# chenruduan/OAReactDiff

Hardware: AMD Instinct MI355X
Metric: denoising_steps_per_sec (higher is better)
Workload: dtype f32; 1 GPU; EGNNDynamics.forward (LEFTNet H=196 R=96 L=6), B=64 reactions/GPU x 3 objects x 23 atoms, complete graph per reaction (N=4416, E=300288), T=1000 sampler step shape; batch_per_gpu=64, atoms_per_object=23, parallelism=replica x1 (no collective), launch=eager

## Files before the change

oareactdiff_amd/_capi.py:

```python
from __future__ import annotations

import ctypes as C
import os

from .build import LIB

OARD_MAX_OBJECTS = 8
ABI_VERSION = 2048
OARD_OK, OARD_EINVAL, OARD_ENOTCOMPLETE, OARD_EHIP, OARD_ENOMEM = 0, -1, -2, -3, -4
ERRORS = {OARD_EINVAL: "invalid argument / unsupported configuration", OARD_ENOTCOMPLETE: "topology is not complete-per-sample",
          OARD_EHIP: "HIP runtime error", OARD_ENOMEM: "workspace too small"}

PREC_GCL_BF16X3, PREC_EQUI_BF16X3, PREC_TRAIN_BF16X3 = 1, 2, 4
TAP_S, TAP_VEC, TAP_EDGE, TAP_POS_FRAME, TAP_DPOS, TAP_HOUT, TAP_LABELS, TAP_NE1 = 1, 2, 3, 4, 5, 6, 7, 8

EXPORTS = ["oard_version", "oard_supported", "oard_param_count", "oard_packed_bytes", "oard_pack_weights",
           "oard_topology_create", "oard_topology_destroy", "oard_topology_num_nodes", "oard_topology_num_edges",
           "oard_topology_num_inner_edges", "oard_topology_num_samples", "oard_topology_check_edge_index",
           "oard_workspace_bytes", "oard_forward", "oard_active_inner_edges", "oard_debug_lin3u_table", "oard_sampler_step", "oard_sampler_step_dev", "oard_inpaint_step", "oard_inpaint_step_dev", "oard_tap", "oard_debug_stop_after", "oard_debug_option", "oard_timing_enable", "oard_timing_reset",
           "oard_timing_get",
           "oard_topology_create_parts", "oard_topology_export", "oard_tape_bytes", "oard_tape_entry", "oard_forward_train",
           "oard_packed_bwd_bytes", "oard_pack_weights_bwd", "oard_gcl_backward_dx", "oard_edge_node_sums",
           "oard_equi_backward_dx", "oard_scalarize_backward", "oard_equi_msg_backward", "oard_lin3u_forward", "oard_lin3u_backward", "oard_wgrad_scratch_bytes", "oard_wgrad",
           "oard_train_scratch_bytes", "oard_train_scratch_poison", "oard_train_scratch_entry", "oard_train_tail_backward",
           "oard_train_layer_backward", "oard_train_init_backward", "oard_train_stage_backward",
           "oard_loss_prepare", "oard_loss_terms", "oard_loss_eval_prepare", "oard_loss_eval_terms", "oard_adamw_step", "oard_adamw_step_dev", "oard_nan_replace",
           "oard_adamw_step_ema", "oard_adamw_step_dev_ema", "oard_ema_update", "oard_kabsch_rmsd", "oard_matched_rmsd", "oard_rank_metrics",
           "oard_graph_create", "oard_graph_destroy", "oard_graph_num_nodes", "oard_graph_num_edges", "oard_graph_object_rows",
           "oard_graph_is_complete", "oard_graph_workspace_bytes", "oard_graph_forward", "oard_library_stream",
           "oard_confidence_forward", "oard_confidence_forward_train", "oard_confidence_tail_backward", "oard_dataset_gather"]
STAGE_RECOMPUTE, STAGE_UPDATE, STAGE_MESSAGE, STAGE_GCL_NODE, STAGE_NODE_PRE, STAGE_GCL_EDGE, STAGE_EQUI_EDGE = range(7)
SCRATCH_XH, SCRATCH_XQ, SCRATCH_CR, SCRATCH_DCD, SCRATCH_DCR = range(1, 6)

TOPO_NODE_REF, TOPO_NODE_OBJ, TOPO_NODE_ROW, TOPO_NODE_SAMPLE, TOPO_NODE_TIDX, TOPO_SAMPLE_PTR, TOPO_GROUP_PTR, \
    TOPO_INNER_SRC, TOPO_INNER_TGT, TOPO_ROW_SRC, TOPO_ROW_TGT = range(1, 12)
TAPE_HIN, TAPE_GEO, TAPE_RBF, TAPE_PP0, TAPE_X1 = 1, 2, 3, 4, 5
TAPE_S_IN, TAPE_VEC_IN, TAPE_EW, TAPE_AGG, TAPE_S_MID, TAPE_Z1, TAPE_Z2, TAPE_ATT, TAPE_Z3, TAPE_ZD1, TAPE_CD, TAPE_S_A, TAPE_VEC_A = range(16, 29)


class OardConfig(C.Structure):
    _fields_ = [
        ("hidden", C.c_int32), ("num_radial", C.c_int32), ("num_layers", C.c_int32), ("in_hidden", C.c_int32),
        ("n_obj", C.c_int32), ("node_nf", C.c_int32 * OARD_MAX_OBJECTS), ("enc_alias", C.c_int32 * OARD_MAX_OBJECTS),
        ("condition_nf", C.c_int32), ("condition_time", C.c_int32), ("pos_dim", C.c_int32), ("cutoff", C.c_float),
        ("reflect_equiv", C.c_int32), ("precision", C.c_int32),
    ]


OARD_STORE_OBJECTS = 3


class OardReactionStore(C.Structure):
    _fields_ = [
        ("offsets", C.c_void_p * OARD_STORE_OBJECTS), ("pos", C.c_void_p * OARD_STORE_OBJECTS), ("z", C.c_void_p * OARD_STORE_OBJECTS),
        ("sel", C.c_void_p), ("target", C.c_void_p), ("rmsd", C.c_void_p), ("ediff", C.c_void_p * 2),
        ("n_raw", C.c_int64), ("n_sel", C.c_int64), ("n_obj", C.c_int32),
        ("src_obj", C.c_int32 * OARD_STORE_OBJECTS), ("reflect_obj", C.c_int32 * OARD_STORE_OBJECTS),
        ("append_charge", C.c_int32 * OARD_STORE_OBJECTS),
        ("swap", C.c_int32), ("reflect", C.c_int32), ("center", C.c_int32), ("zero_charge", C.c_int32), ("append_frag", C.c_int32),
    ]


class OardError(RuntimeError):
    pass


def check(rc: int, what: str) -> None:
    if rc != OARD_OK:
        raise OardError(f"{what} failed: {ERRORS.get(rc, rc)}")


def ptr_array(tensors, n=None):
    if tensors is None:
        return None
    ptrs = [None if t is None else t.data_ptr() for t in tensors]
    return (C.c_void_p * (len(ptrs) if n is None else n))(*ptrs)


_lib = None


def lib() -> C.CDLL:
    global _lib
    if _lib is not None:
        return _lib
    if not os.path.exists(LIB):
        raise OardError(f"{LIB} not found: build it with `python -m oareactdiff_amd.build` "
                        "(there is no CPU fallback for the HIP backend)")
    L = C.CDLL(LIB)
    vp, i32, i64, sz = C.c_void_p, C.c_int32, C.c_int64, C.c_size_t
    cfgp = C.POINTER(OardConfig)
    L.oard_version.restype = C.c_int
    got = L.oard_version()
    if got != ABI_VERSION:
        raise OardError(f"{LIB} has ABI version {got}, this package expects {ABI_VERSION}: rebuild it "
                        "(`python -m oareactdiff_amd.build --force`, or the script that made the OARD_LIB build)")
    L.oard_supported.argtypes = [cfgp]; L.oard_supported.restype = C.c_int
    L.oard_param_count.argtypes = [cfgp]; L.oard_param_count.restype = sz
    L.oard_packed_bytes.argtypes = [cfgp]; L.oard_packed_bytes.restype = sz
    L.oard_pack_weights.argtypes = [cfgp, C.POINTER(vp), sz, vp, sz, vp]; L.oard_pack_weights.restype = C.c_int
    L.oard_topology_create.argtypes = [cfgp, C.POINTER(i64), C.POINTER(i64), i64, C.POINTER(vp)]
    L.oard_topology_create.restype = C.c_int
    L.oard_topology_destroy.argtypes = [vp]; L.oard_topology_destroy.restype = None
    for f in ("oard_topology_num_nodes", "oard_topology_num_edges", "oard_topology_num_inner_edges",
              "oard_topology_num_samples"):
        getattr(L, f).argtypes = [vp]; getattr(L, f).restype = i64
    L.oard_topology_check_edge_index.argtypes = [vp, vp, i64, vp, vp]; L.oard_topology_check_edge_index.restype = C.c_int
    L.oard_workspace_bytes.argtypes = [cfgp, vp]; L.oard_workspace_bytes.restype = sz
    L.oard_forward.argtypes = [cfgp, vp, vp, C.POINTER(vp), vp, C.c_int, vp, C.POINTER(vp), vp, sz, vp, vp]
    L.oard_forward.restype = C.c_int
    L.oard_confidence_forward.argtypes = [cfgp, vp, vp, C.POINTER(vp), C.POINTER(vp), vp, C.c_int, vp, vp, vp, sz, vp, vp]
    L.oard_confidence_forward.restype = C.c_int
    L.oard_confidence_forward_train.argtypes = [cfgp, vp, vp, C.POINTER(vp), C.POINTER(vp), vp, C.c_int, vp, vp, vp, sz, vp, sz, vp, vp]
    L.oard_confidence_forward_train.restype = C.c_int
    L.oard_confidence_tail_backward.argtypes = [cfgp, vp, vp, C.POINTER(vp), vp, vp, vp, C.POINTER(vp), vp, sz, vp]
    L.oard_confidence_tail_backward.restype = C.c_int
    L.oard_debug_lin3u_table.argtypes = [cfgp, vp, C.c_int, vp, vp]; L.oard_debug_lin3u_table.restype = C.c_int
    L.oard_active_inner_edges.argtypes = [cfgp, vp, vp, sz, C.POINTER(i64), vp]; L.oard_active_inner_edges.restype = C.c_int
    L.oard_sampler_step.argtypes = [cfgp, vp, C.c_int, C.POINTER(vp), C.POINTER(vp), C.POINTER(vp), C.POINTER(vp),
                                    C.c_float, C.c_float, C.c_float, C.c_int, C.POINTER(vp), vp]
    L.oard_sampler_step.restype = C.c_int
    L.oard_sampler_step_dev.argtypes = [cfgp, vp, C.c_int, C.POINTER(vp), C.POINTER(vp), C.POINTER(vp), C.POINTER(vp), vp, C.c_int,
                                        C.POINTER(vp), vp]
    L.oard_sampler_step_dev.restype = C.c_int
    pv = C.POINTER(vp)
    L.oard_inpaint_step.argtypes = [cfgp, vp, C.c_uint, pv, pv, pv, pv, pv, pv, pv, C.POINTER(C.c_float), C.c_int, pv, vp]
    L.oard_inpaint_step.restype = C.c_int
    L.oard_inpaint_step_dev.argtypes = [cfgp, vp, C.c_uint, pv, pv, pv, pv, pv, pv, pv, vp, C.c_int, pv, vp]
    L.oard_inpaint_step_dev.restype = C.c_int
    L.oard_tap.argtypes = [cfgp, vp, vp, C.c_int, C.c_int, vp, vp]; L.oard_tap.restype = C.c_int
    ci = C.c_int
    L.oard_topology_create_parts.argtypes = [cfgp, C.POINTER(i64), C.POINTER(i64), i64, ci, C.POINTER(vp)]
    L.oard_topology_create_parts.restype = ci
    L.oard_topology_export.argtypes = [vp, ci, vp, i64, vp]; L.oard_topology_export.restype = ci
    L.oard_tape_bytes.argtypes = [cfgp, vp]; L.oard_tape_bytes.restype = sz
    L.oard_tape_entry.argtypes = [cfgp, vp, ci, ci, C.POINTER(sz), C.POINTER(i64), C.POINTER(i64)]; L.oard_tape_entry.restype = ci
    L.oard_forward_train.argtypes = [cfgp, vp, vp, C.POINTER(vp), vp, ci, vp, C.POINTER(vp), vp, sz, vp, sz, vp, vp]
    L.oard_forward_train.restype = ci
    L.oard_packed_bwd_bytes.argtypes = [cfgp]; L.oard_packed_bwd_bytes.restype = sz
    L.oard_pack_weights_bwd.argtypes = [cfgp, C.POINTER(vp), sz, vp, sz, vp]; L.oard_pack_weights_bwd.restype = ci
    L.oard_gcl_backward_dx.argtypes = [cfgp, vp, vp, ci, vp, vp, vp, vp, vp, vp, vp, vp, vp]; L.oard_gcl_backward_dx.restype = ci
    L.oard_edge_node_sums.argtypes = [cfgp, vp, vp, vp, vp, vp]; L.oard_edge_node_sums.restype = ci
    L.oard_equi_backward_dx.argtypes = [cfgp, vp, vp, ci, vp, vp, vp, vp, vp]; L.oard_equi_backward_dx.restype = ci
    L.oard_scalarize_backward.argtypes = [cfgp, vp, vp, vp, vp, ci, vp, vp, vp, vp]; L.oard_scalarize_backward.restype = ci
    L.oard_equi_msg_backward.argtypes = [cfgp, vp, vp, ci, vp, vp, vp, vp, vp, vp, vp, vp, vp]; L.oard_equi_msg_backward.restype = ci
    L.oard_lin3u_forward.argtypes = [cfgp, vp, ci, vp, i64, vp, vp]; L.oard_lin3u_forward.restype = ci
    L.oard_lin3u_backward.argtypes = [cfgp, vp, ci, vp, vp, i64, vp, vp, vp, vp, vp, vp, vp]; L.oard_lin3u_backward.restype = ci
    L.oard_wgrad_scratch_bytes.argtypes = [ci, ci, i64]; L.oard_wgrad_scratch_bytes.restype = sz
    L.oard_wgrad.argtypes = [vp, ci, ci, ci, ci, ci, vp, ci, ci, ci, ci, ci, ci, i64, vp, vp, vp, sz, vp]; L.oard_wgrad.restype = ci
    pvp = C.POINTER(vp)
    L.oard_train_scratch_bytes.argtypes = [cfgp, vp]; L.oard_train_scratch_bytes.restype = sz
    L.oard_train_scratch_poison.argtypes = [cfgp, vp, vp, sz, vp]; L.oard_train_scratch_poison.restype = ci
    L.oard_train_scratch_entry.argtypes = [cfgp, vp, ci, C.POINTER(sz), C.POINTER(i64), C.POINTER(i64)]; L.oard_train_scratch_entry.restype = ci
    L.oard_train_tail_backward.argtypes = [cfgp, vp, vp, vp, vp, pvp, vp, vp, pvp, pvp, vp, sz, vp]; L.oard_train_tail_backward.restype = ci
    L.oard_train_layer_backward.argtypes = [cfgp, vp, vp, vp, vp, ci, vp, vp, vp, pvp, pvp, vp, sz, vp]; L.oard_train_layer_backward.restype = ci
    L.oard_train_init_backward.argtypes = [cfgp, vp, vp, vp, vp, pvp, vp, vp, pvp, pvp, vp, sz, vp]; L.oard_train_init_backward.restype = ci
    L.oard_train_stage_backward.argtypes = [cfgp, vp, vp, vp, vp, ci, ci, vp, vp, vp, vp, vp, vp, pvp, pvp, vp, sz, vp]
    L.oard_train_stage_backward.restype = ci
    L.oard_nan_replace.argtypes = [cfgp, vp, vp, pvp, pvp, vp]; L.oard_nan_replace.restype = ci
    pf, cf = C.POINTER(C.c_float), C.c_float
    L.oard_loss_prepare.argtypes = [cfgp, vp, pvp, pvp, pvp, pvp, vp, vp, ci, pf, pf, ci, ci, pvp, pvp, vp]; L.oard_loss_prepare.restype = ci
    L.oard_loss_terms.argtypes = [cfgp, vp, pvp, pvp, pvp, pvp, pvp, vp, vp, ci, pf, pf, pf, ci, ci, vp, vp, pvp, vp]; L.oard_loss_terms.restype = ci
    cd = C.c_double
    L.oard_loss_eval_prepare.argtypes = [cfgp, vp, pvp, pvp, pvp, pvp, pvp, vp, vp, ci, pf, pf, ci, ci, pvp, pvp, pvp, pvp, vp]
    L.oard_loss_eval_prepare.restype = ci
    L.oard_loss_eval_terms.argtypes = [cfgp, vp, pvp, pvp, pvp, pvp, pvp, pvp, pvp, vp, vp, vp, ci, pf, pf, pf, ci, cd, ci, vp, vp, vp]
    L.oard_loss_eval_terms.restype = ci
    L.oard_adamw_step.argtypes = [vp, vp, vp, vp, vp, i64, cd, cd, cd, cd, cd, i64, ci, cd, vp]; L.oard_adamw_step.restype = ci
    L.oard_adamw_step_dev.argtypes = [vp, vp, vp, vp, vp, i64, cd, cd, cd, cd, cd, ci, ci, vp, ci, vp, vp, vp, vp]; L.oard_adamw_step_dev.restype = ci
    L.oard_adamw_step_ema.argtypes = [vp, vp, vp, vp, vp, i64, cd, cd, cd, cd, cd, i64, ci, cd, vp, cd, vp]; L.oard_adamw_step_ema.restype = ci
    L.oard_adamw_step_dev_ema.argtypes = [vp, vp, vp, vp, vp, i64, cd, cd, cd, cd, cd, ci, ci, vp, ci, vp, vp, vp, vp, cd, vp]
    L.oard_adamw_step_dev_ema.restype = ci
    L.oard_ema_update.argtypes = [vp, vp, i64, cd, vp]; L.oard_ema_update.restype = ci
    L.oard_kabsch_rmsd.argtypes = [vp, i64, vp, i64, vp, i64, ci, cf, vp, vp, vp, vp]; L.oard_kabsch_rmsd.restype = ci
    L.oard_matched_rmsd.argtypes = [vp, i64, vp, i64, vp, vp, vp, i64, ci, cf, ci, vp, vp, vp, vp, vp, vp]; L.oard_matched_rmsd.restype = ci
    L.oard_rank_metrics.argtypes = [vp, vp, i64, vp, i64, vp, vp, vp, vp]; L.oard_rank_metrics.restype = ci
    L.oard_dataset_gather.argtypes = [C.POINTER(OardReactionStore), vp, pvp, i64, i64, pvp, pvp, pvp, pvp, pvp, vp, vp, vp, vp, vp]
    L.oard_dataset_gather.restype = ci
    L.oard_library_stream.argtypes = [ci, pvp]; L.oard_library_stream.restype = ci
    L.oard_graph_create.argtypes = [cfgp, vp, vp, i64, vp, i64, pvp]; L.oard_graph_create.restype = ci
    L.oard_graph_destroy.argtypes = [vp]; L.oard_graph_destroy.restype = None
    L.oard_graph_num_nodes.argtypes = [vp]; L.oard_graph_num_nodes.restype = i64
    L.oard_graph_num_edges.argtypes = [vp]; L.oard_graph_num_edges.restype = i64
    L.oard_graph_object_rows.argtypes = [vp, ci]; L.oard_graph_object_rows.restype = i64
    L.oard_graph_is_complete.argtypes = [vp]; L.oard_graph_is_complete.restype = ci
    L.oard_graph_workspace_bytes.argtypes = [cfgp, vp]; L.oard_graph_workspace_bytes.restype = sz
    L.oard_graph_forward.argtypes = [cfgp, vp, pvp, sz, pvp, vp, ci, vp, pvp, vp, sz, vp, vp]; L.oard_graph_forward.restype = ci
    L.oard_debug_stop_after.argtypes = [C.c_int]; L.oard_debug_stop_after.restype = C.c_int
    L.oard_debug_option.argtypes = [C.c_char_p, C.c_int]; L.oard_debug_option.restype = C.c_int
    L.oard_timing_enable.argtypes = [C.c_int]; L.oard_timing_enable.restype = C.c_int
    L.oard_timing_reset.argtypes = []; L.oard_timing_reset.restype = C.c_int
    L.oard_timing_get.argtypes = [C.c_char_p, C.POINTER(C.c_double), C.POINTER(i64)]; L.oard_timing_get.restype = C.c_int
    for env, opt in (("OARD_GCL_VARIANT", b"gcl_variant"), ("OARD_EQUI_VARIANT", b"equi_variant"),
                     ("OARD_NODE_VARIANT", b"node_variant"), ("OARD_GCL_SKIP", b"gcl_skip"), ("OARD_EQUI_SKIP", b"equi_skip"), ("OARD_EQUI_L0_SKIP", b"equi_l0_skip"), ("OARD_EQUI_RBF_TABLE", b"equi_rbf_table"),("OARD_GCL_MSUM", b"gcl_msum"), ("OARD_GCL_PERSIST", b"gcl_persist"), ("OARD_GCL_GRID", b"gcl_grid"), ("OARD_PARTS", b"parts"), ("OARD_SEQUENTIAL", b"sequential"), ("OARD_POISON", b"poison"), ("OARD_AUTO_SMALL", b"auto_small"), ("OARD_AUTO_TINY", b"auto_tiny"), ("OARD_NPB", b"npb"),
                     ("OARD_WGRAD_WGS", b"wgrad_wgs"), ("OARD_WGRAD_LDS", b"wgrad_lds"), ("OARD_WGRAD_T16", b"wgrad_t16"), ("OARD_WGRAD_QUEUE", b"wgrad_queue"), ("OARD_GATE_FOLD", b"gate_fold"), ("OARD_WGRAD_SHAPES", b"wgrad_shapes"), ("OARD_TRAIN_DUAL", b"train_dual"), ("OARD_SMALL_SPLIT", b"small_split"),
                     ("OARD_SKIP_FAMILIES", b"skip_families")):
        if os.environ.get(env) not in (None, ""):
            check(L.oard_debug_option(opt, int(os.environ[env])), f"oard_debug_option({opt.decode()})")
    _lib = L
    return L


def timing_get(family: str):
    ms, n = C.c_double(0.0), C.c_int64(0)
    check(lib().oard_timing_get(family.encode(), C.byref(ms), C.byref(n)), "oard_timing_get")
    return ms.value, n.value
```

oareactdiff_amd/csrc/oard_hip.hip:

```cpp
#include <algorithm>
#include <cmath>
#include <cstdio>
#include <cstring>
#include <map>
#include <string>
#include <vector>
#include <mutex>
#include <chrono>
#include <utility>

#include "oard_kernels.h"
#include "oard_edge_v1.h"
#include "oard_edge_p.h"
#include "oard_wgrad_t16.h"
#include "oard_edge_b3.h"
#ifdef OARD_EXPERIMENTS
#include "oard_edge_fp.h"
#endif
#include "oard_node_v1.h"
#include "oard_edge_small.h"
#include "oard_edge_bwd.h"
#include "oard_node_bwd.h"
#include "oard_rows.h"
#include "oard_conf.h"
#include "oard_conf_bwd.h"
#include "oard_plan.h"
#include "oard_inst.h"

#define OARD_VERSION 2048
#ifdef OARD_EXPERIMENTS
static constexpr bool kV0 = true;
#else
static constexpr bool kV0 = false;
#endif

#define HIP_TRY(x) do { hipError_t e_ = (x); if (e_ != hipSuccess) { \
    fprintf(stderr, "liboard_hip: %s failed: %s (%s:%d)\n", #x, hipGetErrorString(e_), __FILE__, __LINE__); \
    return OARD_EHIP; } } while (0)

namespace {
enum Family { F_GCL_EDGE = 0, F_EQUI_EDGE, F_NODE, F_INIT, F_OTHER, F_GCL_BWD, F_EQUI_BWD, F_WGRAD, F_COUNT };
const char* kFamilyNames[F_COUNT] = {"gcl_edge", "equi_edge", "node", "init", "other", "gcl_edge_bwd", "equi_edge_bwd", "wgrad"};
struct TimingRec { hipEvent_t a, b; int fam; };
struct Timing {
    bool on = false;
    std::vector<TimingRec> recs;
    std::vector<hipEvent_t> pool;
    double total_ms[F_COUNT] = {0};
    long long launches[F_COUNT] = {0};
    hipEvent_t get() {
        if (!pool.empty()) { hipEvent_t e = pool.back(); pool.pop_back(); return e; }
        hipEvent_t e; (void)hipEventCreate(&e); return e;
    }
    void flush() {
        for (auto& r : recs) {
            (void)hipEventSynchronize(r.b);
            float ms = 0.f;
            (void)hipEventElapsedTime(&ms, r.a, r.b);
            total_ms[r.fam] += ms; launches[r.fam] += 1;
            pool.push_back(r.a); pool.push_back(r.b);
        }
        recs.clear();
    }
} g_timing;
int g_stop_after = 0;
FwdOptions g_fwd;
int g_sequential = 0;
int g_npb = 0;
int g_poison = 0;
int g_gcl_msum_taken = 0;
int g_equi_l0_taken = 0;
int g_equi_rbf_taken = 0;
int g_parts = 0;
int g_wgrad_shapes = 3;
int g_wgrad_t16 = 256;
int g_wgrad_lds = 256;
int g_wgrad_wgs = 512;
int g_skip_families = 0;

struct ScopedLaunch {
    hipStream_t st; hipEvent_t a; int fam; bool on;
    ScopedLaunch(int f, hipStream_t s) : st(s), fam(f), on(g_timing.on) {
        if (on) { a = g_timing.get(); (void)hipEventRecord(a, st); }
    }
    ~ScopedLaunch() {
        if (on) { hipEvent_t b = g_timing.get(); (void)hipEventRecord(b, st); g_timing.recs.push_back({a, b, fam}); }
    }
};
#define LAUNCH(fam, kern, grid, block, stream, ...) do { ScopedLaunch sl_(fam, stream); if (!((g_skip_families >> (fam)) & 1)) \
    hipLaunchKernelGGL(kern, dim3((unsigned)(grid)), dim3(block), 0, stream, __VA_ARGS__); } while (0)
#define LAUNCH2(fam, kern, gx, gy, block, stream, ...) do { ScopedLaunch sl_(fam, stream); if (!((g_skip_families >> (fam)) & 1)) \
    hipLaunchKernelGGL(kern, dim3((unsigned)(gx), (unsigned)(gy)), dim3(block), 0, stream, __VA_ARGS__); } while (0)

#ifndef OARD_DIMS_LIST
#define OARD_DIMS_LIST X(196, 96) X(32, 8) X(32, 32)
#endif

inline size_t align_up(size_t x, size_t a) { return (x + a - 1) / a * a; }
inline long long cdiv(long long a, long long b) { return (a + b - 1) / b; }

bool config_ok(const oard_config* c) {
    if (!c) return false;
    bool dims = false;
#define X(h, r) dims = dims || (c->hidden == (h) && c->num_radial == (r));
    OARD_DIMS_LIST
#undef X
    if (!dims) return false;
    if (c->num_layers < 1 || c->num_layers > OARD_MAX_LAYERS) return false;
    if (c->in_hidden < 1 || c->in_hidden > 16) return false;
    if (c->n_obj < 1 || c->n_obj > OARD_MAX_OBJECTS) return false;
    if (c->pos_dim != 3 || (c->reflect_equiv != 0 && c->reflect_equiv != 1)) return false;
    if (c->precision & ~(OARD_PREC_GCL_BF16X3 | OARD_PREC_EQUI_BF16X3 | OARD_PREC_TRAIN_BF16X3)) return false;
    const int emb = c->in_hidden - (c->condition_time ? 1 : 0) - (c->condition_nf > 0 ? c->condition_nf : 0);
    if (emb < 1) return false;
    for (int k = 0; k < c->n_obj; ++k) {
        const int d = c->node_nf[k] - 3;
        if (d < 1 || d > 16) return false;
        const int a = c->enc_alias[k];
        if (a < 0 || a >= c->n_obj || c->node_nf[a] != c->node_nf[k]) return false;
    }
    return true;
}
int embed_dim(const oard_config* c) {
    return c->in_hidden - (c->condition_time ? 1 : 0) - (c->condition_nf > 0 ? c->condition_nf : 0);
}

PackOff make_layout(const oard_config* c) {
    const RDims d(c->hidden, c->num_radial);
    PackOff po;
    memset(&po, 0, sizeof(po));
    size_t cur = 0;
    auto take = [&](size_t n) { size_t o = cur; cur = align_up(cur + n, 64); return o; };
    auto mat = [&](int MT, int KB) { return take((size_t)MT * KB * 256); };
    const int emb = embed_dim(c);
    po.emb = mat(d.HT, 1); po.emb_b = take(d.HP);
    po.nbemb = mat(d.HT, 1); po.nbemb_b = take(d.HP);
    po.s2v = mat(d.HT, d.HT); po.s2v_b = take(d.HP);
    po.rl0 = mat(d.HT, d.RB); po.rl0_b = take(d.HP);
    po.rl2 = mat(d.HT, d.HT); po.rl2_b = take(d.HP);
    po.lin3 = take((size_t)d.H4 * 5 + 1);
    po.pe0 = take((size_t)d.H2 * 3);
    po.pe1 = mat(d.HT, d.PB);
    po.embout = mat(1, d.HT); po.embout_b = take(16);
    po.v1p = mat(d.HT, d.HT); po.v2p = take(d.HP);
    po.un0 = mat(d.HT, 2 * d.HT); po.un0_b = take(d.HP);
    po.un2 = mat(1, d.HT); po.un2_b = take(16);
    po.c0row = take(d.WP);
    po.u0 = take(d.HP);
    po.rbf_means = take(d.RP); po.rbf_betas = take(d.RP);
    for (int k = 0; k < c->n_obj; ++k) {
        const int dd = c->node_nf[k] - 3;
        po.enc[k] = take((size_t)2 * dd * dd + 2 * dd + (size_t)emb * 2 * dd + emb);
        po.dec[k] = take((size_t)2 * dd * emb + 2 * dd + (size_t)dd * 2 * dd + dd);
    }
    for (int l = 0; l < c->num_layers; ++l) {
        LayerOff& lo = po.layer[l];
        lo.ln_g_w = take(d.HP); lo.ln_g_b = take(d.HP);
        lo.W1a = mat(d.HT, d.HT); lo.b1 = take(d.HP);
        lo.W1b = mat(d.HT, d.HT);
        lo.W1c = mat(d.HT, d.WB);
        lo.W2 = mat(d.HT, d.HT); lo.b2 = take(d.HP);
        lo.watt = take(d.HP); lo.batt = take(1);
        lo.W3 = mat(d.WB, d.HT); lo.b3 = take(d.WP);
        lo.nm0 = mat(d.HT, 2 * d.HT); lo.nm0b = take(d.HP);
        lo.nm1 = mat(d.HT, d.HT); lo.nm1b = take(d.HP);
        lo.ln_q_w = take(d.HP); lo.ln_q_b = take(d.HP);
        lo.xp0 = mat(d.HT, d.HT);
        lo.xp2 = mat(3 * d.HT, d.HT);
        lo.dp0 = mat(d.D1T, d.WB); lo.dp0b = take(d.D1P);
        lo.dp2 = mat(3 * d.HT, d.D1T); lo.dp2b = take(3 * d.HP);
        lo.rbfp = mat(3 * d.HT, d.RB);
        lo.rbfw = take((size_t)3 * d.H * d.R); lo.rbff = take(4);
        lo.vp = mat(2 * d.HT, d.HT);
        lo.xv0 = mat(d.HT, 2 * d.HT);
        lo.xv2 = mat(3 * d.HT, d.HT);
        lo.l3u = take(593);
        lo.l3t = take(L3T_FLOATS);
        lo.gcl_stream = take((size_t)(d.WB * d.HT + (d.HT + 1) * (d.HT + 1) + d.WB * (d.HT + 1)) * 256);
        lo.equi_stream = take((size_t)(d.WB * d.D1T + 3 * d.HT * (1 + d.D1T + d.RB)) * 256);
        {
            const int nbh = (d.HT + 1) / 2, nbw = (d.WB + 1) / 2;
            lo.gcl_b3 = take((size_t)(nbw * 3 * d.HT + (d.HT + 1) * (1 + 3 * nbh) + d.WB * (1 + 3 * nbh)) * 256);
            lo.equi_b3 = take((size_t)(nbw * 3 * d.D1T + ((d.RB + 1) / 2 + (d.D1T + 1) / 2) * 9 * d.HT) * 256);
        }
    }
    po.head = cur;
    for (int l = 0; l < c->num_layers; ++l) po.layer[l].rbft = take(rbt_layer_floats(d.HT));
    po.total = cur;
    po.signed_scal = c->reflect_equiv ? 0 : 1;
    for (int l = 0; l < c->num_layers; ++l) po.layer[l].xcross = c->reflect_equiv ? 0 : 1;
    return po;
}

struct ParamIdx {
    int emb_w, emb_b, embout_w, embout_b, means, betas, nbemb_w, nbemb_b, s2v_w, s2v_b, rl0_w, rl0_b, rl2_w, rl2_b,
        lin30_w, lin30_b, lin32_w, lin32_b, pe0_w, pe1_w;
    int gcl0, msg0, upd0, out0, enc0, dec0, count;
    explicit ParamIdx(const oard_config* c) {
        int i = 0;
        emb_w = i++; emb_b = i++; embout_w = i++; embout_b = i++; means = i++; betas = i++;
        nbemb_w = i++; nbemb_b = i++; s2v_w = i++; s2v_b = i++; rl0_w = i++; rl0_b = i++; rl2_w = i++; rl2_b = i++;
        lin30_w = i++; lin30_b = i++; lin32_w = i++; lin32_b = i++; pe0_w = i++; pe1_w = i++;
        i += 2;
        gcl0 = i; i += 14 * c->num_layers;
        msg0 = i; i += 9 * c->num_layers;
        upd0 = i; i += 9 * c->num_layers;
        i += 2;
        out0 = i; i += 6;
        enc0 = i; i += 4 * c->n_obj;
        dec0 = i; i += 4 * c->n_obj;
        count = i;
    }
};

struct Packer {
    const float* const* p; float* blob; hipStream_t st;
    std::vector<GenJob> jobs;
    long long blocks = 0;
    void push(GenJob j, size_t work) {
        j.block0 = blocks;
        blocks += cdiv((long long)std::max<size_t>(work, 1), 256);
        jobs.push_back(j);
    }
    void matrix(int src, int src_ld, int col_off, int msl, int msp, int ms, int ksl, int ksp, int ks, int MT, int KB,
                size_t dst, size_t tstride = 0, size_t bstride = 256, int perm_ht = 0, int transpose = 0, int tail_compact = 0,
                int rows4 = 0) {
        if (tstride == 0) tstride = (size_t)KB * 256;
        GenJob j;
        memset(&j, 0, sizeof(j));
        j.type = 0;
        j.m = PackJob{p[src], src_ld, col_off, msl, msp, ms, ksl, ksp, ks, MT, KB, dst, tstride, bstride, perm_ht, transpose, rows4, tail_compact};
        push(j, (size_t)MT * KB * 256);
    }
    void nat(int src, int src_ld, int col_off, int M, int K, int MT, int KB, size_t dst) {
        matrix(src, src_ld, col_off, M, MT * 16, 1, K, KB * 16, 1, MT, KB, dst);
    }
    void vec(int src, int sect_len, int sect_pad, int sects, int n_dst, size_t dst) {
        GenJob j;
        memset(&j, 0, sizeof(j));
        j.type = 1; j.src = src >= 0 ? p[src] : nullptr; j.dst = dst; j.sect_len = sect_len; j.sect_pad = sect_pad; j.sects = sects; j.n = n_dst;
        push(j, (size_t)n_dst);
    }
    void bias_chunks(int src, int sect_len, int sect_pad, int sects, int n_tiles, size_t dst, size_t tstride,
                     int perm_ht = 0) {
        GenJob j;
        memset(&j, 0, sizeof(j));
        j.type = 2; j.src = p[src]; j.dst = dst; j.sect_len = sect_len; j.sect_pad = sect_pad; j.sects = sects; j.n = n_tiles * 256;
        j.tstride = tstride; j.perm_ht = perm_ht;
        push(j, (size_t)n_tiles * 256);
    }
    void raw(int src, int n, size_t dst) {
        GenJob j;
        memset(&j, 0, sizeof(j));
        j.type = 3; j.src = p[src]; j.dst = dst; j.n = n;
        push(j, (size_t)n);
    }
    int flush() {
        if (jobs.empty()) return OARD_OK;
        struct Cached { std::vector<GenJob> host; GenJob* dev = nullptr; size_t cap = 0; };
        static std::mutex mu;
        static std::map<std::pair<const void*, int>, Cached> cache;
        int devid = 0;
        (void)hipGetDevice(&devid);
        const GenJob* table = nullptr;
        {
            std::lock_guard<std::mutex> lk(mu);
            Cached& c = cache[{(const void*)blob, devid}];
            const bool same = c.host.size() == jobs.size() && memcmp(c.host.data(), jobs.data(), jobs.size() * sizeof(GenJob)) == 0;
            if (!same) {
                HIP_TRY(hipStreamSynchronize(st));
                if (c.cap < jobs.size()) {
                    if (c.dev) (void)hipFree(c.dev);
                    HIP_TRY(hipMalloc((void**)&c.dev, jobs.size() * sizeof(GenJob)));
                    c.cap = jobs.size();
                }
                HIP_TRY(hipMemcpy(c.dev, jobs.data(), jobs.size() * sizeof(GenJob), hipMemcpyHostToDevice));
                c.host = jobs;
            }
            table = c.dev;
        }
        hipLaunchKernelGGL(k_pack_all, dim3((unsigned)blocks), dim3(256), 0, st, table, (int)jobs.size(), blob);
        jobs.clear();
        blocks = 0;
        return OARD_OK;
    }
};
struct RbfTablesOf { const void* blob; unsigned good; };
static std::mutex g_rbf_mu;
static std::vector<RbfTablesOf> g_rbf_known;
static void rbf_tables_forget(const void* blob) {
    std::lock_guard<std::mutex> lk(g_rbf_mu);
    g_rbf_known.erase(std::remove_if(g_rbf_known.begin(), g_rbf_known.end(), [&](const RbfTablesOf& e) { return e.blob == blob; }), g_rbf_known.end());
}
static int rbf_tables_for(const oard_config* c, const PackOff& po, const float* blob, hipStream_t st, unsigned* good) {
    *good = 0;
    std::lock_guard<std::mutex> lk(g_rbf_mu);
    for (const RbfTablesOf& e : g_rbf_known) if (e.blob == blob) { *good = e.good; return OARD_OK; }
    hipStreamCaptureStatus cap = hipStreamCaptureStatusNone;
    HIP_TRY(hipStreamIsCapturing(st, &cap));
    if (cap != hipStreamCaptureStatusNone) return OARD_OK;
    const RDims d(c->hidden, c->num_radial);
    RbtJobs j;
    memset(&j, 0, sizeof(j));
    for (int l = 0; l < c->num_layers; ++l) { j.w[l] = po.layer[l].rbfw; j.tab[l] = po.layer[l].rbft; j.flag[l] = po.layer[l].rbff; }
    j.means = po.rbf_means; j.betas = po.rbf_betas; j.H = d.H; j.HT = d.HT; j.R = d.R;
    hipLaunchKernelGGL(k_rbf_table_fill, dim3((unsigned)cdiv((long long)3 * d.HT * (RBT_N + 1) * 4, 256), (unsigned)c->num_layers), dim3(256), 0, st,
                       const_cast<float*>(blob), j);
    hipLaunchKernelGGL(k_rbf_table_check, dim3((unsigned)(3 * d.HT * 4), (unsigned)c->num_layers), dim3(256), 0, st, const_cast<float*>(blob), j);
    HIP_TRY(hipGetLastError());
    std::vector<float> flags((size_t)c->num_layers, 0.f);
    for (int l = 0; l < c->num_layers; ++l)
        HIP_TRY(hipMemcpyAsync(&flags[l], blob + po.layer[l].rbff, sizeof(float), hipMemcpyDeviceToHost, st));
    HIP_TRY(hipStreamSynchronize(st));
    unsigned mask = 0;
    for (int l = 0; l < c->num_layers; ++l) if (flags[l] == 1.0f) mask |= 1u << l;
    if (g_rbf_known.size() >= 64) g_rbf_known.erase(g_rbf_known.begin());
    g_rbf_known.push_back({blob, mask});
    *good = mask;
    return OARD_OK;
}

#define OARD_SMALL_MAX_EDGES (512 * 16 * 16)
static WsOff make_ws(const oard_config* c, const TopoDev& td) {
    const RDims d(c->hidden, c->num_radial);
    const size_t N = td.N, E = td.E + 1, A = td.A + 1;
    WsOff w;
    size_t cur = 0;
    auto take = [&](size_t bytes) { size_t o = cur; cur = align_up(cur + bytes, 256); return o; };
    w.pos = take(N * 3 * 4); w.pf64 = take(N * 3 * 8); w.pf32 = take(N * 3 * 4); w.x1 = take(N * 3 * 4);
    w.pp0 = take(N * 4); w.labels = take(N * 4); w.hin = take(N * 16 * 4);
    w.zemb = take(N * d.HP * 4); w.nb = take(N * d.HP * 4); w.s = take(N * d.HP * 4); w.s1 = take(N * d.HP * 4);
    w.ne1 = take(N * 3 * d.HP * 4); w.xh = take(N * d.HP * 4); w.P = take(N * d.HP * 4); w.Q = take(N * d.HP * 4);
    w.xq = take(N * 3 * d.HP * 4); w.vec = take(N * 3 * d.HP * 4); w.vec2 = take(N * 3 * d.HP * 4); w.v2buf = take(N * 3 * d.HP * 4);
    w.sc0 = take(N * d.HP * 4); w.vdot = take(N * d.HP * 4);
    w.geo = take(A * GEO_STRIDE * 4); w.d64 = take(A * 8); w.rbuf = take(A * d.RP * 4);
    w.ew = take(E * d.WP * 4); w.mbuf = take(std::max(E, (size_t)(td.CI + td.CX) + 1) * d.HP * 4);
    w.xmsg = take(A * d.HP * 4); w.vmsg = take(A * 3 * d.HP * 4);
    w.dpos = take(N * 3 * 4); w.hout = take(N * 16 * 4);
    w.al_rows = take(A * 4); w.al_src = take(A * 4); w.al_pre = take(A * 4); w.al_cnt = take((size_t)cdiv((long long)td.A, 256) * 4 + 4); w.al_n = take(4);
    w.d1s = take((size_t)cdiv((long long)td.A, 128) * 8 * d.D1T * 1024);
    w.small_a = E <= (size_t)OARD_SMALL_MAX_EDGES ? take(A * d.D1P * 4) : 0;
    w.rbt = take(A * RBT_ROW * 4);
    w.total = cur;
    return w;
}



template <class K>
int set_lds(K kernel, size_t bytes) {
    HIP_TRY(hipFuncSetAttribute((const void*)kernel, hipFuncAttributeMaxDynamicSharedMemorySize, (int)bytes));
    return OARD_OK;
}

#define LAUNCH_LDS(fam, kern, grid, block, lds, stream, ...) do { \
    static bool attr_done_[64] = {}; \
    int dev_ = 0; (void)hipGetDevice(&dev_); dev_ &= 63; \
    if (!attr_done_[dev_]) { int rc_ = set_lds(kern, lds); if (rc_ != OARD_OK) return rc_; attr_done_[dev_] = true; } \
    ScopedLaunch sl_(fam, stream); if (!((g_skip_families >> (fam)) & 1)) \
    hipLaunchKernelGGL(kern, dim3((unsigned)(grid)), dim3(block), lds, stream, __VA_ARGS__); } while (0)

static int device_cus() {
    static int cus[64] = {};
    int d = 0;
    (void)hipGetDevice(&d);
    d &= 63;
    if (!cus[d]) {
        int n = 0;
        if (hipDeviceGetAttribute(&n, hipDeviceAttributeMultiprocessorCount, d) != hipSuccess || n < 1) { (void)hipGetLastError(); n = 256; }
        cus[d] = n;
    }
    return cus[d];
}
struct GclArgs {
    const TopoDev& tp; const float* wb; const LayerOff& lo;
    const float *stream, *P, *Q, *u0, *c0; float *ew_in, *ew_out, *mbuf;
    GclTape tape; hipStream_t st;
};
template <class D, bool S1, bool S3>
int launch_gcl_v1s(const GclLaunch& L, bool msum, const GclArgs& a) {
    constexpr size_t RING3 = GclStream<D, 2>::LDS_BYTES / 2 * 3;
#define GCL_STREAMED(kern, waves, lds, w_) do { LAUNCH_LDS(F_GCL_EDGE, kern, L.grid, (waves) * 64, lds, a.st, a.tp, w_, a.P, a.Q, a.u0, a.c0, \
                                                           L.r0, L.r1, a.ew_in, a.ew_out, a.mbuf, a.tape); return OARD_OK; } while (0)
    switch ((int)L.shape) {
        case GCL_PERSIST:
            if (msum) GCL_STREAMED((k_gcl_edge_p<D, S1, S3, false, true>), 8, RING3, a.stream);
            GCL_STREAMED((k_gcl_edge_p<D, S1, S3>), 8, RING3, a.stream);
        case GCL_RING3:
            if (msum) GCL_STREAMED((k_gcl_edge_v1<D, 8, 2, S1, S3, false, true, 2, 3>), 8, RING3, a.stream);
            GCL_STREAMED((k_gcl_edge_v1<D, 8, 2, S1, S3, false, false, 2, 3>), 8, RING3, a.stream);
        case GCL_TRAIN_PERSIST: GCL_STREAMED((k_gcl_edge_p<D, S1, S3, true>), 8, RING3, a.stream);
        case GCL_TRAIN_RING3: GCL_STREAMED((k_gcl_edge_v1<D, 8, 2, S1, S3, true, false, 2, 3>), 8, RING3, a.stream);
        case GCL_B3: GCL_STREAMED((k_gcl_edge_b3<D, S1, S3>), 8, (GclB3Stream<D>::LDS_BYTES), a.wb + a.lo.gcl_b3);
        case GCL_TRAIN_B3: GCL_STREAMED((k_gcl_edge_b3<D, S1, S3, true>), 8, (GclB3Stream<D>::LDS_BYTES), a.wb + a.lo.gcl_b3);
        case GCL_W4: GCL_STREAMED((k_gcl_edge_v1<D, 4, 2, S1, S3, false>), 4, (GclStream<D, 2>::LDS_BYTES), a.stream);
        case GCL_SMALL:
            LAUNCH_LDS(F_GCL_EDGE, (k_gcl_edge_small<D, 8, S1, S3>), L.grid, 512, (GclSmall<D>::LDS_BYTES), a.st,
                       a.tp, a.wb, a.lo, a.P, a.Q, a.u0, a.c0, L.r0, L.r1, a.ew_out, a.mbuf);
            return OARD_OK;
#ifdef OARD_EXPERIMENTS
        case GCL_V0: LAUNCH(F_GCL_EDGE, (k_gcl_edge<D>), L.grid, 256, a.st, a.tp, a.wb, a.lo, a.P, a.Q, a.ew_in, a.mbuf); return OARD_OK;
        case GCL_X0 + 7: GCL_STREAMED((k_gcl_edge_v1<D, 8, 2, S1, S3, false>), 8, (GclStream<D, 2>::LDS_BYTES), a.stream);
        case GCL_X0 + 8: GCL_STREAMED((k_gcl_edge_v1<D, 8, 3, S1, S3, false>), 8, (GclStream<D, 3>::LDS_BYTES), a.stream);
        case GCL_X0 + 9: GCL_STREAMED((k_gcl_edge_v1<D, 8, 4, S1, S3, false>), 8, (GclStream<D, 4>::LDS_BYTES), a.stream);
        case GCL_X0 + 4: GCL_STREAMED((k_gcl_edge_fp<D, 8, 2, S1, S3, false>), 8, (GclRing<D, 2, 4>::LDS_BYTES), a.stream);
        case GCL_X0 + 5: GCL_STREAMED((k_gcl_edge_fp<D, 8, 2, S1, S3, false, 3>), 8, (GclRing<D, 2, 3>::LDS_BYTES), a.stream);
        case GCL_X0 + 10: GCL_STREAMED((k_gcl_edge_v1<D, 12, 1, S1, S3, false, false, 3>), 12, (GclStream<D, 1>::LDS_BYTES), a.stream);
        case GCL_X0 + 11: GCL_STREAMED((k_gcl_edge_v1<D, 12, 2, S1, S3, false, false, 3>), 12, (GclStream<D, 2>::LDS_BYTES), a.stream);
        case GCL_X0 + 12: GCL_STREAMED((k_gcl_edge_v1<D, 4, 1, S1, S3, false, false, 3>), 4, (GclStream<D, 1>::LDS_BYTES), a.stream);
#endif
        default: return OARD_EINVAL;
    }
#undef GCL_STREAMED
}
template <class D>
int launch_gcl_v1(const GclLayer& g, bool msum, const GclArgs& a) {
    for (int i = 0; i < g.n; ++i) {
        const GclLaunch& L = g.l[i];
        const int rc = L.s1 ? (L.s3 ? launch_gcl_v1s<D, true, true>(L, msum, a) : launch_gcl_v1s<D, true, false>(L, msum, a))
                            : (L.s3 ? launch_gcl_v1s<D, false, true>(L, msum, a) : launch_gcl_v1s<D, false, false>(L, msum, a));
        if (rc != OARD_OK) return rc;
    }
    return OARD_OK;
}
template <class D>
int launch_equi_v1(const FwdPlan& plan, int l, const TopoDev& tp, const float* wb, const LayerOff& lo, const float* stream, const float* dp0b,
                   const float* ew, const float* rbuf, float* qbuf, float* zd1, float* cd, hipStream_t st, float* d1s, float* small, ActList al,
                   const float* rbt) {
    const long long tiles = cdiv(tp.A, 16);
    switch (plan.equi) {
        case EQ_TRAIN_B3:
            LAUNCH_LDS(F_EQUI_EDGE, (k_equi_edge_b3<D, true>), cdiv(tp.A, 16 * 8), 8 * 64, (EquiB3Stream<D>::LDS_BYTES), st, tp, wb + lo.equi_b3,
                       dp0b, wb + lo.dp2b, ew, rbuf, qbuf, d1s, zd1, cd, ActList{});
            return OARD_OK;
        case EQ_TRAIN:
            LAUNCH_LDS(F_EQUI_EDGE, (k_equi_edge_v1<D, 8, true>), cdiv(tp.A, 16 * 8), 8 * 64, (EquiStream<D>::LDS_BYTES), st,
                       tp, stream, dp0b, ew, rbuf, qbuf, zd1, cd, ActList{}, 0, (const float*)nullptr);
            return OARD_OK;
        case EQ_SMALL_SPLIT:
            LAUNCH_LDS(F_EQUI_EDGE, (k_equi_small_s1<D, 8>), tiles * cdiv(D::D1T, 8), 512, (size_t)D::WB * 1024, st, tp, wb, lo, ew, small);
            LAUNCH_LDS(F_EQUI_EDGE, (k_equi_small_s2<D, 8>), tiles * cdiv(3 * D::HT, 8), 512, (size_t)(D::D1T + D::RB) * 1024, st,
                       tp, wb, lo, (const float*)small, rbuf, qbuf);
            return OARD_OK;
        case EQ_SMALL:
            LAUNCH_LDS(F_EQUI_EDGE, (k_equi_edge_small<D, 8>), tiles, 512, (EquiSmall<D>::LDS_BYTES), st, tp, wb, lo, ew, rbuf, qbuf);
            return OARD_OK;
        case EQ_B3:
            LAUNCH_LDS(F_EQUI_EDGE, (k_equi_edge_b3<D>), cdiv(tp.A, 16 * 8), 8 * 64, (EquiB3Stream<D>::LDS_BYTES), st, tp, wb + lo.equi_b3,
                       dp0b, wb + lo.dp2b, ew, rbuf, qbuf, d1s, nullptr, nullptr, al);
            return OARD_OK;
        case EQ_W4:
            LAUNCH_LDS(F_EQUI_EDGE, (k_equi_edge_v1<D, 4, false>), cdiv(tp.A, 16 * 4), 4 * 64, (EquiStream<D>::LDS_BYTES), st,
                       tp, stream, dp0b, ew, rbuf, qbuf, nullptr, nullptr, al, 0, (const float*)nullptr);
            return OARD_OK;
        case EQ_W8:
            if (plan.rbf_table[l])
                LAUNCH_LDS(F_EQUI_EDGE, (k_equi_edge_v1<D, 8, false, true>), cdiv(tp.A, 16 * 8), 8 * 64, (EquiStream<D>::LDS_BYTES), st,
                           tp, stream, dp0b, ew, rbt, qbuf, nullptr, nullptr, al, plan.l0_skip && l == 0 ? 1 : 0, wb + lo.rbft);
            else
                LAUNCH_LDS(F_EQUI_EDGE, (k_equi_edge_v1<D, 8, false>), cdiv(tp.A, 16 * 8), 8 * 64, (EquiStream<D>::LDS_BYTES), st,
                           tp, stream, dp0b, ew, rbuf, qbuf, nullptr, nullptr, al, plan.l0_skip && l == 0 ? 1 : 0, (const float*)nullptr);
            return OARD_OK;
        default: return OARD_EINVAL;
    }
}

struct TapeOff {
    size_t hin, geo, rbuf, pp0, x1;
    size_t s_in[OARD_MAX_LAYERS + 1], vec_in[OARD_MAX_LAYERS + 1];
    size_t agg[OARD_MAX_LAYERS], s_mid[OARD_MAX_LAYERS];
    size_t s_a[OARD_MAX_LAYERS], vec_a[OARD_MAX_LAYERS];
    size_t ew[OARD_MAX_LAYERS + 1];
    size_t z1[OARD_MAX_LAYERS], z2[OARD_MAX_LAYERS], att[OARD_MAX_LAYERS], z3[OARD_MAX_LAYERS];
    size_t zd1[OARD_MAX_LAYERS], cd[OARD_MAX_LAYERS];
    size_t total;
};
static TapeOff make_tape(const oard_config* c, const TopoDev& td) {
    const RDims d(c->hidden, c->num_radial);
    const size_t N = td.N, E = td.E + 1, A = td.A + 1;
    TapeOff t;
    memset(&t, 0, sizeof(t));
    size_t cur = 0;
    auto take = [&](size_t bytes) { size_t o = cur; cur = align_up(cur + bytes, 256); return o; };
    t.hin = take(N * 16 * 4); t.geo = take(A * GEO_STRIDE * 4); t.rbuf = take(A * d.RP * 4); t.pp0 = take(N * 4); t.x1 = take(N * 3 * 4);
    for (int l = 0; l <= c->num_layers; ++l) {
        t.s_in[l] = take(N * d.HP * 4); t.vec_in[l] = take(N * 3 * d.HP * 4); t.ew[l] = take(E * d.WP * 4);
        if (l == c->num_layers) break;
        t.agg[l] = take(N * d.HP * 4); t.s_mid[l] = take(N * d.HP * 4);
        t.s_a[l] = take(N * d.HP * 4); t.vec_a[l] = take(N * 3 * d.HP * 4);
        t.z1[l] = take(E * d.HP * 4); t.z2[l] = take(E * d.HP * 4); t.att[l] = take(E * 4); t.z3[l] = take(E * d.WP * 4);
        t.zd1[l] = take(A * d.D1P * 4); t.cd[l] = take(A * 3 * d.HP * 4);
    }
    t.total = cur;
    return t;
}

struct ConfHead { ConfReadout w; float* out; };
template <class D>
static int forward_impl(const FwdOptions& opt, const oard_config* c, const TopoPart* topo, const float* wb, const float* const* xh,
                        const float* t, int t_scalar, const float* cond, float* const* out, char* ws, char* tape,
                        int* status, hipStream_t st, const ConfHead* conf = nullptr) {
    const TopoDev& tp = topo->d;
    const PackOff po = make_layout(c);
    const WsOff w = make_ws(c, tp);
    const bool train = tape != nullptr;
    const TapeOff to = train ? make_tape(c, tp) : TapeOff{};
    const int emb = embed_dim(c);
    float* pos = (float*)(ws + w.pos); double* pf64 = (double*)(ws + w.pf64); float* pf32 = (float*)(ws + w.pf32);
    auto slot = [&](size_t ws_off, size_t tape_off) -> float* { return train ? (float*)(tape + tape_off) : (float*)(ws + ws_off); };
    float* x1 = slot(w.x1, to.x1); float* pp0 = slot(w.pp0, to.pp0); int* labels = (int*)(ws + w.labels);
    float* hin = slot(w.hin, to.hin); float* zemb = (float*)(ws + w.zemb); float* nb = (float*)(ws + w.nb);
    float* s = (float*)(ws + w.s); float* s1 = (float*)(ws + w.s1); float* ne1 = (float*)(ws + w.ne1);
    float* xhb = (float*)(ws + w.xh); float* P = (float*)(ws + w.P); float* Q = (float*)(ws + w.Q);
    float* xq = (float*)(ws + w.xq); float* vec = slot(w.vec, to.vec_in[0]); float* v2buf = (float*)(ws + w.v2buf);
    float* scal = (float*)(ws + w.sc0); float* vdot = (float*)(ws + w.vdot);
    float* geo = slot(w.geo, to.geo); double* d64 = (double*)(ws + w.d64); float* rbuf = slot(w.rbuf, to.rbuf);
    float* mbuf = (float*)(ws + w.mbuf); float* xmsg = (float*)(ws + w.xmsg);
    float* vmsg = (float*)(ws + w.vmsg); float* dpos = (float*)(ws + w.dpos); float* hout = (float*)(ws + w.hout);
    auto ew_at = [&](int l) -> float* { return train ? (float*)(tape + to.ew[l]) : (float*)(ws + w.ew); };
    float* ew = ew_at(0);
    auto s_at = [&](int l) -> float* { return train ? (float*)(tape + to.s_in[l]) : s; };
    auto s_mid_at = [&](int l) -> float* { return train ? (float*)(tape + to.s_mid[l]) : s; };

    ObjPtrs op;
    memset(&op, 0, sizeof(op));
    for (int k = 0; k < c->n_obj; ++k) {
        op.xh[k] = xh[k]; op.out[k] = out ? out[k] : nullptr; op.node_nf[k] = c->node_nf[k]; op.enc[k] = po.enc[k]; op.dec[k] = po.dec[k];
    }
    const long long N = tp.N, E = tp.E, A = tp.A;
    const unsigned gN = (unsigned)cdiv(N, 64), gA = (unsigned)cdiv(A, 64);
    const double cutoff = (double)c->cutoff;
    FwdPlanIn plan_in{opt, c->precision, train, topo->conc, tp.npb, device_cus(), A, E, tp.CI, tp.CX, c->num_layers, w.small_a != 0};
    if (plan_rbf_wanted(plan_in)) { const int rc = rbf_tables_for(c, po, wb, st, &plan_in.rbf_good); if (rc != OARD_OK) return rc; }
    const FwdPlan plan = make_fwd_plan(plan_in);
    bool any_rbt = false, all_rbt = c->num_layers > 0;
    for (int l = 0; l < c->num_layers; ++l) { any_rbt = any_rbt || plan.rbf_table[l]; all_rbt = all_rbt && plan.rbf_table[l]; }
    g_equi_rbf_taken = all_rbt;
    const bool msum = plan.msum, use_al = plan.use_al, nv1 = plan.node != NODE_V0;
    const int stop_after = train ? 0 : g_stop_after;
    int* al_cnt = (int*)(ws + w.al_cnt);
    const ActList al = use_al ? ActList{(const int*)(ws + w.al_rows), (const int*)(ws + w.al_src), (const int*)(ws + w.al_pre), (const int*)(ws + w.al_n)}
                              : ActList{nullptr, nullptr, nullptr, nullptr};
    if (!use_al) HIP_TRY(hipMemsetAsync(ws + w.al_n, 0xff, sizeof(int), st));
    LAUNCH(F_OTHER, k_prep, cdiv(N, 128), 128, st, tp, op, wb, pos, hin, t, t_scalar, cond,
           c->condition_nf > 0 ? c->condition_nf : 0, c->condition_time, emb);
    LAUNCH(F_INIT, k_geom, tp.n_groups, 64, st, tp, (const float*)pos, cutoff, pf64, pf32, x1, pp0, labels);
    if (plan.fill_edges || stop_after == 1)
        LAUNCH(F_INIT, k_fill_edges, std::min<long long>(cdiv((E - A + 1) * (D::WP / 4), 256), 8192), 256, st,
               wb + po.c0row, ew + (size_t)A * D::WP, E - A + 1, D::WP);
    if (A > 0) {
        LAUNCH(F_INIT, k_edge_geo, cdiv(A, 256), 256, st, tp, (const float*)pos, (const double*)pf64, cutoff, geo, d64, use_al ? al_cnt : nullptr);
        if (use_al) LAUNCH(F_INIT, k_active_list, cdiv(A, 256), 256, st, tp, (const float*)geo, (const int*)al_cnt, (int*)al.rows, (int*)al.src, (int*)al.pre, (int*)al.n);
        LAUNCH(F_INIT, k_rbf, cdiv(A * D::RP, 256), 256, st, tp, (const double*)d64, (const float*)geo,
               wb + po.rbf_means, wb + po.rbf_betas, cutoff, rbuf, ew, D::R, D::RP, D::H, D::WP, any_rbt ? (float*)(ws + w.rbt) : (float*)nullptr);
    }
    LAUNCH(F_INIT, (k_node_embed<D>), gN, 256, st, tp, wb, po, (const float*)hin, zemb, nb);
    if (A > 0) LAUNCH(F_INIT, (k_radial_lin<D>), gA, 256, st, tp, wb, po, (const float*)rbuf, (const float*)geo, ew);
    constexpr int NW = D::HT <= 16 ? D::HT : 8;
    const unsigned gNb = (unsigned)cdiv(N, tp.npb);
    if (plan.init_v1) {
        LAUNCH(F_INIT, (k_neighbor_v1<D, NW>), gNb, NW * 64, st, tp, wb, po, (const float*)zemb, (const float*)nb, (const float*)ew, s_at(0), s1);
        LAUNCH(F_INIT, (k_s2v_agg_v1<D, NW>), gNb, NW * 64, st, tp, (const float*)s1, (const float*)ew, (const float*)geo, ne1);
    } else if constexpr (kV0) {
        LAUNCH(F_INIT, (k_neighbor<D>), gN, 256, st, tp, wb, po, (const float*)zemb, (const float*)nb, (const float*)ew, s_at(0), s1);
        LAUNCH(F_INIT, (k_s2v_agg<D>), gN, 256, st, tp, (const float*)s1, (const float*)ew, (const float*)geo, ne1);
    } else return OARD_EINVAL;
    if (A > 0) LAUNCH2(F_INIT, (k_scalarize<D>), gA, (plan.scalarize_tiles ? D::HT : 1), 256, st, tp, wb, po, (const float*)ne1, (const float*)geo, ew);
    HIP_TRY(hipMemsetAsync(vec, 0, (size_t)N * 3 * D::HP * sizeof(float), st));
    if (stop_after == 1) return OARD_OK;

    float* vec2 = (float*)(ws + w.vec2);
    float* vcur = vec;
    float* vnext = vec2;
    g_gcl_msum_taken = msum;
    for (int l = 0; l < c->num_layers; ++l) {
        const LayerOff lo = po.layer[l];
        const unsigned gN16 = (unsigned)cdiv(N, tp.npb);
        float* ew_in = ew_at(l);
        float* ew_out = ew_at(l + 1);
        if (train) vnext = (float*)(tape + to.vec_in[l + 1]);

        if (nv1) LAUNCH(F_NODE, (k_node_pre_v1<D, NW>), gN16, NW * 64, st, tp, wb, po, lo, (const float*)s_at(l), (const float*)pp0, xhb, P, Q);
        else if constexpr (kV0) LAUNCH(F_NODE, (k_node_pre<D>), gN, 256, st, tp, wb, po, lo, (const float*)s, (const float*)pp0, xhb, P, Q);
        else return OARD_EINVAL;
        GclTape gt{};
        if (train) gt = GclTape{(float*)(tape + to.z1[l]), (float*)(tape + to.z2[l]), (float*)(tape + to.att[l]), (float*)(tape + to.z3[l])};
        int rc = launch_gcl_v1<D>(plan.gcl_at(l), msum, GclArgs{tp, wb, lo, wb + lo.gcl_stream, P, Q, wb + po.u0, wb + po.c0row, ew_in, ew_out, mbuf, gt, st});
        if (rc != OARD_OK) return rc;
        const bool rows = plan.node == NODE_ROWS;
        if (nv1 && rows) LAUNCH(F_NODE, (k_gcl_node_v1<D, NW, true>), gN16, NW * 64, st, tp, wb, lo, (const float*)xhb, (const float*)mbuf, s_mid_at(l), xq,
                                train ? (float*)(tape + to.agg[l]) : nullptr);
        else if (nv1 && msum) LAUNCH(F_NODE, (k_gcl_node_v1<D, NW, false, true>), gN16, NW * 64, st, tp, wb, lo, (const float*)xhb, (const float*)mbuf, s_mid_at(l), xq,
                                     (float*)nullptr);
        else if (nv1) LAUNCH(F_NODE, (k_gcl_node_v1<D, NW, false>), gN16, NW * 64, st, tp, wb, lo, (const float*)xhb, (const float*)mbuf, s_mid_at(l), xq,
                             train ? (float*)(tape + to.agg[l]) : nullptr);
        else if constexpr (kV0) LAUNCH(F_NODE, (k_gcl_node<D>), gN, 256, st, tp, wb, lo, (const float*)xhb, (const float*)mbuf, s, xq);
        else return OARD_EINVAL;
        if (stop_after == 100 + 10 * l + 1) { topo->vec_final = (size_t)((char*)vcur - ws); return OARD_OK; }
        if (plan.equi == EQ_V0) {
            if constexpr (kV0) {
                if (A > 0) LAUNCH(F_EQUI_EDGE, (k_equi_edge<D>), gA, 256, st, tp, wb, lo, (const float*)ew_out, (const float*)rbuf,
                                  (const float*)geo, (const float*)xq, (const float*)vcur, xmsg, vmsg);
                LAUNCH(F_NODE, (k_equi_agg<D>), gN, 256, st, tp, wb, lo, (const float*)xmsg, (const float*)vmsg, (const float*)x1,
                       s, vcur, v2buf, scal, vdot);
            } else return OARD_EINVAL;
        } else {
            const bool l0_skip = l == 0 && plan.l0_skip;
            if (l == 0) g_equi_l0_taken = l0_skip;
            if (A > 0) {
                rc = launch_equi_v1<D>(plan, l, tp, wb, lo, wb + lo.equi_stream, wb + lo.dp0b, ew_out, rbuf, vmsg,
                                       train ? (float*)(tape + to.zd1[l]) : nullptr, train ? (float*)(tape + to.cd[l]) : nullptr, st,
                                       (float*)(ws + w.d1s), (float*)(ws + w.small_a), al, (const float*)(ws + w.rbt));
                if (rc != OARD_OK) return rc;
            }
#define EQUI_NODE_V1(D_, ROWS_, XC_) LAUNCH(F_NODE, (k_equi_node_v1<D_, NW, ROWS_, XC_>), gN16, NW * 64, st, tp, wb, lo, (const float*)vmsg, \
                       (const float*)xq, (const float*)geo, (const float*)x1, (const float*)s_mid_at(l), s_at(l + 1), (const float*)vcur, vnext, \
                       train ? (float*)(tape + to.s_a[l]) : nullptr, train ? (float*)(tape + to.vec_a[l]) : nullptr, al)
            if (nv1 && rows) {
                if (lo.xcross) EQUI_NODE_V1(D, true, true); else EQUI_NODE_V1(D, true, false);
            } else if (nv1 && l0_skip) {
                if (lo.xcross) EQUI_NODE_V1(Layer0<D>, false, true); else EQUI_NODE_V1(Layer0<D>, false, false);
            } else if (nv1) {
                if (lo.xcross) EQUI_NODE_V1(D, false, true); else EQUI_NODE_V1(D, false, false);
            } else if constexpr (kV0) {
                LAUNCH(F_NODE, (k_equi_agg_v1<D>), gN, 256, st, tp, wb, lo, (const float*)vmsg, (const float*)xq,
                       (const float*)geo, (const float*)x1, s, (const float*)vcur, vnext, v2buf, scal, vdot);
            } else return OARD_EINVAL;
            std::swap(vcur, vnext);
        }
        if constexpr (kV0) {
            if (!nv1) LAUNCH(F_NODE, (k_equi_upd<D>), gN, 256, st, tp, wb, lo, (const float*)scal, (const float*)vdot,
                             (const float*)v2buf, s, vcur);
        }
        if (stop_after == 100 + 10 * l + 2) { topo->vec_final = (size_t)((char*)vcur - ws); return OARD_OK; }
    }
    if (!train) topo->vec_final = (size_t)((char*)vcur - ws);
    if (train) {
        ZeroRows z;
        z.count = 0;
        auto add = [&](size_t off, size_t row, int ld) {
            if (z.count == 64) { LAUNCH(F_OTHER, k_zero_rows, 64, 256, st, z); z.count = 0; }
            z.p[z.count] = (float*)(tape + off) + row * (size_t)ld; z.n[z.count] = ld; ++z.count;
        };
        for (int l = 0; l <= c->num_layers; ++l) {
            add(to.ew[l], (size_t)E, D::WP);
            if (l == c->num_layers) break;
            add(to.z1[l], (size_t)E, D::HP); add(to.z2[l], (size_t)E, D::HP); add(to.att[l], (size_t)E, 1); add(to.z3[l], (size_t)E, D::WP);
            add(to.zd1[l], (size_t)A, D::D1P); add(to.cd[l], (size_t)A, 3 * D::HP);
        }
        add(to.geo, (size_t)A, GEO_STRIDE); add(to.rbuf, (size_t)A, D::RP);
        if (z.count > 0) LAUNCH(F_OTHER, k_zero_rows, z.count, 256, st, z);
    }
    if (conf) {
        ScopedLaunch sl_(F_OTHER, st);
        hipLaunchKernelGGL(k_conf_readout, dim3((unsigned)tp.B), dim3(CONF_WAVES * 64), 5 * D::H * sizeof(double), st, tp,
                           (const float*)s_at(c->num_layers), D::H, D::HP, conf->w, conf->out, status);
        HIP_TRY(hipGetLastError());
        return OARD_OK;
    }
    if (plan.init_v1)
        LAUNCH(F_NODE, (k_out_v1<D, NW>), gNb, NW * 64, st, tp, wb, po, (const float*)s_at(c->num_layers), (const float*)vcur, dpos, hout, status);
    else if constexpr (kV0)
        LAUNCH(F_NODE, (k_out<D>), gN, 256, st, tp, wb, po, (const float*)s, (const float*)vcur, dpos, hout, status);
    else return OARD_EINVAL;
    LAUNCH(F_OTHER, k_post, cdiv(N, 128), 128, st, tp, op, wb, (const float*)dpos, (const float*)hout, emb);
    HIP_TRY(hipGetLastError());
    return OARD_OK;
}

template <class F> static int dispatch_dims(const oard_config* c, F&& f) {
#define X(h, r) if (c->hidden == (h) && c->num_radial == (r)) { f(Dims<(h), (r)>{}); return 0; }
    OARD_DIMS_LIST
#undef X
    return OARD_EINVAL;
}
#define DISPATCH_DIMS(c, CALL)                                                                         \
    do {                                                                                               \
        if (dispatch_dims((c), [&](auto d_) { using D = decltype(d_); CALL; }) != 0) return OARD_EINVAL; \
    } while (0)

struct BwdLayerOff { size_t gcl, equi, watt; };
struct BwdOff { BwdLayerOff layer[OARD_MAX_LAYERS]; size_t total; };
static BwdOff make_bwd_layout(const oard_config* c) {
    const RDims d(c->hidden, c->num_radial);
    BwdOff b;
    memset(&b, 0, sizeof(b));
    size_t cur = 0;
    auto take = [&](size_t n) { size_t o = cur; cur = align_up(cur + n, 64); return o; };
    for (int l = 0; l < c->num_layers; ++l) {
        b.layer[l].gcl = take((size_t)(2 * d.WB * d.HT + d.HT * d.HT) * 256);
        b.layer[l].equi = take((size_t)(3 * d.HT * d.D1T + d.WB * d.D1T) * 256);
        b.layer[l].watt = take(d.HP);
    }
    b.total = cur;
    return b;
}
template <class D>
static int gcl_backward_impl(const oard_config* c, const TopoDev& tp, const float* pb, const BwdLayerOff& bl, int layer,
                             const char* tape, const TapeOff& to, const float* dagg, float* dew, float* dz3, float* mout,
                             float* dz2, float* da, float* dz1, hipStream_t st, float* gate_part = nullptr, long long* gate_rows = nullptr) {
    GclBwdArgs a;
    a.gate_part = gate_part;
    a.z1 = (const float*)(tape + to.z1[layer]); a.z2 = (const float*)(tape + to.z2[layer]);
    a.att = (const float*)(tape + to.att[layer]); a.z3 = (const float*)(tape + to.z3[layer]);
    a.dagg = dagg; a.watt = pb + bl.watt; a.dew = dew; a.dz3 = dz3; a.mout = mout; a.dz2 = dz2; a.da = da; a.dz1 = dz1;
    const float* stream = pb + bl.gcl;
    const bool last = layer == c->num_layers - 1;
    const long long r_full = last ? tp.A : tp.E;
    long long rows = 0;
    if (r_full > 0) {
        LAUNCH_LDS(F_GCL_BWD, (k_gcl_edge_bwd<D, 8, 2, true>), cdiv(r_full, 128), 512, (GclBwdStream<D, 2>::LDS_BYTES), st,
                   tp, stream, 0LL, r_full, a);
        rows += cdiv(r_full, 128) * 8;
    }
    if (last && tp.E > tp.A) {
        if (a.gate_part) a.gate_part += (size_t)rows * D::HP;
        LAUNCH_LDS(F_GCL_BWD, (k_gcl_edge_bwd<D, 8, 2, false>), cdiv(tp.E - tp.A, 128), 512, (GclBwdStream<D, 2>::LDS_BYTES), st,
                   tp, stream, tp.A, tp.E, a);
        rows += cdiv(tp.E - tp.A, 128) * 8;
    }
    if (gate_rows) *gate_rows = rows;
    HIP_TRY(hipGetLastError());
    return OARD_OK;
}

template <class D>
static int equi_backward_impl(const TopoDev& tp, const float* stream, const float* dcd, const float* zd1, float* dew,
                              float* dzd1, hipStream_t st) {
    LAUNCH_LDS(F_EQUI_BWD, (k_equi_edge_bwd<D, 8>), cdiv(tp.A, 128), 512, (EquiBwdStream<D>::LDS_BYTES), st, tp, stream, dcd,
               zd1, dew, dzd1);
    HIP_TRY(hipGetLastError());
    return OARD_OK;
}

#ifndef OARD_SCAL_BWD_WAVES
#define OARD_SCAL_BWD_WAVES 2
#endif
template <class D>
static int scalarize_backward_impl(const oard_config* c, const TopoDev& tp, const float* wb, const char* tape, const TapeOff& to,
                                   const float* ne1, int ld, const float* dew, float* dne1, float* part, hipStream_t st) {
    const PackOff po = make_layout(c);
    constexpr int NW = OARD_SCAL_BWD_WAVES;
    if (po.signed_scal)
        LAUNCH(F_INIT, (k_scalarize_bwd<D, NW, true>), tp.N, NW * 64, st, tp, wb + po.lin3, ne1, ld, (const float*)(tape + to.geo), dew, dne1, part);
    else
        LAUNCH(F_INIT, (k_scalarize_bwd<D, NW, false>), tp.N, NW * 64, st, tp, wb + po.lin3, ne1, ld, (const float*)(tape + to.geo), dew, dne1, part);
    HIP_TRY(hipGetLastError());
    return OARD_OK;
}

template <class D>
static int equi_msg_backward_impl(const oard_config* c, const TopoDev& tp, const char* tape, const TapeOff& to, int layer, const float* xq, const float* cr,
                                  const float* gs, const float* gv, float* dcd, float* dcr, float* dxq, float* dvec, hipStream_t st) {
    const Strided3 xq3{xq, 3 * D::H, D::H}, vec3{(const float*)(tape + to.vec_in[layer]), 3 * D::HP, D::HP}, cr3{cr, 3 * D::H, D::H},
        gv3{gv, 3 * D::H, D::H};
    LAUNCH(F_NODE, (k_equi_msg_bwd<D>), tp.N, 256, st, tp, (const float*)(tape + to.geo), xq3, vec3, (const float*)(tape + to.cd[layer]), cr3,
           gs, D::H, gv3, dcd, dcr, dxq, dvec, D::H, c->reflect_equiv ? 0 : 1);
    HIP_TRY(hipGetLastError());
    return OARD_OK;
}

struct WgradPlan { int transposed, NT, nPB, nQG, PP, QP, gy; long long rpc; int n_chunks; int lds, PBW, QGW;
                   long long cap; };
struct WglShape { int NT, PBW, QGW; };
static const WglShape kWglShapes[2] = {{7, 4, 2}, {8, 4, 2}};
static WgradPlan wgrad_plan(int ncY, int ncX, long long rows) {
    WgradPlan p;
    p.transposed = ncX > ncY ? 1 : 0;
    const int ncP = p.transposed ? ncX : ncY, ncQ = p.transposed ? ncY : ncX;
    const int nQT = (int)cdiv(ncQ, 16);
    p.NT = (cdiv(nQT, 7) * 7 <= cdiv(nQT, 8) * 8) ? 7 : 8;
    p.nPB = (int)cdiv(ncP, 64); p.nQG = (int)cdiv(nQT, p.NT);
    p.PP = p.nPB * 64; p.QP = p.nQG * p.NT * 16;
    p.gy = (int)cdiv((long long)p.nPB * p.nQG, 4);
    long long want = std::max<long long>(1, g_wgrad_wgs / p.gy);
    want = std::min(want, std::max<long long>(1, cdiv(rows, rows < 16384 ? 128 : 64)));
    p.rpc = align_up((size_t)cdiv(std::max<long long>(rows, 1), want), 4 * OARD_WG_PD);
    p.n_chunks = (int)cdiv(std::max<long long>(rows, 1), p.rpc);
    p.cap = want;
    p.lds = 0; p.PBW = 4; p.QGW = 2;
    if (g_wgrad_lds > 0 && rows >= 16384) {
        long long best = -1;
        for (int k = 0; k < 2; ++k) {
            if (!((g_wgrad_shapes >> k) & 1)) continue;
            const WglShape& c = kWglShapes[k];
            const long long nQG = cdiv(nQT, c.NT);
            if (nQG < 2) continue;
            const long long sP = cdiv(p.nPB, c.PBW) * c.PBW, sQ = cdiv(nQG, c.QGW) * c.QGW;
            if ((long long)p.nPB * nQG * 20 < sP * sQ * 17) continue;
            const long long cost = sP * 64 * sQ * c.NT * 16;
            if (best < 0 || cost < best) { best = cost; p.lds = 1; p.NT = c.NT; p.PBW = c.PBW; p.QGW = c.QGW; p.nQG = (int)nQG; }
        }
        if (p.lds) p.QP = p.nQG * p.NT * 16;
    }
    if (p.lds) {
        const long long tiles = cdiv(p.nPB, p.PBW) * cdiv(p.nQG, p.QGW);
        long long w2 = std::max<long long>(1, g_wgrad_lds / tiles);
        w2 = std::min(w2, std::max<long long>(1, cdiv(rows, 4 * WGL_ROWS)));
        p.rpc = align_up((size_t)cdiv(rows, w2), WGL_ROWS);
        p.n_chunks = (int)cdiv(rows, p.rpc);
        p.cap = w2;
        p.gy = (int)tiles;
    }
    return p;
}
}

extern "C" {

int oard_version(void) { return OARD_VERSION; }
int oard_supported(const oard_config* cfg) { return config_ok(cfg) ? OARD_OK : OARD_EINVAL; }
size_t oard_param_count(const oard_config* cfg) { return config_ok(cfg) ? (size_t)ParamIdx(cfg).count : 0; }
size_t oard_packed_bytes(const oard_config* cfg) { return config_ok(cfg) ? make_layout(cfg).total * sizeof(float) : 0; }

int oard_pack_weights(const oard_config* c, const float* const* params, size_t n_params, void* packed,
                      size_t packed_bytes, oard_stream_t stream) {
    if (!config_ok(c) || !params || !packed) return OARD_EINVAL;
    const ParamIdx pi(c);
    if (n_params != (size_t)pi.count) return OARD_EINVAL;
    const PackOff po = make_layout(c);
    if (packed_bytes < po.total * sizeof(float)) return OARD_ENOMEM;
    const RDims d(c->hidden, c->num_radial);
    const int H = d.H, R = d.R, W = d.W, C = c->in_hidden, emb = embed_dim(c);
    hipStream_t st = (hipStream_t)stream;
    rbf_tables_forget(packed);
    HIP_TRY(hipMemsetAsync(packed, 0, po.head * sizeof(float), st));
    Packer pk{params, (float*)packed, st, {}, 0};

    pk.nat(pi.emb_w, C, 0, H, C, d.HT, 1, po.emb);          pk.vec(pi.emb_b, H, d.HP, 1, d.HP, po.emb_b);
    pk.nat(pi.nbemb_w, C, 0, H, C, d.HT, 1, po.nbemb);      pk.vec(pi.nbemb_b, H, d.HP, 1, d.HP, po.nbemb_b);
    pk.nat(pi.s2v_w, H, 0, H, H, d.HT, d.HT, po.s2v);       pk.vec(pi.s2v_b, H, d.HP, 1, d.HP, po.s2v_b);
    pk.nat(pi.rl0_w, R, 0, H, R, d.HT, d.RB, po.rl0);       pk.vec(pi.rl0_b, H, d.HP, 1, d.HP, po.rl0_b);
    pk.nat(pi.rl2_w, H, 0, H, H, d.HT, d.HT, po.rl2);       pk.vec(pi.rl2_b, H, d.HP, 1, d.HP, po.rl2_b);
    pk.raw(pi.lin30_w, d.H4 * 3, po.lin3);
    pk.raw(pi.lin30_b, d.H4, po.lin3 + d.H4 * 3);
    pk.raw(pi.lin32_w, d.H4, po.lin3 + d.H4 * 4);
    pk.raw(pi.lin32_b, 1, po.lin3 + d.H4 * 5);
    pk.raw(pi.pe0_w, d.H2 * 3, po.pe0);
    pk.nat(pi.pe1_w, d.H2, 0, H, d.H2, d.HT, d.PB, po.pe1);
    pk.nat(pi.embout_w, H, 0, C, H, 1, d.HT, po.embout);    pk.vec(pi.embout_b, C, 16, 1, 16, po.embout_b);
    pk.raw(pi.means, R, po.rbf_means);                      pk.raw(pi.betas, R, po.rbf_betas);
    const int o = pi.out0;
    pk.nat(o + 0, H, 0, H, H, d.HT, d.HT, po.v1p);
    pk.vec(o + 1, H, d.HP, 1, d.HP, po.v2p);
    pk.matrix(o + 2, 2 * H, 0, H, d.HP, 1, H, d.HP, 2, d.HT, 2 * d.HT, po.un0);   pk.vec(o + 3, H, d.HP, 1, d.HP, po.un0_b);
    pk.nat(o + 4, H, 0, 2, H, 1, d.HT, po.un2);                                  pk.vec(o + 5, 2, 16, 1, 16, po.un2_b);
    for (int k = 0; k < c->n_obj; ++k) {
        const int a = c->enc_alias[k], dd = c->node_nf[k] - 3;
        const int e = pi.enc0 + 4 * a, q = pi.dec0 + 4 * a;
        size_t off = po.enc[k];
        pk.raw(e + 0, 2 * dd * dd, off); off += 2 * dd * dd;
        pk.raw(e + 1, 2 * dd, off); off += 2 * dd;
        pk.raw(e + 2, emb * 2 * dd, off); off += emb * 2 * dd;
        pk.raw(e + 3, emb, off);
        off = po.dec[k];
        pk.raw(q + 0, 2 * dd * emb, off); off += 2 * dd * emb;
        pk.raw(q + 1, 2 * dd, off); off += 2 * dd;
        pk.raw(q + 2, dd * 2 * dd, off); off += dd * 2 * dd;
        pk.raw(q + 3, dd, off);
    }
    for (int l = 0; l < c->num_layers; ++l) {
        const LayerOff& lo = po.layer[l];
        const int g = pi.gcl0 + 14 * l;
        const int ld0 = 2 * H + W;
        pk.nat(g + 0, ld0, 0, H, H, d.HT, d.HT, lo.W1a);     pk.vec(g + 1, H, d.HP, 1, d.HP, lo.b1);
        pk.nat(g + 0, ld0, H, H, H, d.HT, d.HT, lo.W1b);
        pk.nat(g + 0, ld0, 2 * H, H, W, d.HT, d.WB, lo.W1c);
        pk.nat(g + 2, H, 0, H, H, d.HT, d.HT, lo.W2);        pk.vec(g + 3, H, d.HP, 1, d.HP, lo.b2);
        pk.matrix(g + 4, 2 * H, 0, H, d.HP, 1, H, d.HP, 2, d.HT, 2 * d.HT, lo.nm0);   pk.vec(g + 5, H, d.HP, 1, d.HP, lo.nm0b);
        pk.nat(g + 6, H, 0, H, H, d.HT, d.HT, lo.nm1);       pk.vec(g + 7, H, d.HP, 1, d.HP, lo.nm1b);
        pk.nat(g + 8, H, 0, W, H, d.WB, d.HT, lo.W3);        pk.vec(g + 9, W, d.WP, 1, d.WP, lo.b3);
        pk.vec(g + 10, H, d.HP, 1, d.HP, lo.watt);           pk.raw(g + 11, 1, lo.batt);
        pk.vec(g + 12, H, d.HP, 1, d.HP, lo.ln_g_w);         pk.vec(g + 13, H, d.HP, 1, d.HP, lo.ln_g_b);
        const int m = pi.msg0 + 9 * l;
        pk.nat(m + 0, W, 0, 3 * H, W, d.D1T, d.WB, lo.dp0);   pk.vec(m + 1, 3 * H, d.D1P, 1, d.D1P, lo.dp0b);
        pk.matrix(m + 2, 3 * H, 0, H, d.HP, 3, 3 * H, d.D1P, 1, 3 * d.HT, d.D1T, lo.dp2);
        pk.vec(m + 3, H, d.HP, 3, 3 * d.HP, lo.dp2b);
        pk.nat(m + 4, H, 0, H, H, d.HT, d.HT, lo.xp0);
        pk.matrix(m + 5, H, 0, H, d.HP, 3, H, d.HP, 1, 3 * d.HT, d.HT, lo.xp2);
        pk.matrix(m + 6, R, 0, H, d.HP, 3, R, d.RP, 1, 3 * d.HT, d.RB, lo.rbfp);
        pk.raw(m + 6, 3 * H * R, lo.rbfw);
        pk.vec(m + 7, H, d.HP, 1, d.HP, lo.ln_q_w);          pk.vec(m + 8, H, d.HP, 1, d.HP, lo.ln_q_b);
        const int u = pi.upd0 + 9 * l;
        pk.matrix(u + 0, H, 0, H, d.HP, 2, H, d.HP, 1, 2 * d.HT, d.HT, lo.vp);
        pk.matrix(u + 1, 2 * H, 0, H, d.HP, 1, H, d.HP, 2, d.HT, 2 * d.HT, lo.xv0);
        pk.matrix(u + 2, H, 0, H, d.HP, 3, H, d.HP, 1, 3 * d.HT, d.HT, lo.xv2);
        pk.raw(u + 3, 144, lo.l3u); pk.raw(u + 4, 48, lo.l3u + 144); pk.raw(u + 5, 384, lo.l3u + 192);
        pk.raw(u + 6, 8, lo.l3u + 576); pk.raw(u + 7, 8, lo.l3u + 584); pk.raw(u + 8, 1, lo.l3u + 592);
        {
            const size_t G2 = (size_t)(d.HT + 1) * 256;
            const size_t s1 = lo.gcl_stream, s2 = s1 + (size_t)d.WB * d.HT * 256, s3 = s2 + (size_t)(d.HT + 1) * G2;
            const int tc = (H % 16 >= 1 && H % 16 <= 4 && d.HT >= 3 && (d.HT & 1)) ? 1 : 0;
            pk.matrix(g + 0, ld0, 2 * H, H, d.HP, 1, W, d.WP, 1, d.HT, d.WB, s1, 256, (size_t)d.HT * 256, 0, 0, 0, tc * d.HT);
            pk.matrix(g + 2, H, 0, H, d.HP, 1, H, d.HP, 1, d.HT, d.HT, s2 + 256, G2, 256, 0, 0, tc, tc * d.HT);
            pk.bias_chunks(g + 3, H, d.HP, 1, d.HT, s2, G2);
            pk.matrix(g + 10, H, 0, 1, 16, 1, H, d.HP, 1, 1, d.HT, s2 + d.HT * G2 + 256, G2, 256, 0, 0, tc, tc);
            pk.bias_chunks(g + 11, 1, 16, 1, 1, s2 + d.HT * G2, G2);
            pk.matrix(g + 8, H, 0, W, d.WP, 1, H, d.HP, 1, d.WB, d.HT, s3 + 256, G2, 256, 0, 0, tc);
            pk.bias_chunks(g + 9, W, d.WP, 1, d.WB, s3, G2);
            const size_t GE = (size_t)(1 + d.D1T + d.RB) * 256;
            const size_t t1 = lo.equi_stream, t2 = t1 + (size_t)d.WB * d.D1T * 256;
            pk.matrix(m + 0, W, 0, 3 * H, d.D1P, 1, W, d.WP, 1, d.D1T, d.WB, t1, 256, (size_t)d.D1T * 256);
            const int r4 = (H % 16 >= 1 && H % 16 <= 4) ? d.HT : 0;
            pk.matrix(m + 2, 3 * H, 0, H, d.HP, 3, 3 * H, d.D1P, 1, 3 * d.HT, d.D1T, t2 + 256, GE, 256, d.HT, 0, 0, r4);
            pk.matrix(m + 6, R, 0, H, d.HP, 3, R, d.RP, 1, 3 * d.HT, d.RB, t2 + (size_t)(1 + d.D1T) * 256, GE, 256, d.HT, 0, 0, r4);
            pk.bias_chunks(m + 3, H, d.HP, 3, 3 * d.HT, t2, GE, d.HT);
        }
    }
    { int rcf = pk.flush(); if (rcf != OARD_OK) return rcf; }
    {
        L3tJobs lj;
        memset(&lj, 0, sizeof(lj));
        for (int l = 0; l < c->num_layers; ++l) { lj.l3u[l] = po.layer[l].l3u; lj.l3t[l] = po.layer[l].l3t; }
        hipLaunchKernelGGL(k_lin3u_table_fill, dim3(L3T_N / 256, (unsigned)c->num_layers), dim3(256), 0, st, (float*)packed, lj);
        hipLaunchKernelGGL(k_lin3u_table_check, dim3(L3T_N / 256, (unsigned)c->num_layers), dim3(256), 0, st, (float*)packed, lj);
    }
    hipLaunchKernelGGL(k_c0row, dim3((unsigned)cdiv(d.WP, 256)), dim3(256), 0, st, params[pi.lin30_b], params[pi.lin32_w],
                       params[pi.lin32_b], params[pi.rl0_b], params[pi.rl2_w], params[pi.rl2_b],
                       (float*)packed + po.c0row, H, d.H4, d.WP);
    hipLaunchKernelGGL(k_u0, dim3((unsigned)cdiv(d.HP, 64)), dim3(64), 0, st, params[pi.gcl0 + 0],
                       (const float*)packed + po.c0row, (float*)packed + po.u0, H, W, d.HP);
// ... 1283 lines not shown
    for (int p = 0; p < topo->n_parts; ++p)
        LAUNCH(F_OTHER, k_nan_replace, cdiv(topo->parts[p].d.N, 128), 128, (hipStream_t)stream, topo->parts[p].d, np, (const int*)status);
    HIP_TRY(hipGetLastError());
    return OARD_OK;
}

static LossCfg make_loss_cfg(const oard_config* c, const float* norm_values, const float* norm_biases, const float* scales, int pos_only,
                             int fixed_mask, int T) {
    LossCfg lc;
    memset(&lc, 0, sizeof(lc));
    for (int i = 0; i < 3; ++i) { lc.norm_value[i] = norm_values ? norm_values[i] : 1.0f; lc.norm_bias[i] = norm_biases ? norm_biases[i] : 0.0f; }
    for (int k = 0; k < c->n_obj; ++k) lc.scale[k] = scales ? scales[k] : 1.0f;
    lc.pos_only = pos_only; lc.fixed_mask = fixed_mask; lc.T = T;
    return lc;
}
int oard_loss_prepare(const oard_config* c, const oard_topology* topo, const float* const* pos, const int64_t* const* one_hot,
                      const int64_t* const* charge, const float* const* noise, const float* t_int, const float* gamma, int T,
                      const float* norm_values, const float* norm_biases, int pos_only, int fixed_mask, float* const* z,
                      float* const* eps, oard_stream_t stream) {
    topo_touch(topo, (hipStream_t)stream);
    if (!config_ok(c) || !topo || topo->n_parts != 1 || !pos || !one_hot || !charge || !noise || !t_int || !gamma || !z || !eps)
        return OARD_EINVAL;
    LossPtrs lp;
    memset(&lp, 0, sizeof(lp));
    for (int k = 0; k < c->n_obj; ++k) {
        if (c->node_nf[k] < 5 || c->node_nf[k] - 4 > 16) return OARD_EINVAL;
        lp.pos[k] = pos[k]; lp.one_hot[k] = (const long long*)one_hot[k]; lp.charge[k] = (const long long*)charge[k];
        lp.noise[k] = noise[k]; lp.z[k] = z[k]; lp.eps[k] = eps[k]; lp.node_nf[k] = c->node_nf[k];
    }
    const TopoDev& tp = topo->parts[0].d;
    LAUNCH(F_OTHER, k_loss_prep, cdiv(tp.N, 128), 128, (hipStream_t)stream, tp, lp,
           make_loss_cfg(c, norm_values, norm_biases, nullptr, pos_only, fixed_mask, T), t_int, gamma);
    HIP_TRY(hipGetLastError());
    return OARD_OK;
}
int oard_loss_terms(const oard_config* c, const oard_topology* topo, const float* const* eps, const float* const* net,
                    const float* const* z, const int64_t* const* one_hot, const int64_t* const* charge, const float* t_int,
                    const float* gamma, int T, const float* norm_values, const float* norm_biases, const float* scales, int pos_only,
                    int B, float* nll, float* terms, float* const* dnet, oard_stream_t stream) {
    topo_touch(topo, (hipStream_t)stream);
    if (!config_ok(c) || !topo || topo->n_parts != 1 || !eps || !net || !z || !one_hot || !charge || !t_int || !gamma || !nll || !terms ||
        !dnet || B < 1)
        return OARD_EINVAL;
    LossPtrs lp;
    memset(&lp, 0, sizeof(lp));
    for (int k = 0; k < c->n_obj; ++k) {
        if (c->node_nf[k] < 5 || c->node_nf[k] - 4 > 16) return OARD_EINVAL;
        lp.eps[k] = (float*)eps[k]; lp.net[k] = net[k]; lp.z[k] = (float*)z[k]; lp.one_hot[k] = (const long long*)one_hot[k];
        lp.charge[k] = (const long long*)charge[k]; lp.dnet[k] = dnet[k]; lp.node_nf[k] = c->node_nf[k];
    }
    const TopoDev& tp = topo->parts[0].d;
    LAUNCH(F_OTHER, k_loss_terms, tp.B, 64, (hipStream_t)stream, tp, lp, make_loss_cfg(c, norm_values, norm_biases, scales, pos_only, 0, T),
           t_int, gamma, B, nll, terms);
    HIP_TRY(hipGetLastError());
    return OARD_OK;
}
static bool loss_eval_args_ok(const oard_config* c, const oard_topology* topo, int T) {
    if (!c || !topo || T <= 0) return false;
    if (c->n_obj < 1 || c->n_obj > OARD_MAX_OBJECTS) return false;
    for (int k = 0; k < c->n_obj; ++k)
        if (c->node_nf[k] < 5 || c->node_nf[k] - 4 > 16) return false;
    return config_ok(c) && topo->n_parts == 1 && c->n_obj == topo->n_obj;
}
int oard_loss_eval_prepare(const oard_config* c, const oard_topology* topo, const float* const* pos, const int64_t* const* one_hot,
                           const int64_t* const* charge, const float* const* noise_t, const float* const* noise_0, const float* t_int,
                           const float* gamma, int T, const float* norm_values, const float* norm_biases, int pos_only, int fixed_mask,
                           float* const* z_t, float* const* eps_t, float* const* z_0, float* const* eps_0, oard_stream_t stream) {
    if (!pos || !one_hot || !charge || !noise_t || !noise_0 || !t_int || !gamma || !z_t || !eps_t || !z_0 || !eps_0) return OARD_EINVAL;
    if (!loss_eval_args_ok(c, topo, T)) return OARD_EINVAL;
    topo_touch(topo, (hipStream_t)stream);
    EvalPrepPtrs ep;
    memset(&ep, 0, sizeof(ep));
    for (int k = 0; k < c->n_obj; ++k) {
        ep.pos[k] = pos[k]; ep.one_hot[k] = (const long long*)one_hot[k]; ep.charge[k] = (const long long*)charge[k];
        ep.noise_t[k] = noise_t[k]; ep.noise_0[k] = noise_0[k]; ep.z_t[k] = z_t[k]; ep.eps_t[k] = eps_t[k]; ep.z_0[k] = z_0[k];
        ep.eps_0[k] = eps_0[k]; ep.node_nf[k] = c->node_nf[k];
    }
    const TopoDev& tp = topo->parts[0].d;
    LAUNCH(F_OTHER, k_eval_prep, cdiv(tp.N, 128), 128, (hipStream_t)stream, tp, ep,
           make_loss_cfg(c, norm_values, norm_biases, nullptr, pos_only, fixed_mask, T), t_int, gamma);
    HIP_TRY(hipGetLastError());
    return OARD_OK;
}
int oard_loss_eval_terms(const oard_config* c, const oard_topology* topo, const float* const* eps_t, const float* const* net_t,
                         const float* const* eps_0, const float* const* net_0, const float* const* z_0, const int64_t* const* one_hot,
                         const int64_t* const* charge, const float* t_int, const float* gamma, const float* snr, int T,
                         const float* norm_values, const float* norm_biases, const float* scales, int pos_only, double delta_log_px, int B,
                         float* nll, float* terms, oard_stream_t stream) {
    if (!eps_t || !net_t || !eps_0 || !net_0 || !z_0 || !one_hot || !charge || !t_int || !gamma || !snr || !nll || !terms || B < 1)
        return OARD_EINVAL;
    if (!loss_eval_args_ok(c, topo, T)) return OARD_EINVAL;
    topo_touch(topo, (hipStream_t)stream);
    VlbPtrs vp;
    memset(&vp, 0, sizeof(vp));
    for (int k = 0; k < c->n_obj; ++k) {
        vp.eps_t[k] = eps_t[k]; vp.net_t[k] = net_t[k]; vp.eps_0[k] = eps_0[k]; vp.net_0[k] = net_0[k]; vp.z_0[k] = z_0[k];
        vp.one_hot[k] = (const long long*)one_hot[k]; vp.charge[k] = (const long long*)charge[k]; vp.node_nf[k] = c->node_nf[k];
    }
    const TopoDev& tp = topo->parts[0].d;
    LAUNCH(F_OTHER, k_vlb_terms, tp.B, 64, (hipStream_t)stream, tp, vp, make_loss_cfg(c, norm_values, norm_biases, scales, pos_only, 0, T),
           t_int, gamma, snr, delta_log_px, B, nll, terms);
    HIP_TRY(hipGetLastError());
    return OARD_OK;
}
static bool ema_args_ok(const float* ema, double ema_decay) { return ema && ema_decay >= 0.0 && ema_decay <= 1.0; }

struct AdamwCall { float* p; const float* g; float *m, *v, *vmax; int64_t n; int amsgrad; bool with_ema; float* ema; double ema_decay; };

static bool adamw_call_ok(const AdamwCall& c) {
    return c.p && c.g && c.m && c.v && (!c.amsgrad || c.vmax) && c.n >= 0 && (!c.with_ema || ema_args_ok(c.ema, c.ema_decay));
}

static void adamw_launch(const AdamwCall& c, const AdamScal& host, const AdamScal* dev, hipStream_t stream) {
    auto kern = dev ? (c.with_ema ? k_adamw<true, true> : k_adamw<true, false>) : (c.with_ema ? k_adamw<false, true> : k_adamw<false, false>);
    LAUNCH(F_OTHER, kern, cdiv(c.n, 256), 256, stream, c.p, c.g, c.m, c.v, c.vmax, (long long)c.n, c.amsgrad, host, dev, c.ema,
           (float)c.ema_decay, (float)(1.0 - c.ema_decay));
}

static int adamw_host_step(const AdamwCall& c, double lr, double beta1, double beta2, double eps, double weight_decay, int64_t step,
                           double grad_scale, oard_stream_t stream) {
    if (!adamw_call_ok(c) || step < 1) return OARD_EINVAL;
    if (c.n == 0) return OARD_OK;
    const double bc1 = 1.0 - pow(beta1, (double)step), bc2 = 1.0 - pow(beta2, (double)step);
    AdamScal sc = {};
    sc.decay = (float)(1.0 - lr * weight_decay); sc.w1 = (float)(1.0 - beta1); sc.beta2 = (float)beta2; sc.w2 = (float)(1.0 - beta2);
    sc.eps = (float)eps; sc.step_size = (float)(lr / bc1); sc.inv_bc2s = (float)(1.0 / sqrt(bc2)); sc.gscale = (float)grad_scale;
    adamw_launch(c, sc, nullptr, (hipStream_t)stream);
    HIP_TRY(hipGetLastError());
    return OARD_OK;
}

static int adamw_dev_step(const AdamwCall& c, double lr, double beta1, double beta2, double eps, double weight_decay, int clip,
                          double* clip_state, int capacity, const float* grad_norm, const float* flag, float* out4, oard_stream_t stream) {
    if (!adamw_call_ok(c) || !clip_state || capacity < 1 || capacity > 64 || !grad_norm || !flag || !out4) return OARD_EINVAL;
    LAUNCH(F_OTHER, k_clip_decide, 1, 64, (hipStream_t)stream, clip_state, capacity, grad_norm, flag, clip, lr, beta1, beta2, eps, weight_decay, out4);
    if (c.n > 0) adamw_launch(c, AdamScal{}, reinterpret_cast<const AdamScal*>(clip_state + 4 + capacity), (hipStream_t)stream);
    HIP_TRY(hipGetLastError());
    return OARD_OK;
}

int oard_adamw_step(float* param, const float* grad, float* exp_avg, float* exp_avg_sq, float* max_exp_avg_sq, int64_t n, double lr,
                    double beta1, double beta2, double eps, double weight_decay, int64_t step, int amsgrad, double grad_scale,
                    oard_stream_t stream) {
    return adamw_host_step({param, grad, exp_avg, exp_avg_sq, max_exp_avg_sq, n, amsgrad, false, nullptr, 0.0}, lr, beta1, beta2, eps,
                           weight_decay, step, grad_scale, stream);
}
int oard_adamw_step_ema(float* param, const float* grad, float* exp_avg, float* exp_avg_sq, float* max_exp_avg_sq, int64_t n, double lr,
                        double beta1, double beta2, double eps, double weight_decay, int64_t step, int amsgrad, double grad_scale,
                        float* ema, double ema_decay, oard_stream_t stream) {
    return adamw_host_step({param, grad, exp_avg, exp_avg_sq, max_exp_avg_sq, n, amsgrad, true, ema, ema_decay}, lr, beta1, beta2, eps,
                           weight_decay, step, grad_scale, stream);
}
int oard_adamw_step_dev(float* param, const float* grad, float* exp_avg, float* exp_avg_sq, float* max_exp_avg_sq, int64_t n, double lr,
                        double beta1, double beta2, double eps, double weight_decay, int amsgrad, int clip, double* clip_state,
                        int capacity, const float* grad_norm, const float* flag, float* out4, oard_stream_t stream) {
    return adamw_dev_step({param, grad, exp_avg, exp_avg_sq, max_exp_avg_sq, n, amsgrad, false, nullptr, 0.0}, lr, beta1, beta2, eps,
                          weight_decay, clip, clip_state, capacity, grad_norm, flag, out4, stream);
}
int oard_adamw_step_dev_ema(float* param, const float* grad, float* exp_avg, float* exp_avg_sq, float* max_exp_avg_sq, int64_t n, double lr,
                            double beta1, double beta2, double eps, double weight_decay, int amsgrad, int clip, double* clip_state,
                            int capacity, const float* grad_norm, const float* flag, float* out4, float* ema, double ema_decay,
                            oard_stream_t stream) {
    return adamw_dev_step({param, grad, exp_avg, exp_avg_sq, max_exp_avg_sq, n, amsgrad, true, ema, ema_decay}, lr, beta1, beta2, eps,
                          weight_decay, clip, clip_state, capacity, grad_norm, flag, out4, stream);
}

int oard_ema_update(float* ema, const float* param, int64_t n, double ema_decay, oard_stream_t stream) {
    if (!param || n < 0 || !ema_args_ok(ema, ema_decay)) return OARD_EINVAL;
    if (n == 0) return OARD_OK;
    LAUNCH(F_OTHER, k_ema_update, cdiv(n, 256), 256, (hipStream_t)stream, ema, param, (long long)n, (float)ema_decay, (float)(1.0 - ema_decay));
    HIP_TRY(hipGetLastError());
    return OARD_OK;
}

int oard_kabsch_rmsd(const float* a, int64_t lda, const float* b, int64_t ldb, const int32_t* seg_ptr, int64_t n_segments, int flags,
                     float cap, float* rmsd, float* rot, float* aligned, oard_stream_t stream) {
    if (!a || !b || !seg_ptr || !rmsd || n_segments < 0 || n_segments > 0x7fffffffLL || lda < 3 || ldb < 3) return OARD_EINVAL;
    if (n_segments == 0) return OARD_OK;
    LAUNCH(F_OTHER, k_kabsch_rmsd, n_segments, 64, (hipStream_t)stream, a, (long long)lda, b, (long long)ldb, seg_ptr, flags, cap, rmsd, rot,
           aligned);
    HIP_TRY(hipGetLastError());
    return OARD_OK;
}

int oard_matched_rmsd(const float* a, int64_t lda, const float* b, int64_t ldb, const int32_t* species_a, const int32_t* species_b,
                      const int32_t* seg_ptr, int64_t n_segments, int flags, float cap, int exact_limit, float* rmsd, float* rot,
                      float* aligned, int32_t* perm, int32_t* status, oard_stream_t stream) {
    if (!a || !b || !species_a || !seg_ptr || !rmsd || n_segments < 0 || n_segments > 0x7fffffffLL || lda < 3 || ldb < 3 ||
        exact_limit < 0 || exact_limit > MATCH_LIMIT)
        return OARD_EINVAL;
    if (n_segments == 0) return OARD_OK;
    LAUNCH(F_OTHER, k_matched_rmsd, n_segments, 64, (hipStream_t)stream, a, (long long)lda, b, (long long)ldb, species_a, species_b, seg_ptr,
           flags, cap, exact_limit, rmsd, rot, aligned, perm, status);
    HIP_TRY(hipGetLastError());
    return OARD_OK;
}

int oard_rank_metrics(const float* score, const float* target, int64_t n, const int32_t* seg_ptr, int64_t n_segments, double* rank_score,
                      double* rank_target, double* out, oard_stream_t stream) {
    if (n < 0 || n > 0x7fffffffLL || n_segments < 0 || n_segments >= 0x7fffffffLL || (!rank_score && !rank_target && !out)) return OARD_EINVAL;
    if (n_segments > 0 && (!score || !target || !seg_ptr)) return OARD_EINVAL;
    if (n_segments == 0) return OARD_OK;
    if ((rank_score || rank_target) && n > 0) {
        LAUNCH(F_OTHER, k_rank_count, cdiv(n, RANK_ROWS), RANK_BLOCK, (hipStream_t)stream, score, target, (int)n, seg_ptr, (int)n_segments,
               rank_score, rank_target);
        HIP_TRY(hipGetLastError());
    }
    if (out) {
        LAUNCH(F_OTHER, k_rank_stats, n_segments, 64, (hipStream_t)stream, score, target, (int)n, seg_ptr, (const double*)rank_score,
               (const double*)rank_target, out);
        HIP_TRY(hipGetLastError());
    }
    return OARD_OK;
}

int oard_dataset_gather(const oard_reaction_store* s, const int64_t* index, const int64_t* const* epoch_off, int64_t first, int64_t B,
                        int64_t* const* size, float* const* pos, int64_t* const* one_hot, int64_t* const* charge, int64_t* const* mask,
                        int64_t* condition, int64_t* target, float* rmsd, float* ediff, oard_stream_t stream) {
    if (!s || !index || !epoch_off || !size || !pos || !one_hot || !charge || !mask || !condition) return OARD_EINVAL;
    if ((s->n_obj != 1 && s->n_obj != OARD_STORE_OBJECTS) || s->n_raw < 1 || s->n_sel < 1 || !s->sel) return OARD_EINVAL;
    if (first < 0 || B < 0 || first >= 0x7fffffffLL || B >= 0x7fffffffLL || first + B >= 0x7fffffffLL || B * s->n_obj >= 0x7fffffffLL) return OARD_EINVAL;
    for (int flag : {s->swap, s->reflect, s->center, s->zero_charge, s->append_frag}) if (flag != 0 && flag != 1) return OARD_EINVAL;
    if (s->n_sel > s->n_raw) return OARD_EINVAL;
    if ((target != nullptr) != (s->target != nullptr) || (rmsd != nullptr) != (s->rmsd != nullptr)) return OARD_EINVAL;
    if ((ediff != nullptr) != (s->ediff[0] != nullptr) || (s->ediff[0] != nullptr) != (s->ediff[1] != nullptr)) return OARD_EINVAL;
    DatasetOut o = {};
    for (int k = 0; k < s->n_obj; ++k) {
        const int src = s->src_obj[k];
        if (src < 0 || src >= OARD_STORE_OBJECTS || (s->reflect_obj[k] != 0 && s->reflect_obj[k] != 1)) return OARD_EINVAL;
        for (int q : {src, s->swap ? 2 - src : src}) if (!s->offsets[q] || !s->pos[q] || !s->z[q]) return OARD_EINVAL;
        if (!epoch_off[k] || !size[k] || !pos[k] || !one_hot[k] || !charge[k] || !mask[k]) return OARD_EINVAL;
        o.size[k] = (long long*)size[k]; o.pos[k] = pos[k]; o.one_hot[k] = (long long*)one_hot[k]; o.charge[k] = (long long*)charge[k];
        o.mask[k] = (long long*)mask[k]; o.epoch_off[k] = (const long long*)epoch_off[k];
    }
    o.condition = (long long*)condition; o.target = (long long*)target; o.rmsd = rmsd; o.ediff = ediff;
    if (B == 0) return OARD_OK;
    LAUNCH(F_OTHER, k_reaction_gather, cdiv(B * s->n_obj, DATASET_WAVES), DATASET_WAVES * 64, (hipStream_t)stream, *s, (const long long*)index,
           (long long)first, (long long)B, o);
    HIP_TRY(hipGetLastError());
    return OARD_OK;
}

int oard_train_scratch_entry(const oard_config* c, const oard_topology* topo, int which, size_t* offset_bytes, int64_t* rows,
                             int64_t* row_floats) {
    if (!config_ok(c) || !topo || topo->n_parts != 1 || !offset_bytes || !rows || !row_floats) return OARD_EINVAL;
    const TopoDev& d = topo->parts[0].d;
    const TrainWs w = make_train_ws(c, d);
    const RDims r(c->hidden, c->num_radial);
    switch (which) {
        case OARD_SCRATCH_XH: *offset_bytes = w.xh; *rows = d.N; *row_floats = r.HP; break;
        case OARD_SCRATCH_XQ: *offset_bytes = w.xq; *rows = d.N; *row_floats = 3 * r.HP; break;
        case OARD_SCRATCH_CR: *offset_bytes = w.cr; *rows = d.A + 1; *row_floats = 3 * r.HP; break;
        case OARD_SCRATCH_DCD: *offset_bytes = w.dcd; *rows = d.A + 1; *row_floats = 3 * r.HP; break;
        case OARD_SCRATCH_DCR: *offset_bytes = w.dcr; *rows = d.A + 1; *row_floats = 3 * r.HP; break;
        default: return OARD_EINVAL;
    }
    return OARD_OK;
}

int oard_tap(const oard_config* c, const oard_topology* topo, const void* ws_, int which, int layer, float* dst,
             oard_stream_t stream) {
    topo_touch(topo, (hipStream_t)stream);
    if (!config_ok(c) || !topo || !ws_ || !dst || layer != 0) return OARD_EINVAL;
    const RDims d(c->hidden, c->num_radial);
    ws_total(c, topo);
    hipStream_t st = (hipStream_t)stream;
    for (int p = 0; p < topo->n_parts; ++p) {
        const TopoDev& tp = topo->parts[p].d;
        const WsOff w = make_ws(c, tp);
        const char* ws = (const char*)ws_ + topo->parts[p].ws_off;
        auto nodes = [&](const float* src, int ld, int sections, int sect_pad, int sect_len) {
            const long long tot = (long long)tp.N * sections * sect_len;
            hipLaunchKernelGGL(k_tap_nodes, dim3((unsigned)cdiv(tot, 256)), dim3(256), 0, st, tp, src, ld, sections, sect_pad, sect_len, dst);
        };
        switch (which) {
            case OARD_TAP_S: nodes((const float*)(ws + w.s), d.HP, 1, d.HP, d.H); break;
            case OARD_TAP_VEC: nodes((const float*)(ws + topo->parts[p].vec_final), 3 * d.HP, 3, d.HP, d.H); break;
            case OARD_TAP_NE1: nodes((const float*)(ws + w.ne1), 3 * d.HP, 3, d.HP, d.H); break;
            case OARD_TAP_POS_FRAME: nodes((const float*)(ws + w.pf32), 3, 1, 3, 3); break;
            case OARD_TAP_DPOS: nodes((const float*)(ws + w.dpos), 3, 1, 3, 3); break;
            case OARD_TAP_HOUT: nodes((const float*)(ws + w.hout), 16, 1, 16, c->in_hidden); break;
            case OARD_TAP_LABELS:
                hipLaunchKernelGGL(k_tap_labels, dim3((unsigned)cdiv(tp.N, 256)), dim3(256), 0, st, tp, (const int*)(ws + w.labels), dst);
                break;
            case OARD_TAP_EDGE:
                if (tp.E > 0)
                    hipLaunchKernelGGL(k_tap_edges, dim3((unsigned)cdiv(tp.E * d.W, 256)), dim3(256), 0, st, tp,
                                       (const float*)(ws + w.ew), d.WP, d.W, dst);
                break;
            default: return OARD_EINVAL;
        }
    }
    HIP_TRY(hipGetLastError());
    return OARD_OK;
}

int oard_debug_stop_after(int code) { g_stop_after = code; return OARD_OK; }
int oard_debug_option(const char* name, int value) {
    if (!name) return OARD_EINVAL;
    static const struct { const char* name; int* value; } table[] = {
        {"gcl_variant", &g_fwd.gcl_variant}, {"equi_variant", &g_fwd.equi_variant}, {"node_variant", &g_fwd.node_variant},
        {"auto_small", &g_fwd.auto_small}, {"auto_tiny", &g_fwd.auto_tiny}, {"small_split", &g_fwd.small_split},
        {"gcl_persist", &g_fwd.gcl_persist}, {"gcl_grid", &g_fwd.gcl_grid}, {"gcl_skip", &g_fwd.gcl_skip}, {"equi_skip", &g_fwd.equi_skip},
        {"equi_l0_skip", &g_fwd.equi_l0_skip}, {"gcl_msum", &g_fwd.gcl_msum}, {"equi_rbf_table", &g_fwd.equi_rbf_table},
        {"skip_families", &g_skip_families}, {"parts", &g_parts}, {"sequential", &g_sequential}, {"poison", &g_poison}, {"npb", &g_npb},
        {"wgrad_wgs", &g_wgrad_wgs}, {"wgrad_t16", &g_wgrad_t16}, {"wgrad_queue", &g_wgrad_queue}, {"gate_fold", &g_gate_fold},
        {"wgrad_lds", &g_wgrad_lds}, {"wgrad_shapes", &g_wgrad_shapes}, {"train_dual", &g_train_dual}};
    if (strcmp(name, "experiments") == 0) return kV0 ? OARD_OK : OARD_EINVAL;
    if (strcmp(name, "gcl_msum_taken") == 0) return g_gcl_msum_taken ? OARD_OK : OARD_EINVAL;
    if (strcmp(name, "equi_rbf_taken") == 0) return g_equi_rbf_taken ? OARD_OK : OARD_EINVAL;
    if (strcmp(name, "equi_l0_taken") == 0) return g_equi_l0_taken ? OARD_OK : OARD_EINVAL;
    for (const auto& e : table) {
        if (strcmp(name, e.name) != 0) continue;
        if (!kV0 && value == 0 && strstr(name, "_variant")) return OARD_EINVAL;
        *e.value = e.value == &g_wgrad_shapes ? value & 3 : value;
        return OARD_OK;
    }
    return OARD_EINVAL;
}
#ifdef OARD_PHASE_PROBE
int oard_debug_probe_read(unsigned long long* out8) {
    if (!out8) return OARD_EINVAL;
    HIP_TRY(hipDeviceSynchronize());
    HIP_TRY(hipMemcpyFromSymbol(out8, HIP_SYMBOL(g_phase_probe), 8 * sizeof(unsigned long long)));
    unsigned long long z[8] = {};
    HIP_TRY(hipMemcpyToSymbol(HIP_SYMBOL(g_phase_probe), z, sizeof(z)));
    return OARD_OK;
}
#endif
#ifdef OARD_TIMELINE
int oard_debug_timeline_read(long long* out, int waves) {
    if (!out || waves < 1 || waves > 16) return OARD_EINVAL;
    HIP_TRY(hipDeviceSynchronize());
    HIP_TRY(hipMemcpyFromSymbol(out, HIP_SYMBOL(g_timeline), (size_t)waves * TL_MAX * sizeof(long long)));
    return OARD_OK;
}
#endif
#ifdef OARD_EXPERIMENTS
int oard_debug_fp_timeouts(unsigned int* out) {
    if (!out) return OARD_EINVAL;
    HIP_TRY(hipDeviceSynchronize());
    HIP_TRY(hipMemcpyFromSymbol(out, HIP_SYMBOL(g_fp_timeouts), sizeof(unsigned int)));
    return OARD_OK;
}
#endif
int oard_timing_enable(int on) { g_timing.on = on != 0; return OARD_OK; }
int oard_timing_reset(void) {
    g_timing.flush();
    for (int f = 0; f < F_COUNT; ++f) { g_timing.total_ms[f] = 0; g_timing.launches[f] = 0; }
    return OARD_OK;
}
int oard_timing_get(const char* family, double* total_ms, int64_t* launches) {
    if (!family || !total_ms || !launches) return OARD_EINVAL;
    g_timing.flush();
    for (int f = 0; f < F_COUNT; ++f)
        if (strcmp(family, kFamilyNames[f]) == 0) { *total_ms = g_timing.total_ms[f]; *launches = g_timing.launches[f]; return OARD_OK; }
    return OARD_EINVAL;
}

}
```

oareactdiff_amd/csrc/oard_inst.h:

```cpp
#pragma once
#if !defined(OARD_EXPERIMENTS) && !defined(OARD_SINGLE_TU)

#define OARD_UNPAREN(...) __VA_ARGS__
#ifdef OARD_INST_DEFINE
#define OARD_INST(K, ARGS) template __global__ void OARD_UNPAREN K ARGS;
#else
#define OARD_INST(K, ARGS) extern template __global__ void OARD_UNPAREN K ARGS;
#endif
#ifndef OARD_DIMS_LIST
#define OARD_DIMS_LIST X(196, 96) X(32, 8) X(32, 32)
#endif
#define OARD_BOOL4(M, D) M(D, true, true) M(D, false, true) M(D, true, false) M(D, false, false)

#define OARD_NW(h) (((h) + 15) / 16 <= 16 ? ((h) + 15) / 16 : 8)
#define OARD_A_GCL (TopoDev, const float*, const float*, const float*, const float*, const float*, long long, long long, const float*, float*, float*, GclTape)

#if !defined(OARD_INST_DEFINE) || defined(OARD_INST_UNIT_GCL_P)
#define OARD_I_GCL_P(D, S1, S3) OARD_INST((k_gcl_edge_p<OARD_UNPAREN D, S1, S3, false>), OARD_A_GCL) OARD_INST((k_gcl_edge_p<OARD_UNPAREN D, S1, S3, true>), OARD_A_GCL) \
    OARD_INST((k_gcl_edge_p<OARD_UNPAREN D, S1, S3, false, true>), OARD_A_GCL)
#define X(h, r) OARD_BOOL4(OARD_I_GCL_P, (Dims<h, r>))
OARD_DIMS_LIST
#undef X
#endif

#if !defined(OARD_INST_DEFINE) || defined(OARD_INST_UNIT_GCL_V1)
#define OARD_I_GCL_V1(D, S1, S3) \
    OARD_INST((k_gcl_edge_v1<OARD_UNPAREN D, 8, 2, S1, S3, false, false, 2, 3>), OARD_A_GCL) OARD_INST((k_gcl_edge_v1<OARD_UNPAREN D, 8, 2, S1, S3, true, false, 2, 3>), OARD_A_GCL) \
    OARD_INST((k_gcl_edge_v1<OARD_UNPAREN D, 8, 2, S1, S3, false, true, 2, 3>), OARD_A_GCL) \
    OARD_INST((k_gcl_edge_v1<OARD_UNPAREN D, 4, 2, S1, S3, false, false, 2, 2>), OARD_A_GCL) \
    OARD_INST((k_gcl_edge_small<OARD_UNPAREN D, 8, S1, S3>), (TopoDev, const float*, LayerOff, const float*, const float*, const float*, const float*, long long, long long, float*, float*))
#define X(h, r) OARD_BOOL4(OARD_I_GCL_V1, (Dims<h, r>))
OARD_DIMS_LIST
#undef X
#endif

#if !defined(OARD_INST_DEFINE) || defined(OARD_INST_UNIT_B3)
#define OARD_A_EQUI_B3 (TopoDev, const float*, const float*, const float*, const float*, const float*, float*, float*, float*, float*, ActList)
#define OARD_I_GCL_B3(D, S1, S3) OARD_INST((k_gcl_edge_b3<OARD_UNPAREN D, S1, S3, false>), OARD_A_GCL) OARD_INST((k_gcl_edge_b3<OARD_UNPAREN D, S1, S3, true>), OARD_A_GCL)
#define X(h, r) OARD_BOOL4(OARD_I_GCL_B3, (Dims<h, r>)) OARD_INST((k_equi_edge_b3<Dims<h, r>, false>), OARD_A_EQUI_B3) OARD_INST((k_equi_edge_b3<Dims<h, r>, true>), OARD_A_EQUI_B3)
OARD_DIMS_LIST
#undef X
#endif

#if !defined(OARD_INST_DEFINE) || defined(OARD_INST_UNIT_EQUI)
#define OARD_A_EQUI (TopoDev, const float*, const float*, const float*, const float*, float*, float*, float*, ActList, int, const float*)
#define OARD_A_EQUI_NODE (TopoDev, const float*, LayerOff, const float*, const float*, const float*, const float*, const float*, float*, const float*, float*, float*, float*, ActList)
#define X(h, r) \
    OARD_INST((k_equi_edge_v1<Dims<h, r>, 8, false>), OARD_A_EQUI) OARD_INST((k_equi_edge_v1<Dims<h, r>, 8, true>), OARD_A_EQUI) \
    OARD_INST((k_equi_edge_v1<Dims<h, r>, 4, false>), OARD_A_EQUI) OARD_INST((k_equi_edge_v1<Dims<h, r>, 8, false, true>), OARD_A_EQUI) \
    OARD_INST((k_equi_node_v1<Dims<h, r>, OARD_NW(h), false, false>), OARD_A_EQUI_NODE) OARD_INST((k_equi_node_v1<Dims<h, r>, OARD_NW(h), false, true>), OARD_A_EQUI_NODE) \
    OARD_INST((k_equi_node_v1<Dims<h, r>, OARD_NW(h), true, false>), OARD_A_EQUI_NODE) OARD_INST((k_equi_node_v1<Dims<h, r>, OARD_NW(h), true, true>), OARD_A_EQUI_NODE) \
    OARD_INST((k_equi_node_v1<Layer0<Dims<h, r> >, OARD_NW(h), false, false>), OARD_A_EQUI_NODE) OARD_INST((k_equi_node_v1<Layer0<Dims<h, r> >, OARD_NW(h), false, true>), OARD_A_EQUI_NODE) \
    OARD_INST((k_gcl_edge_bwd<Dims<h, r>, 8, 2, true>), (TopoDev, const float*, long long, long long, GclBwdArgs)) \
    OARD_INST((k_gcl_edge_bwd<Dims<h, r>, 8, 2, false>), (TopoDev, const float*, long long, long long, GclBwdArgs)) \
    OARD_INST((k_equi_edge_bwd<Dims<h, r>, 8>), (TopoDev, const float*, const float*, const float*, float*, float*))
OARD_DIMS_LIST
#undef X
#endif

#if !defined(OARD_INST_DEFINE) || defined(OARD_INST_UNIT_NODE)
#define OARD_A_GCL_NODE (TopoDev, const float*, LayerOff, const float*, const float*, float*, float*, float*)
#define OARD_A_OUT (TopoDev, const float*, PackOff, const float*, const float*, float*, float*, int*)
#define OARD_A_SCAL_BWD (TopoDev, const float*, const float*, int, const float*, const float*, float*, float*)
#define OARD_A_MSG_BWD (TopoDev, const float*, Strided3, Strided3, const float*, Strided3, const float*, int, Strided3, float*, float*, float*, float*, int, int, int)
#define X(h, r) \
    OARD_INST((k_gcl_node_v1<Dims<h, r>, OARD_NW(h), false>), OARD_A_GCL_NODE) OARD_INST((k_gcl_node_v1<Dims<h, r>, OARD_NW(h), true>), OARD_A_GCL_NODE) \
    OARD_INST((k_gcl_node_v1<Dims<h, r>, OARD_NW(h), false, true>), OARD_A_GCL_NODE) \
    OARD_INST((k_out_v1<Dims<h, r>, OARD_NW(h)>), OARD_A_OUT) \
    OARD_INST((k_scalarize_bwd<Dims<h, r>, 2, false>), OARD_A_SCAL_BWD) OARD_INST((k_scalarize_bwd<Dims<h, r>, 2, true>), OARD_A_SCAL_BWD) \
    OARD_INST((k_equi_msg_bwd<Dims<h, r> >), OARD_A_MSG_BWD)
OARD_DIMS_LIST
#undef X
OARD_INST((k_lin3u_bwd_fused<4>), (const float*, const float*, const float*, long long, float*, float*))
#define OARD_I_ROWS(KB, EPI) OARD_INST((k_rows_dense<KB, EPI, 8>), (RowsDense)) OARD_INST((k_rows_dense_long<KB, EPI, 8, 4>), (RowsDense))
OARD_I_ROWS(13, 0) OARD_I_ROWS(13, 2) OARD_I_ROWS(13, 3) OARD_I_ROWS(7, 3) OARD_I_ROWS(6, 0) OARD_I_ROWS(6, 1) OARD_I_ROWS(4, 1) OARD_I_ROWS(4, 3)
OARD_INST((k_rows_dense<26, 1, 8>), (RowsDense)) OARD_INST((k_rows_dense<26, 3, 8>), (RowsDense))
OARD_INST((k_rows_dense2<13, 1, 8, 13>), (RowsDense2)) OARD_INST((k_rows_dense2<13, 2, 8, 13>), (RowsDense2))
OARD_INST((k_rows_dense2<26, 1, 8, 13>), (RowsDense2)) OARD_INST((k_rows_dense2<39, 2, 8, 13>), (RowsDense2))
#endif

#if !defined(OARD_INST_DEFINE) || defined(OARD_INST_UNIT_WGRAD)
#define OARD_A_WG (const float*, int, int, const float*, int, int, long long, long long, long long, int, int, float*, float*, float*)
OARD_INST((k_wgrad_t16<4, 7, false>), (WgtArgs)) OARD_INST((k_wgrad_t16<4, 7, true>), (WgtArgs)) OARD_INST((k_wgrad_t16<5, 3, false>), (WgtArgs))
OARD_INST((k_wgrad_t16<5, 5, true>), (WgtArgs)) OARD_INST((k_wgrad_t16<5, 7, true>), (WgtArgs)) OARD_INST((k_wgrad_t16<6, 5, false>), (WgtArgs))
OARD_INST((k_wgrad_t16<6, 7, false>), (WgtArgs))
OARD_INST((k_wgrad<false, 7>), OARD_A_WG) OARD_INST((k_wgrad<false, 8>), OARD_A_WG) OARD_INST((k_wgrad<true, 7>), OARD_A_WG) OARD_INST((k_wgrad<true, 8>), OARD_A_WG)
OARD_INST((k_wgrad_lds<false, 7, 4, 2>), OARD_A_WG) OARD_INST((k_wgrad_lds<false, 8, 4, 2>), OARD_A_WG)
OARD_INST((k_wgrad_lds<true, 7, 4, 2>), OARD_A_WG) OARD_INST((k_wgrad_lds<true, 8, 4, 2>), OARD_A_WG)
#endif

#endif
```

oareactdiff_amd/csrc/oard_layout.h:

```cpp
#pragma once
#include <hip/hip_runtime.h>
#include <stdint.h>
#include <stddef.h>
#include "../../include/oard.h"

#define OARD_MAX_LAYERS 16
#define OARD_MAX_GROUP 1024

template <int H_, int R_>
struct Dims {
    static constexpr int H = H_, R = R_;
    static constexpr int HT = (H + 15) / 16, HP = HT * 16;
    static constexpr int W = 3 * H + R, WB = (W + 15) / 16, WP = WB * 16;
    static constexpr int RB = (R + 15) / 16, RP = RB * 16;
    static constexpr int H2 = H / 2, PB = (H2 + 15) / 16, PP = PB * 16;
    static constexpr int D1T = (3 * H + 15) / 16, D1P = D1T * 16;
    static constexpr int H4 = H / 4;
    static_assert(H % 4 == 0 && R % 4 == 0, "feature widths must be multiples of 4");
};

struct RDims {
    int H, R, HT, HP, W, WB, WP, RB, RP, H2, PB, PP, D1T, D1P, H4;
    explicit RDims(int h, int r) {
        H = h; R = r; HT = (H + 15) / 16; HP = HT * 16; W = 3 * H + R; WB = (W + 15) / 16; WP = WB * 16;
        RB = (R + 15) / 16; RP = RB * 16; H2 = H / 2; PB = (H2 + 15) / 16; PP = PB * 16;
        D1T = (3 * H + 15) / 16; D1P = D1T * 16; H4 = H / 4;
    }
};

#define L3T_X 16.0f
#define L3T_H 0.03125f
#define L3T_N 1024
#define L3T_FLOATS (2 * (L3T_N + 1) + 4)

struct LayerOff {
    size_t ln_g_w, ln_g_b, W1a, b1, W1b, W1c, W2, b2, watt, batt, W3, b3, nm0, nm0b, nm1, nm1b;
    size_t ln_q_w, ln_q_b, xp0, xp2, dp0, dp0b, dp2, dp2b, rbfp;
    size_t rbfw, rbff, rbft;
    size_t vp, xv0, xv2, l3u;
    size_t l3t;
    size_t gcl_stream, equi_stream;
    size_t gcl_b3, equi_b3;
    int xcross;
};
struct PackOff {
    size_t emb, emb_b, nbemb, nbemb_b, s2v, s2v_b, rl0, rl0_b, rl2, rl2_b;
    size_t lin3;
    size_t pe0;
    size_t pe1, embout, embout_b, v1p, v2p, un0, un0_b, un2, un2_b;
    size_t c0row;
    size_t u0;
    size_t rbf_means, rbf_betas;
    size_t enc[OARD_MAX_OBJECTS], dec[OARD_MAX_OBJECTS];
    LayerOff layer[OARD_MAX_LAYERS];
    size_t head;
    size_t total;
    int signed_scal;
};

struct TopoDev {
    int N, B, n_obj, n_groups;
    int npb;
    long long E, A;
    const int *node_obj, *node_row, *node_ref, *node_tidx, *node_sample, *sample_ptr;
    const int *edge_ptr, *edge_src, *edge_tgt;
    const int *edge_row;
    const int *row_src, *row_tgt;
    const int *row_eid;
    const int *grp_ptr;
    const int *act_ptr, *act_src, *act_tgt, *act_edge;
    const long long *ref_edge_ptr;
    long long CI, CX;
    const int *col_info;
    const int *node_cols;
};

struct ActList {
    const int* rows;
    const int* src;
    const int* pre;
    const int* n;
};

#define OARD_MAX_PARTS 8
struct TopoPart {
    TopoDev d;
    void* dev_block = nullptr;
    size_t dev_cap = 0;
    void* stage = nullptr;
    size_t stage_cap = 0;
    size_t ws_off = 0;
    int conc = 1;
    mutable size_t vec_final = 0;
};
struct oard_topology {
    int device = 0;
    int n_parts = 0;
    TopoPart parts[OARD_MAX_PARTS];
    int n_obj = 0, B = 0;
    bool ids_dense = false;
    long long N = 0, E = 0, A = 0;
    int max_group = 0, max_ns = 0;
    int obj_start[OARD_MAX_OBJECTS + 1] = {};
    hipStream_t side[OARD_MAX_PARTS] = {};
    hipEvent_t ev_fork = nullptr, ev_join[OARD_MAX_PARTS] = {};
    void* ref_block = nullptr;
    size_t ref_cap = 0;
    void* ref_stage = nullptr;
    size_t ref_stage_cap = 0;
    hipEvent_t ready = nullptr;
    mutable hipStream_t used_on[4] = {};
    mutable int n_used = 0;
    mutable bool used_many = false;
    const int *ref_sample = nullptr, *ref_rank = nullptr;
    const long long* ref_ptr = nullptr;
    int N_ref = 0;
};

struct WsOff {
    size_t pos, pf64, pf32, x1, pp0, labels, hin, zemb, nb, s, s1, ne1, xh, P, Q, xq, vec, vec2, v2buf, sc0, vdot,
        geo, d64, rbuf, ew, mbuf, xmsg, vmsg, dpos, hout, total;
    size_t al_rows, al_src, al_pre, al_cnt, al_n;
    size_t rbt;
    size_t d1s;
    size_t small_a;
};
```

oareactdiff_amd/csrc/oard_node_v1.h:

```cpp
#pragma once
#include "oard_kernels.h"

OARD_DEV f4 lds_blk(const float* v, int b, int lane) { return *reinterpret_cast<const f4*>(v + b * 256 + lane * 4); }
OARD_DEV void lds_st(float* v, int t, int lane, f4 x) { *reinterpret_cast<f4*>(v + t * 256 + lane * 4) = x; }

#ifndef OARD_NODE_PF
#define OARD_NODE_PF 13
#endif
template <int KB>
OARD_DEV f4 dense_tile_lds(const float* __restrict__ wp, int t, const float* in, int lane, f4 init) {
    const float* base = wp + ((size_t)t * KB * 64 + lane) * 4;
    f4 c0 = init, c1 = f4zero();
    constexpr int G = OARD_NODE_PF;
#pragma unroll
    for (int b0 = 0; b0 < KB; b0 += G) {
        f4 a[G];
#pragma unroll
        for (int i = 0; i < G; ++i)
            if (b0 + i < KB) a[i] = ld_f4(base + (size_t)(b0 + i) * 256);
        __builtin_amdgcn_sched_barrier(0);
#pragma unroll
        for (int i = 0; i < G; ++i)
            if (b0 + i < KB) {
                const f4 x = lds_blk(in, b0 + i, lane);
// ... 146 lines not shown
        const f4 x = lds_blk(v, t, lane);
        const int f0 = 16 * t + 4 * g;
        const float dx = x.x - mean, dy = x.y - mean, dz = x.z - mean, dw = x.w - mean;
        q += (f0 + 0 < H ? dx * dx : 0.f) + (f0 + 1 < H ? dy * dy : 0.f) + (f0 + 2 < H ? dz * dz : 0.f) +
             (f0 + 3 < H ? dw * dw : 0.f);
    }
    rstd = 1.0f / sqrtf(col_reduce(q) * (1.0f / H) + 1e-5f);
}
template <int H>
OARD_DEV f4 ln_apply(f4 x, float mean, float rstd, const float* gamma, const float* beta, int t, int lane) {
    const int f0 = 16 * t + 4 * (lane >> 4);
    f4 y = (x - mean) * rstd * ld_vec(gamma, t, lane) + ld_vec(beta, t, lane);
    y.x = f0 + 0 < H ? y.x : 0.f; y.y = f0 + 1 < H ? y.y : 0.f; y.z = f0 + 2 < H ? y.z : 0.f; y.w = f0 + 3 < H ? y.w : 0.f;
    return y;
}

struct NodeBlk {
    int lane, wave, g, n;
    bool valid;
};
OARD_DEV NodeBlk node_blk(int N, int npb) {
    NodeBlk b;
    b.lane = threadIdx.x & 63; b.wave = threadIdx.x >> 6; b.g = b.lane >> 4;
    const int c = blockIdx.x * npb + (b.lane & 15);
    b.valid = (b.lane & 15) < npb && c < N;
    b.n = b.valid ? c : N - 1;
    return b;
}

struct RowLanes {
    int L, npb, node, slot;
    bool live;
};
OARD_DEV RowLanes row_lanes(int N, int npb, int lane) {
    RowLanes r;
    r.L = npb == 1 ? 16 : (npb == 2 ? 8 : 4); r.npb = npb;
    const int e = lane & 15;
    r.node = e / r.L; r.slot = e % r.L;
    r.live = r.node < npb && blockIdx.x * npb + r.node < N;
    return r;
}
OARD_DEV float rows_total(float x, const RowLanes& r, int lane) {
    for (int d = 1; d < r.L; d <<= 1) x += __shfl_xor(x, d, 64);
    const int e = lane & 15;
    return __shfl(x, (lane & 48) | ((e < r.npb ? e : 0) * r.L), 64);
}
OARD_DEV f4 rows_total4(f4 v, const RowLanes& r, int lane) {
    return (f4){rows_total(v.x, r, lane), rows_total(v.y, r, lane), rows_total(v.z, r, lane), rows_total(v.w, r, lane)};
}

template <class D, int WAVES>
__global__ __launch_bounds__(WAVES * 64) void k_node_pre_v1(TopoDev tp, const float* __restrict__ wb, PackOff po,
                                                            LayerOff lo, const float* __restrict__ s,
                                                            const float* __restrict__ pp0, float* __restrict__ xh,
                                                            float* __restrict__ P, float* __restrict__ Q) {
    __shared__ __attribute__((aligned(16))) float sm[(D::PB + 2 * D::HT) * 256];
    float* hid = sm;
    float* sv = sm + D::PB * 256;
    float* xv = sv + D::HT * 256;
    const NodeBlk nb = node_blk(tp.N, tp.npb);
    const float pp = pp0[nb.n];
    for (int b = nb.wave; b < D::PB; b += WAVES) {
        const int k0 = 16 * b + 4 * nb.g;
        const float* w = wb + po.pe0;
        f4 h;
        h.x = k0 + 0 < D::H2 ? silu1(w[(k0 + 0) * 3] * pp) : 0.f;
        h.y = k0 + 1 < D::H2 ? silu1(w[(k0 + 1) * 3] * pp) : 0.f;
        h.z = k0 + 2 < D::H2 ? silu1(w[(k0 + 2) * 3] * pp) : 0.f;
        h.w = k0 + 3 < D::H2 ? silu1(w[(k0 + 3) * 3] * pp) : 0.f;
        lds_st(hid, b, nb.lane, h);
    }
    __syncthreads();
    constexpr int TPW = (D::HT + WAVES - 1) / WAVES, TPW2 = (2 * D::HT + WAVES - 1) / WAVES;
    {
        TileJob job[TPW];
        f4 acc[TPW];
#pragma unroll
        for (int i = 0; i < TPW; ++i) {
            const int t = min(nb.wave + i * WAVES, D::HT - 1);
            job[i] = tile_job<D::PB>(wb + po.pe1, t, hid);
            acc[i] = f4zero();
        }
        dense_seq<D::PB, TPW, OARD_NODE_PRE_G>(job, nb.lane, acc);
#pragma unroll
        for (int i = 0; i < TPW; ++i)
            if (nb.wave + i * WAVES < D::HT)
                lds_st(sv, nb.wave + i * WAVES, nb.lane, ld_blk(s, nb.n, D::HP, nb.wave + i * WAVES, nb.lane) + acc[i]);
    }
    __syncthreads();
    float mean, rstd;
    ln_stats_lds<D::HT, D::H>(sv, nb.lane, mean, rstd);
    for (int t = nb.wave; t < D::HT; t += WAVES) {
        const f4 y = ln_apply<D::H>(lds_blk(sv, t, nb.lane), mean, rstd, wb + lo.ln_g_w, wb + lo.ln_g_b, t, nb.lane);
        lds_st(xv, t, nb.lane, y);
        if (nb.valid) st_blk(xh, nb.n, D::HP, t, nb.lane, y);
    }
    __syncthreads();
    {
        TileJob job[TPW2];
        f4 acc[TPW2];
#pragma unroll
        for (int i = 0; i < TPW2; ++i) {
            const int t = min(nb.wave + i * WAVES, 2 * D::HT - 1);
            job[i] = t < D::HT ? tile_job<D::HT>(wb + lo.W1a, t, xv) : tile_job<D::HT>(wb + lo.W1b, t - D::HT, xv);
            acc[i] = t < D::HT ? ld_vec(wb + lo.b1, t, nb.lane) : f4zero();
        }
        dense_seq<D::HT, TPW2, OARD_NODE_PRE_G>(job, nb.lane, acc);
#pragma unroll
        for (int i = 0; i < TPW2; ++i) {
            const int t = nb.wave + i * WAVES;
            if (t < 2 * D::HT && nb.valid) {
                if (t < D::HT) st_blk(P, nb.n, D::HP, t, nb.lane, acc[i]);
                else st_blk(Q, nb.n, D::HP, t - D::HT, nb.lane, acc[i]);
            }
        }
    }
}

template <class D, int WAVES, bool ROWS = false, bool MSUM = false>
__global__ __launch_bounds__(WAVES * 64) void k_gcl_node_v1(TopoDev tp, const float* __restrict__ wb, LayerOff lo,
                                                            const float* __restrict__ xh, const float* __restrict__ mbuf,
                                                            float* __restrict__ s, float* __restrict__ xq,
                                                            float* __restrict__ agg_out ) {
    static_assert(!(MSUM && ROWS), "the partial sums exist for the large-batch gather only");
    __shared__ __attribute__((aligned(16))) float sm[4 * D::HT * 256];
    float* in = sm;
    float* hm = sm + 2 * D::HT * 256;
    float* sv = sm + 3 * D::HT * 256;
    const NodeBlk nb = node_blk(tp.N, tp.npb);
    const int smp = tp.node_sample[nb.n];
    const int deg = nb.valid ? tp.sample_ptr[smp + 1] - tp.sample_ptr[smp] - 1 : 0;
    const size_t e0 = (size_t)tp.edge_ptr[nb.n];
    const int mx = wave_max(deg);
    const float inv = 1.0f / (float)max(deg, 1);
    int in_lo = 0, x_lo = 0, n_in = 0, cnt = 0;
    if (MSUM) {
        const int* nc = tp.node_cols + 4 * (size_t)nb.n;
        const int in_hi = nc[1], x_hi = nc[3];
        in_lo = nc[0]; x_lo = nc[2];
        n_in = (nb.valid && in_hi > in_lo) ? 1 + ((in_hi - 1) >> 4) - (in_lo >> 4) : 0;
        cnt = n_in + ((nb.valid && x_hi > x_lo) ? 1 + ((x_hi - 1) >> 4) - (x_lo >> 4) : 0);
    }
    auto pc = [&](int k) -> size_t {
        const int lo = k < n_in ? in_lo : x_lo, j = k < n_in ? k : k - n_in;
        return (size_t)(j == 0 ? lo : ((lo >> 4) + j) << 4);
    };
    const int mxp = MSUM ? wave_max(cnt) : 0;
    for (int t = nb.wave; t < D::HT; t += WAVES) {
        lds_st(in, t, nb.lane, ld_blk(xh, nb.n, D::HP, t, nb.lane));
        f4 a0 = f4zero(), a1 = f4zero();
        if (ROWS) {
            const RowLanes rl = row_lanes(tp.N, tp.npb, nb.lane);
            const int nn = min(blockIdx.x * tp.npb + rl.node, tp.N - 1);
            const int smp2 = tp.node_sample[nn];
            const int deg2 = rl.live ? tp.sample_ptr[smp2 + 1] - tp.sample_ptr[smp2] - 1 : 0;
            const size_t e2 = (size_t)tp.edge_ptr[nn];
            const int mx2 = wave_max(deg2), last2 = max(deg2 - 1, 0);
            for (int k = 0; k < mx2; k += 2 * rl.L) {
                const int k0 = k + rl.slot, k1 = k0 + rl.L;
                const f4 r0 = ld_blk(mbuf, e2 + min(k0, last2), D::HP, t, nb.lane), r1 = ld_blk(mbuf, e2 + min(k1, last2), D::HP, t, nb.lane);
                if (k0 < deg2) a0 += r0;
                if (k1 < deg2) a1 += r1;
            }
            a0 = rows_total4(a0 + a1, rl, nb.lane);
            a1 = f4zero();
        }
        const int last = max(deg - 1, 0);
        for (int k = 0; MSUM && k < mxp; k += 8) {
            f4 r[8];
#pragma unroll
            for (int i = 0; i < 8; ++i) r[i] = ld_blk(mbuf, pc(min(k + i, max(cnt - 1, 0))), D::HP, t, nb.lane);
#pragma unroll
            for (int i = 0; i < 8; ++i) {
                const f4 v = k + i < cnt ? r[i] : f4zero();
                if (i & 1) a1 += v; else a0 += v;
            }
        }
        for (int k = 0; !ROWS && !MSUM && k < mx; k += 8) {
            f4 r[8];
#pragma unroll
            for (int i = 0; i < 8; ++i) r[i] = ld_blk(mbuf, e0 + min(k + i, last), D::HP, t, nb.lane);
#pragma unroll
            for (int i = 0; i < 8; ++i) {
                const f4 v = k + i < deg ? r[i] : f4zero();
                if (i & 1) a1 += v; else a0 += v;
            }
        }
        lds_st(in, D::HT + t, nb.lane, (a0 + a1) * inv);
        if (agg_out != nullptr && nb.valid) st_blk(agg_out, nb.n, D::HP, t, nb.lane, (a0 + a1) * inv);
    }
    __syncthreads();
    constexpr int TPW = (D::HT + WAVES - 1) / WAVES, TPW3 = (3 * D::HT + WAVES - 1) / WAVES;
    int tw[TPW];
#pragma unroll
    for (int i = 0; i < TPW; ++i) tw[i] = min(nb.wave + i * WAVES, D::HT - 1);
    {
        TileJob job[TPW];
        f4 acc[TPW];
#pragma unroll
        for (int i = 0; i < TPW; ++i) { job[i] = tile_job<2 * D::HT>(wb + lo.nm0, tw[i], in); acc[i] = ld_vec(wb + lo.nm0b, tw[i], nb.lane); }
        dense_seq<2 * D::HT, TPW, OARD_GCL_NODE_G>(job, nb.lane, acc);
#pragma unroll
        for (int i = 0; i < TPW; ++i)
            if (nb.wave + i * WAVES < D::HT) lds_st(hm, tw[i], nb.lane, silu4(acc[i]));
    }
    __syncthreads();
    {
        TileJob job[TPW];
        f4 acc[TPW];
#pragma unroll
        for (int i = 0; i < TPW; ++i) { job[i] = tile_job<D::HT>(wb + lo.nm1, tw[i], hm); acc[i] = ld_vec(wb + lo.nm1b, tw[i], nb.lane); }
        dense_seq<D::HT, TPW, OARD_GCL_NODE_G>(job, nb.lane, acc);
#pragma unroll
        for (int i = 0; i < TPW; ++i)
            if (nb.wave + i * WAVES < D::HT) {
                const f4 v = lds_blk(in, tw[i], nb.lane) + acc[i];
                lds_st(sv, tw[i], nb.lane, v);
                if (nb.valid) st_blk(s, nb.n, D::HP, tw[i], nb.lane, v);
            }
    }
    __syncthreads();
    float mean, rstd;
    ln_stats_lds<D::HT, D::H>(sv, nb.lane, mean, rstd);
    float* xln = in;
    float* hq = in + D::HT * 256;
    for (int t = nb.wave; t < D::HT; t += WAVES)
        lds_st(xln, t, nb.lane, ln_apply<D::H>(lds_blk(sv, t, nb.lane), mean, rstd, wb + lo.ln_q_w, wb + lo.ln_q_b, t, nb.lane));
    __syncthreads();
    {
        TileJob job[TPW];
        f4 acc[TPW];
#pragma unroll
        for (int i = 0; i < TPW; ++i) { job[i] = tile_job<D::HT>(wb + lo.xp0, tw[i], xln); acc[i] = f4zero(); }
        dense_seq<D::HT, TPW, OARD_GCL_NODE_G>(job, nb.lane, acc);
#pragma unroll
        for (int i = 0; i < TPW; ++i)
            if (nb.wave + i * WAVES < D::HT) lds_st(hq, tw[i], nb.lane, silu4(acc[i]));
    }
    __syncthreads();
    {
        TileJob job[TPW3];
        f4 acc[TPW3];
#pragma unroll
        for (int i = 0; i < TPW3; ++i) {
            job[i] = tile_job<D::HT>(wb + lo.xp2, min(nb.wave + i * WAVES, 3 * D::HT - 1), hq);
            acc[i] = f4zero();
        }
        dense_seq<D::HT, TPW3, OARD_GCL_NODE_G>(job, nb.lane, acc);
#pragma unroll
        for (int i = 0; i < TPW3; ++i)
            if (nb.wave + i * WAVES < 3 * D::HT && nb.valid) st_blk(xq, nb.n, 3 * D::HP, nb.wave + i * WAVES, nb.lane, acc[i]);
    }
}

OARD_DEV void lin3u_stage(const float* __restrict__ p, float* l3s, int tid, int nthreads) {
    for (int i = tid; i < 48 * 12; i += nthreads) {
        const int k = i / 12, j = i % 12;
        l3s[i] = j < 8 ? p[192 + j * 48 + k] : (j == 8 ? p[3 * k] : (j == 9 ? p[144 + k] : 0.f));
    }
}
OARD_DEV f4 lin3u4(const float* l3s, const float* __restrict__ p, f4 x) {
    const float* b2 = p + 576;
    const float* w4 = p + 584;
    f4 h2[8];
#pragma unroll
    for (int j = 0; j < 8; ++j) h2[j] = (f4){b2[j], b2[j], b2[j], b2[j]};
#pragma unroll 4
    for (int k = 0; k < 48; ++k) {
        const f4 wa = *reinterpret_cast<const f4*>(l3s + 12 * k), wc = *reinterpret_cast<const f4*>(l3s + 12 * k + 4);
        const float w0 = l3s[12 * k + 8], b0 = l3s[12 * k + 9];
        const f4 h = silu4(x * w0 + b0);
        h2[0] += h * wa.x; h2[1] += h * wa.y; h2[2] += h * wa.z; h2[3] += h * wa.w;
        h2[4] += h * wc.x; h2[5] += h * wc.y; h2[6] += h * wc.z; h2[7] += h * wc.w;
    }
    const float b4 = p[592];
    f4 o = (f4){b4, b4, b4, b4};
#pragma unroll
    for (int j = 0; j < 8; ++j) o += silu4(h2[j]) * w4[j];
    return o;
}

OARD_DEV float lin3u1(const float* l3s, const float* __restrict__ p, float x) {
    const float* b2 = p + 576;
    const float* w4 = p + 584;
    float h2[8];
#pragma unroll
    for (int j = 0; j < 8; ++j) h2[j] = b2[j];
#pragma unroll 4
    for (int k = 0; k < 48; ++k) {
        const f4 wa = *reinterpret_cast<const f4*>(l3s + 12 * k), wc = *reinterpret_cast<const f4*>(l3s + 12 * k + 4);
        const float h = silu1(x * l3s[12 * k + 8] + l3s[12 * k + 9]);
        h2[0] += h * wa.x; h2[1] += h * wa.y; h2[2] += h * wa.z; h2[3] += h * wa.w;
        h2[4] += h * wc.x; h2[5] += h * wc.y; h2[6] += h * wc.z; h2[7] += h * wc.w;
    }
    float o = p[592];
#pragma unroll
    for (int j = 0; j < 8; ++j) o += silu1(h2[j]) * w4[j];
    return o;
}

template <class D> struct Layer0 : D {};
template <class D> struct is_layer0 { static constexpr bool value = false; };
template <class D> struct is_layer0<Layer0<D> > { static constexpr bool value = true; };
template <class D, int WAVES, bool ROWS = false, bool XC = false>
__global__ __launch_bounds__(WAVES * 64) void k_equi_node_v1(TopoDev tp, const float* __restrict__ wb, LayerOff lo,
                                                             const float* __restrict__ qbuf, const float* __restrict__ xq,
                                                             const float* __restrict__ geo, const float* __restrict__ x1,
                                                             const float* s, float* s_out, const float* __restrict__ vec_in,
                                                             float* __restrict__ vec_out,
                                                             float* __restrict__ sa_out, float* __restrict__ va_out ,
                                                             ActList al ) {
    constexpr bool L0 = is_layer0<D>::value;
    static_assert(!(L0 && ROWS), "the layer-0 form exists for the large-batch gather only");
    constexpr int HT = D::HT;
    constexpr int TPW = (HT + WAVES - 1) / WAVES;
    __shared__ __attribute__((aligned(16))) float sm[6 * HT * 256 + 48 * 12 + L3T_FLOATS];
    float* l3s = sm + 6 * HT * 256;
    float* l3t = l3s + 48 * 12;
#ifdef OARD_NO_L3T
    const bool l3t_ok = false;
#else
    const bool l3t_ok = tp.npb > 4 && (wb + lo.l3t)[2 * (L3T_N + 1)] > 0.5f;
#endif
    if (l3t_ok)
        for (int i = threadIdx.x; i < 2 * (L3T_N + 1) / 4; i += WAVES * 64)
            reinterpret_cast<f4*>(l3t)[i] = ld_f4(wb + lo.l3t + 4 * i);
    if (l3t_ok && threadIdx.x < 2) l3t[2 * (L3T_N + 1) - 2 + threadIdx.x] = (wb + lo.l3t)[2 * (L3T_N + 1) - 2 + threadIdx.x];
#ifdef OARD_TIMELINE
    const bool tl_on_ = blockIdx.x == gridDim.x / 2 && (threadIdx.x & 63) == 0; int tl_n_ = 0;
#endif
    TL(1);
    lin3u_stage(wb + lo.l3u, l3s, threadIdx.x, WAVES * 64);
    float* vx = sm;
    float* in = sm + 3 * HT * 256;
    float* hx = sm + 5 * HT * 256;
    const NodeBlk nb = node_blk(tp.N, tp.npb);
    const int n = nb.n;
    const bool listed = al.pre != nullptr && (long long)__builtin_amdgcn_readfirstlane(*al.n) != tp.A;
    const int a0 = listed ? al.pre[tp.act_ptr[n]] : tp.act_ptr[n];
    const int cnt = nb.valid ? (listed ? al.pre[tp.act_ptr[n + 1]] : tp.act_ptr[n + 1]) - a0 : 0;
    const int mx = wave_max(cnt);
    auto row_of = [&](int k) -> int { return listed ? al.rows[k] : k; };
    auto src_of = [&](int k) -> int { return listed ? al.src[k] : tp.act_src[k]; };
    const float inv_sqrt2 = 0.70710678118654752f, inv_sqrt3 = 0.57735026918962576f,
                inv_sqrt_h = 1.0f / sqrtf((float)D::H);

    for (int t = nb.wave; t < HT; t += WAVES) {
        f4 dx = f4zero(), v0 = f4zero(), v1 = f4zero(), v2 = f4zero();
        const f4 xn0 = ld_blk(xq, n, 3 * D::HP, t, nb.lane), xn1 = ld_blk(xq, n, 3 * D::HP, HT + t, nb.lane),
                 xn2 = ld_blk(xq, n, 3 * D::HP, 2 * HT + t, nb.lane);
        const int a_hi = (int)max(tp.A - 1, 0LL);
        if (ROWS) {
            const RowLanes rl = row_lanes(tp.N, tp.npb, nb.lane);
            const int nn = min(blockIdx.x * tp.npb + rl.node, tp.N - 1);
            const int b0 = listed ? al.pre[tp.act_ptr[nn]] : tp.act_ptr[nn];
            const int cnt2 = rl.live ? (listed ? al.pre[tp.act_ptr[nn + 1]] : tp.act_ptr[nn + 1]) - b0 : 0;
            const int mx2 = wave_max(cnt2);
            const f4 zn0 = ld_blk(xq, nn, 3 * D::HP, t, nb.lane), zn1 = ld_blk(xq, nn, 3 * D::HP, HT + t, nb.lane),
                     zn2 = ld_blk(xq, nn, 3 * D::HP, 2 * HT + t, nb.lane);
            for (int k = 0; k < mx2; k += rl.L) {
                const int kk = k + rl.slot;
                const int ke = min(b0 + min(kk, max(cnt2 - 1, 0)), a_hi);
                const size_t a = cnt2 > 0 ? (size_t)row_of(ke) : 0;
                const int m = cnt2 > 0 ? src_of(ke) : 0;
                const float* gp = geo + a * GEO_STRIDE;
                const float gx = gp[2], gy = gp[3], gz = gp[4];
                const float cx = XC ? gp[5] : 0.f, cy = XC ? gp[6] : 0.f, cz = XC ? gp[7] : 0.f;
                const f4 q0 = ld_blk(qbuf, a, 3 * D::HP, t, nb.lane), q1 = ld_blk(qbuf, a, 3 * D::HP, HT + t, nb.lane),
                         q2 = ld_blk(qbuf, a, 3 * D::HP, 2 * HT + t, nb.lane);
                const f4 y0 = ld_blk(xq, m, 3 * D::HP, t, nb.lane), y1 = ld_blk(xq, m, 3 * D::HP, HT + t, nb.lane),
                         y2 = ld_blk(xq, m, 3 * D::HP, 2 * HT + t, nb.lane);
                const f4 w0 = ld_blk(vec_in, (size_t)m * 3 + 0, D::HP, t, nb.lane), w1 = ld_blk(vec_in, (size_t)m * 3 + 1, D::HP, t, nb.lane),
                         w2 = ld_blk(vec_in, (size_t)m * 3 + 2, D::HP, t, nb.lane);
                if (kk < cnt2) {
                    const f4 xm = (y0 + zn0) * q0;
                    dx += xm;
                    const f4 a2 = (y1 + zn1) * q1 * inv_sqrt3;
                    const f4 a3 = (y2 + zn2) * q2;
                    v0 += (XC ? w0 * a2 + a3 * gx + xm * cx : w0 * a2 + a3 * gx) * inv_sqrt_h;
                    v1 += (XC ? w1 * a2 + a3 * gy + xm * cy : w1 * a2 + a3 * gy) * inv_sqrt_h;
                    v2 += (XC ? w2 * a2 + a3 * gz + xm * cz : w2 * a2 + a3 * gz) * inv_sqrt_h;
                }
            }
            dx = rows_total4(dx, rl, nb.lane); v0 = rows_total4(v0, rl, nb.lane);
            v1 = rows_total4(v1, rl, nb.lane); v2 = rows_total4(v2, rl, nb.lane);
        }
        int mnext[2], rnext[2];
        auto entry = [&](int kk, int& m, int& r) {
            const int ke = min(a0 + min(kk, max(cnt - 1, 0)), a_hi);
            m = cnt > 0 ? src_of(ke) : 0;
            r = cnt > 0 ? row_of(ke) : 0;
        };
#pragma unroll
        for (int i = 0; i < 2; ++i) entry(i, mnext[i], rnext[i]);
        float zero1 = 0.f;
        if (L0) asm volatile("" : "+v"(zero1));
        const f4 zero4 = {zero1, zero1, zero1, zero1};
        for (int k = 0; !ROWS && k < mx; k += 2) {
            f4 q0[2], q1[2], q2[2], y0[2], y1[2], y2[2], w0[2], w1[2], w2[2];
            float gx[2], gy[2], gz[2], cx[2], cy[2], cz[2];
            const int mc[2] = {mnext[0], mnext[1]}, rc[2] = {rnext[0], rnext[1]};
#pragma unroll
            for (int i = 0; i < 2; ++i)
                entry(k + 2 + i, mnext[i], rnext[i]);
#pragma unroll
            for (int i = 0; i < 2; ++i) {
                const size_t a = (size_t)rc[i];
                const int m = mc[i];
                const float* g = geo + a * GEO_STRIDE;
                gx[i] = g[2]; gy[i] = g[3]; gz[i] = g[4];
                cx[i] = XC ? g[5] : 0.f; cy[i] = XC ? g[6] : 0.f; cz[i] = XC ? g[7] : 0.f;
                q0[i] = ld_blk(qbuf, a, 3 * D::HP, t, nb.lane); q1[i] = L0 ? zero4 : ld_blk(qbuf, a, 3 * D::HP, HT + t, nb.lane);
                q2[i] = ld_blk(qbuf, a, 3 * D::HP, 2 * HT + t, nb.lane);
                y0[i] = ld_blk(xq, m, 3 * D::HP, t, nb.lane); y1[i] = L0 ? zero4 : ld_blk(xq, m, 3 * D::HP, HT + t, nb.lane);
                y2[i] = ld_blk(xq, m, 3 * D::HP, 2 * HT + t, nb.lane);
                w0[i] = L0 ? zero4 : ld_blk(vec_in, (size_t)m * 3 + 0, D::HP, t, nb.lane);
                w1[i] = L0 ? zero4 : ld_blk(vec_in, (size_t)m * 3 + 1, D::HP, t, nb.lane);
                w2[i] = L0 ? zero4 : ld_blk(vec_in, (size_t)m * 3 + 2, D::HP, t, nb.lane);
            }
#pragma unroll
            for (int i = 0; i < 2; ++i)
                if (k + i < cnt) {
                    const f4 xm = (y0[i] + xn0) * q0[i];
                    dx += xm;
                    const f4 a2 = (y1[i] + xn1) * q1[i] * inv_sqrt3;
                    const f4 a3 = (y2[i] + xn2) * q2[i];
                    v0 += (XC ? w0[i] * a2 + a3 * gx[i] + xm * cx[i] : w0[i] * a2 + a3 * gx[i]) * inv_sqrt_h;
                    v1 += (XC ? w1[i] * a2 + a3 * gy[i] + xm * cy[i] : w1[i] * a2 + a3 * gy[i]) * inv_sqrt_h;
                    v2 += (XC ? w2[i] * a2 + a3 * gz[i] + xm * cz[i] : w2[i] * a2 + a3 * gz[i]) * inv_sqrt_h;
                }
        }
        const f4 sa = (ld_blk(s, n, D::HP, t, nb.lane) + dx) * inv_sqrt2;
        v0 += ld_blk(vec_in, (size_t)n * 3 + 0, D::HP, t, nb.lane);
        v1 += ld_blk(vec_in, (size_t)n * 3 + 1, D::HP, t, nb.lane);
        v2 += ld_blk(vec_in, (size_t)n * 3 + 2, D::HP, t, nb.lane);
        lds_st(in, t, nb.lane, sa);
        lds_st(vx + 0 * HT * 256, t, nb.lane, v0);
        lds_st(vx + 1 * HT * 256, t, nb.lane, v1);
        lds_st(vx + 2 * HT * 256, t, nb.lane, v2);
        if (sa_out != nullptr && nb.valid) {
            st_blk(sa_out, n, D::HP, t, nb.lane, sa);
            st_blk(va_out, (size_t)n * 3 + 0, D::HP, t, nb.lane, v0);
            st_blk(va_out, (size_t)n * 3 + 1, D::HP, t, nb.lane, v1);
            st_blk(va_out, (size_t)n * 3 + 2, D::HP, t, nb.lane, v2);
        }
    }
    TL(2);
    __syncthreads();
    TL(3);

    const float fx = x1[n * 3], fy = x1[n * 3 + 1], fz = x1[n * 3 + 2];
    const float* l3 = wb + lo.l3u;
    f4 v2k[TPW][3], vdk[TPW];
#pragma unroll
    for (int i = 0; i < TPW; ++i) {
        const int t = nb.wave + i * WAVES;
        if (t < HT) {
            TileJob job[2] = {tile_job<HT>(wb + lo.vp, t, vx), tile_job<HT>(wb + lo.vp, HT + t, vx)};
            f4 acc[6];
#pragma unroll
            for (int k = 0; k < 6; ++k) acc[k] = f4zero();
            dense_seq_xyz<HT, 2, HT * 256, (ROWS ? 5 : OARD_NODE_SEQ_G), ROWS>(job, nb.lane, acc);
            const f4 v1[3] = {acc[0], acc[1], acc[2]}, v2[3] = {acc[3], acc[4], acc[5]};
#pragma unroll
            for (int x = 0; x < 3; ++x) v2k[i][x] = v2[x];
            const f4 sc = v1[0] * fx + v1[1] * fy + v1[2] * fz;
            vdk[i] = (v1[0] * v2[0] + v1[1] * v2[1] + v1[2] * v2[2]) * inv_sqrt_h;
            f4 sca;
            const int f0 = 16 * t + 4 * nb.g;
            if (tp.npb <= 4) {
                float* blk = in + (HT + t) * 256;
                lds_st(in, HT + t, nb.lane, sc);
                __builtin_amdgcn_wave_barrier();
                const int f = nb.lane >> 2, c = nb.lane & 3;
                float* cell = blk + (16 * (f >> 2) + c) * 4 + (f & 3);
                const float y = (c < tp.npb && 16 * t + f < D::H) ? lin3u1(l3s, l3, *cell) : 0.f;
                *cell = y;
            } else {
                const bool in_tab = fabsf(sc.x) < L3T_X && fabsf(sc.y) < L3T_X && fabsf(sc.z) < L3T_X && fabsf(sc.w) < L3T_X;
                if (l3t_ok && !__any(!in_tab))
                    sca = (f4){lin3u_table_eval(l3t, sc.x), lin3u_table_eval(l3t, sc.y), lin3u_table_eval(l3t, sc.z), lin3u_table_eval(l3t, sc.w)};
                else
                    sca = lin3u4(l3s, l3, sc);
                sca.x = f0 + 0 < D::H ? sca.x : 0.f; sca.y = f0 + 1 < D::H ? sca.y : 0.f;
                sca.z = f0 + 2 < D::H ? sca.z : 0.f; sca.w = f0 + 3 < D::H ? sca.w : 0.f;
                lds_st(in, HT + t, nb.lane, sca);
            }
        }
    }
    TL(4);
    __syncthreads();
    TL(5);

    {
        TileJob job[TPW];
        f4 acc[TPW];
#pragma unroll
        for (int i = 0; i < TPW; ++i) { job[i] = tile_job<2 * HT>(wb + lo.xv0, min(nb.wave + i * WAVES, HT - 1), in); acc[i] = f4zero(); }
        dense_seq<2 * HT, TPW>(job, nb.lane, acc);
#pragma unroll
        for (int i = 0; i < TPW; ++i)
            if (nb.wave + i * WAVES < HT) lds_st(hx, nb.wave + i * WAVES, nb.lane, silu4(acc[i]));
    }
    TL(6);
    __syncthreads();
    TL(7);

    {
        TileJob job[3 * TPW];
        f4 acc[3 * TPW];
#pragma unroll
        for (int i = 0; i < TPW; ++i) {
            const int t = min(nb.wave + i * WAVES, HT - 1);
#pragma unroll
            for (int k = 0; k < 3; ++k) { job[3 * i + k] = tile_job<HT>(wb + lo.xv2, k * HT + t, hx); acc[3 * i + k] = f4zero(); }
        }
        dense_seq<HT, 3 * TPW>(job, nb.lane, acc);
#pragma unroll
        for (int i = 0; i < TPW; ++i) {
            const int t = nb.wave + i * WAVES;
            if (t < HT && nb.valid) {
                const f4 a = acc[3 * i], b = acc[3 * i + 1], c = acc[3 * i + 2];
                st_blk(s_out, n, D::HP, t, nb.lane, lds_blk(in, t, nb.lane) + (a + b + vdk[i]) * inv_sqrt2);
#pragma unroll
                for (int x = 0; x < 3; ++x)
                    st_blk(vec_out, (size_t)n * 3 + x, D::HP, t, nb.lane,
                           lds_blk(vx + x * HT * 256, t, nb.lane) + c * v2k[i][x]);
            }
        }
    }
    TL(0);
    TL_END();
}

template <class D, int WAVES>
__global__ __launch_bounds__(WAVES * 64) void k_neighbor_v1(TopoDev tp, const float* __restrict__ wb, PackOff po,
                                                            const float* __restrict__ zemb, const float* __restrict__ nbe,
                                                            const float* __restrict__ ew, float* __restrict__ s,
                                                            float* __restrict__ s1) {
    constexpr int HT = D::HT, TPW = (HT + WAVES - 1) / WAVES;
    __shared__ __attribute__((aligned(16))) float sm[2 * HT * 256];
    float* sv = sm;
    float* yv = sm + HT * 256;
    const NodeBlk nb = node_blk(tp.N, tp.npb);
    const int n = nb.n, smp = tp.node_sample[n], s0 = tp.sample_ptr[smp];
    const int ns = nb.valid ? tp.sample_ptr[smp + 1] - s0 : 0;
    const int mx = wave_max(ns);
    const int self = n - s0;
    const float* c0f = wb + po.c0row + 2 * D::H;
    for (int t = nb.wave; t < HT; t += WAVES) {
        f4 acc = f4zero();
        const bool fok = 16 * t + 4 * nb.g < D::H;
        const int fo = 16 * t + 4 * nb.g;
        for (int k = 0; k < mx; k += 4) {
            int r[4];
#pragma unroll
            for (int i = 0; i < 4; ++i) {
                const int kk = min(k + i, max(ns - 1, 0)), m = s0 + kk;
                r[i] = kk == self ? -1 : tp.edge_row[tp.edge_ptr[m] + self - (self > kk ? 1 : 0)];
            }
            f4 f[4], x[4];
#pragma unroll
            for (int i = 0; i < 4; ++i) {
                const int kk = min(k + i, max(ns - 1, 0));
                const float* frow = (r[i] >= 0 && r[i] < tp.A) ? ew + (size_t)r[i] * D::WP + 2 * D::H : c0f;
                f[i] = fok ? ld_f4(frow + fo) : f4zero();
                x[i] = ld_blk(nbe, s0 + kk, D::HP, t, nb.lane);
            }
#pragma unroll
            for (int i = 0; i < 4; ++i)
                if (k + i < ns && r[i] >= 0) acc += f[i] * x[i];
        }
        acc += ld_blk(zemb, n, D::HP, t, nb.lane);
        lds_st(sv, t, nb.lane, acc);
        if (nb.valid) st_blk(s, n, D::HP, t, nb.lane, acc);
    }
    __syncthreads();
    {
        TileJob job[TPW];
        f4 acc[TPW];
#pragma unroll
        for (int i = 0; i < TPW; ++i) {
            const int t = min(nb.wave + i * WAVES, HT - 1);
            job[i] = tile_job<HT>(wb + po.s2v, t, sv);
            acc[i] = ld_vec(wb + po.s2v_b, t, nb.lane);
        }
        dense_seq<HT, TPW>(job, nb.lane, acc);
#pragma unroll
        for (int i = 0; i < TPW; ++i)
            if (nb.wave + i * WAVES < HT) lds_st(yv, nb.wave + i * WAVES, nb.lane, acc[i]);
    }
    __syncthreads();
    float mean, rstd;
    ln_stats_lds<HT, D::H>(yv, nb.lane, mean, rstd);
    for (int t = nb.wave; t < HT; t += WAVES) {
        const int f0 = 16 * t + 4 * nb.g;
        f4 y = (lds_blk(yv, t, nb.lane) - mean) * rstd;
        y.x = f0 + 0 < D::H ? y.x : 0.f; y.y = f0 + 1 < D::H ? y.y : 0.f;
        y.z = f0 + 2 < D::H ? y.z : 0.f; y.w = f0 + 3 < D::H ? y.w : 0.f;
        if (nb.valid) st_blk(s1, n, D::HP, t, nb.lane, silu4(y));
    }
}

template <class D, int WAVES>
__global__ __launch_bounds__(WAVES * 64) void k_s2v_agg_v1(TopoDev tp, const float* __restrict__ s1,
                                                           const float* __restrict__ ew, const float* __restrict__ geo,
                                                           float* __restrict__ ne1) {
    constexpr int HT = D::HT;
    const NodeBlk nb = node_blk(tp.N, tp.npb);
    const int n = nb.n, a0 = tp.act_ptr[n], cnt = nb.valid ? tp.act_ptr[n + 1] - a0 : 0;
    const int mx = wave_max(cnt);
    const long long a_hi = max(tp.A - 1, 0LL);
    for (int t = nb.wave; t < HT; t += WAVES) {
        f4 ax = f4zero(), ay = f4zero(), az = f4zero();
        const bool fok = 16 * t + 4 * nb.g < D::H;
        for (int k = 0; k < mx; k += 4) {
            f4 f[4], x[4];
            float gx[4], gy[4], gz[4];
#pragma unroll
            for (int i = 0; i < 4; ++i) {
                const size_t a = (size_t)min((long long)a0 + min(k + i, max(cnt - 1, 0)), a_hi);
                const int m = tp.act_src[a];
                const float* g = geo + a * GEO_STRIDE;
                gx[i] = g[2]; gy[i] = g[3]; gz[i] = g[4];
                f[i] = fok ? ld_f4(ew + a * D::WP + 2 * D::H + 16 * t + 4 * nb.g) : f4zero();
                x[i] = ld_blk(s1, m, D::HP, t, nb.lane);
            }
#pragma unroll
            for (int i = 0; i < 4; ++i)
                if (k + i < cnt) {
                    const f4 p = f[i] * x[i];
                    ax += p * gx[i]; ay += p * gy[i]; az += p * gz[i];
                }
        }
        if (nb.valid) {
            st_blk(ne1, (size_t)n * 3 + 0, D::HP, t, nb.lane, ax);
            st_blk(ne1, (size_t)n * 3 + 1, D::HP, t, nb.lane, ay);
            st_blk(ne1, (size_t)n * 3 + 2, D::HP, t, nb.lane, az);
        }
    }
}

typedef double d4 __attribute__((ext_vector_type(4)));
OARD_DEV double col_reduce64(double v) {
    v += __shfl_xor(v, 16, 64);
    v += __shfl_xor(v, 32, 64);
    return v;
}
template <int KB>
OARD_DEV d4 dense_tile_lds_f64(const float* __restrict__ wp, int t, const float* in, int lane) {
    const float* base = wp + ((size_t)t * KB * 64 + lane) * 4;
    d4 c = {0.0, 0.0, 0.0, 0.0};
    constexpr int G = 13;
#pragma unroll
    for (int b0 = 0; b0 < KB; b0 += G) {
        f4 a[G];
#pragma unroll
        for (int i = 0; i < G; ++i)
            if (b0 + i < KB) a[i] = ld_f4(base + (size_t)(b0 + i) * 256);
#pragma unroll
        for (int i = 0; i < G; ++i)
            if (b0 + i < KB) {
                const f4 x = lds_blk(in, b0 + i, lane);
                c = __builtin_amdgcn_mfma_f64_16x16x4f64((double)a[i].x, (double)x.x, c, 0, 0, 0);
                c = __builtin_amdgcn_mfma_f64_16x16x4f64((double)a[i].y, (double)x.y, c, 0, 0, 0);
                c = __builtin_amdgcn_mfma_f64_16x16x4f64((double)a[i].z, (double)x.z, c, 0, 0, 0);
                c = __builtin_amdgcn_mfma_f64_16x16x4f64((double)a[i].w, (double)x.w, c, 0, 0, 0);
            }
    }
    return c;
}

template <class D, int WAVES>
__global__ __launch_bounds__(WAVES * 64) void k_out_v1(TopoDev tp, const float* __restrict__ wb, PackOff po,
                                                       const float* __restrict__ s, const float* __restrict__ vec,
                                                       float* __restrict__ dpos, float* __restrict__ hout,
                                                       int* __restrict__ status) {
    constexpr int HT = D::HT, TPW = (HT + WAVES - 1) / WAVES;
    __shared__ __attribute__((aligned(16))) float sm[5 * HT * 256];
    __shared__ double red[4][16][16];
    float* vx = sm;
    float* in = sm + 3 * HT * 256;
    const NodeBlk nb = node_blk(tp.N, tp.npb);
    const int n = nb.n;
    double part[3] = {0.0, 0.0, 0.0};
    for (int t = nb.wave; t < HT; t += WAVES) {
        const f4 w = ld_vec(wb + po.v2p, t, nb.lane);
#pragma unroll
        for (int x = 0; x < 3; ++x) {
            const f4 v = ld_blk(vec, (size_t)n * 3 + x, D::HP, t, nb.lane);
            lds_st(vx + x * HT * 256, t, nb.lane, v);
            part[x] += (double)v.x * (double)w.x + (double)v.y * (double)w.y + (double)v.z * (double)w.z + (double)v.w * (double)w.w;
        }
        lds_st(in, t, nb.lane, ld_blk(s, n, D::HP, t, nb.lane));
    }
#pragma unroll
    for (int x = 0; x < 3; ++x) {
        const double p = col_reduce64(part[x]);
        if (nb.g == 0 && nb.wave < 16) red[x][nb.wave][nb.lane & 15] = p;
    }
    __syncthreads();
    {
        TileJob job[TPW];
        f4 acc[3 * TPW];
#pragma unroll
        for (int i = 0; i < TPW; ++i) {
            job[i] = tile_job<HT>(wb + po.v1p, min(nb.wave + i * WAVES, HT - 1), vx);
#pragma unroll
            for (int x = 0; x < 3; ++x) acc[3 * i + x] = f4zero();
        }
        dense_seq_xyz<HT, TPW, HT * 256, OARD_NODE_SEQ_G, true>(job, nb.lane, acc);
#pragma unroll
        for (int i = 0; i < TPW; ++i)
            if (nb.wave + i * WAVES < HT) {
                const f4 q = acc[3 * i] * acc[3 * i] + acc[3 * i + 1] * acc[3 * i + 1] + acc[3 * i + 2] * acc[3 * i + 2];
                lds_st(in, HT + nb.wave + i * WAVES, nb.lane, (f4){sqrtf(q.x), sqrtf(q.y), sqrtf(q.z), sqrtf(q.w)});
            }
    }
    __syncthreads();
    {
        const float* b0 = wb + po.un0_b;
        const float* w2 = wb + po.un2;
        double gpart = 0.0;
#pragma unroll
        for (int i = 0; i < TPW; ++i) {
            const int t = nb.wave + i * WAVES;
            if (t < HT) {
                const d4 z = dense_tile_lds_f64<2 * HT>(wb + po.un0, t, in, nb.lane);
#pragma unroll
                for (int r = 0; r < 4; ++r) {
                    const int row = 16 * t + nb.g + 4 * r;
                    const double zz = z[r] + (double)b0[row];
                    const double h = zz / (1.0 + exp(-zz));
                    gpart += (double)w2[(size_t)t * 256 + (16 * r + 1) * 4 + nb.g] * h;
                }
            }
        }
        const double gp = col_reduce64(gpart);
        if (nb.g == 0 && nb.wave < 16) red[3][nb.wave][nb.lane & 15] = gp;
    }
    __syncthreads();
    if (nb.wave == 0 && nb.valid && nb.g == 0) {
        double v[4] = {0.0, 0.0, 0.0, (double)(wb + po.un2_b)[1]};
        constexpr int NWV = WAVES < 16 ? WAVES : 16;
#pragma unroll
        for (int x = 0; x < 4; ++x)
            for (int w = 0; w < NWV; ++w) v[x] += red[x][w][nb.lane & 15];
        const float d0 = (float)(v[3] * v[0]), d1 = (float)(v[3] * v[1]), d2 = (float)(v[3] * v[2]);
        dpos[n * 3] = d0; dpos[n * 3 + 1] = d1; dpos[n * 3 + 2] = d2;
        if (isnan(d0) || isnan(d1) || isnan(d2)) atomicOr(status, 1);
    }
    if (nb.wave == (WAVES > 1 ? 1 : 0)) {
        const f4 ho = dense_tile_lds<HT>(wb + po.embout, 0, in, nb.lane, ld_vec(wb + po.embout_b, 0, nb.lane));
        if (nb.valid) st_blk(hout, n, 16, 0, nb.lane, ho);
    }
}
```

oareactdiff_amd/csrc/oard_plan.h:

```cpp
#pragma once
#include <algorithm>
#include "../../include/oard.h"

struct FwdOptions {
    int gcl_variant = 2;
    int equi_variant = 2;
    int node_variant = 1;
    int auto_small = 4;
    int auto_tiny = 8;
    int small_split = 128;
    int gcl_persist = 1;
    int gcl_grid = 0;
    int gcl_skip = 1;
    int equi_skip = 1;
    int equi_l0_skip = 1;
    int gcl_msum = 1;
    int equi_rbf_table = 1;
};

enum GclShape {
    GCL_INVALID = 0,
    GCL_V0,
    GCL_PERSIST, GCL_RING3,
    GCL_W4, GCL_SMALL, GCL_B3,
    GCL_TRAIN_PERSIST, GCL_TRAIN_RING3, GCL_TRAIN_B3,
    GCL_X0 = 100
};
enum EquiShape { EQ_INVALID = 0, EQ_V0, EQ_W8, EQ_W4, EQ_SMALL, EQ_SMALL_SPLIT, EQ_B3, EQ_TRAIN, EQ_TRAIN_B3 };
enum NodeForm { NODE_V0 = 0, NODE_ROWS, NODE_LARGE };

struct GclLaunch { long long r0, r1; bool s1, s3; GclShape shape; long long grid; };
struct GclLayer { int n; GclLaunch l[2]; };
struct FwdPlanIn {
    FwdOptions opt;
    int precision;
    bool train;
    int conc, npb, cus;
    long long A, E, CI, CX;
    int num_layers;
    bool scratch;
    unsigned rbf_good = 0;
};
struct FwdPlan {
    int num_layers;
    bool fill_edges;
    bool init_v1;
    bool scalarize_tiles;
    bool msum;
    GclLayer gcl[4];
    EquiShape equi;
    bool use_al;
    NodeForm node;
    bool l0_skip;
    bool rbf_table[16];
    const GclLayer& gcl_at(int l) const { return gcl[(l == 0 ? 1 : 0) | (l == num_layers - 1 ? 2 : 0)]; }
};

inline long long plan_cdiv(long long a, long long b) { return (a + b - 1) / b; }
inline int plan_demote(const FwdPlanIn& in, int v, long long n, long long small_tiles, int w4, int lat) {
    const long long load = plan_cdiv(n, 16) * in.conc;
    if (v == 2 && load <= small_tiles * in.opt.auto_small) v = w4;
    if ((v == 2 || v == w4) && load <= 512LL * in.opt.auto_tiny) v = lat;
    return v;
}
inline GclShape plan_gcl_shape(const FwdPlanIn& in, long long n) {
    const int persist = in.opt.gcl_persist;
    if (in.train) return (in.precision & OARD_PREC_TRAIN_BF16X3) ? GCL_TRAIN_B3 : persist ? GCL_TRAIN_PERSIST : GCL_TRAIN_RING3;
    const int v = plan_demote(in, in.opt.gcl_variant, n, 1024, 3, 6);
    switch (v) {
        case 0: return GCL_V0;
        case 2: return (in.precision & OARD_PREC_GCL_BF16X3) ? GCL_B3 : (persist > 1 || (persist == 1 && in.conc == 1)) ? GCL_PERSIST : GCL_RING3;
        case 3: return GCL_W4;
        case 6: return GCL_SMALL;
#ifdef OARD_EXPERIMENTS
        case 4: case 5: case 7: case 8: case 9: case 10: case 11: case 12: return GclShape(GCL_X0 + v);
#endif
        default: return GCL_INVALID;
    }
}
inline long long plan_gcl_grid(const FwdPlanIn& in, GclShape s, long long n) {
    if (s == GCL_PERSIST || s == GCL_TRAIN_PERSIST) {
        const long long nhalf = plan_cdiv(plan_cdiv(n, 16), 4), g = in.opt.gcl_grid;
        return std::min(nhalf, g > 0 ? g : g < 0 ? plan_cdiv(nhalf, 2 * -g) : in.conc > 1 ? std::max(1, in.cus / 2) : in.cus);
    }
    return plan_cdiv(n, s == GCL_SMALL ? 16 : (s == GCL_V0 || s == GCL_W4 || s == GCL_X0 + 12) ? 64 : (s == GCL_X0 + 10 || s == GCL_X0 + 11) ? 192 : 128);
}
inline EquiShape plan_equi_shape(const FwdPlanIn& in) {
    if (in.train) return (in.precision & OARD_PREC_TRAIN_BF16X3) ? EQ_TRAIN_B3 : EQ_TRAIN;
    switch (plan_demote(in, in.opt.equi_variant, in.A, 512, 1, 4)) {
        case 0: return EQ_V0;
        case 1: return EQ_W4;
        case 2: return (in.precision & OARD_PREC_EQUI_BF16X3) ? EQ_B3 : EQ_W8;
        case 4: return in.scratch && plan_cdiv(in.A, 16) * in.conc <= in.opt.small_split ? EQ_SMALL_SPLIT : EQ_SMALL;
        default: return EQ_INVALID;
    }
}
inline bool plan_rbf_wanted(const FwdPlanIn& in) {
    return !in.train && in.opt.equi_rbf_table && in.A > 0 && plan_equi_shape(in) == EQ_W8;
}
inline FwdPlan make_fwd_plan(FwdPlanIn in) {
    if (in.train) { in.opt.gcl_variant = in.opt.equi_variant = 2; in.opt.node_variant = 1; in.opt.gcl_skip = 1; }
    const FwdOptions& o = in.opt;
    const bool nv1 = o.node_variant == 1 && o.equi_variant != 0, skip = o.gcl_skip && o.gcl_variant != 0;
    FwdPlan p = {};
    p.num_layers = in.num_layers;
    p.fill_edges = !skip;
    p.init_v1 = o.node_variant >= 1;
    p.scalarize_tiles = plan_cdiv(in.A, 64) * in.conc <= 2048;
    p.node = !nv1 ? NODE_V0 : in.npb <= 4 ? NODE_ROWS : NODE_LARGE;
    p.equi = plan_equi_shape(in);
    p.use_al = !in.train && o.equi_skip && in.A > 0 && nv1;
    p.l0_skip = !in.train && o.equi_l0_skip && in.A > 0 && p.node == NODE_LARGE && p.equi == EQ_W8;
    for (int l = 0; l < 16; ++l)
        p.rbf_table[l] = !in.train && o.equi_rbf_table && in.A > 0 && p.equi == EQ_W8 && l < in.num_layers && ((in.rbf_good >> l) & 1u);
    auto throughput = [&](long long n) { const GclShape s = plan_gcl_shape(in, n); return n == 0 || s == GCL_PERSIST || s == GCL_RING3; };
    p.msum = !in.train && o.gcl_msum && in.E > 0 && o.gcl_variant == 2 && p.node == NODE_LARGE && throughput(in.CI) && throughput(in.CX);
    const long long inner = p.msum ? in.CI : in.A, all = p.msum ? in.CI + in.CX : in.E;
    for (int k = 0; k < 4; ++k) {
        GclLayer& g = p.gcl[k];
        auto add = [&](long long r0, long long r1, bool s1, bool s3) {
            const GclShape s = plan_gcl_shape(in, r1 - r0);
            if (r1 > r0) g.l[g.n++] = GclLaunch{r0, r1, s1, s3, s, plan_gcl_grid(in, s, r1 - r0)};
        };
        const bool s1 = !(skip && (k & 1)), s3 = !(skip && (k & 2));
        if (s1 && s3) add(0, all, true, true);
        else { add(0, inner, true, true); add(inner, all, s1, s3); }
    }
    return p;
}
```

Before: 3697 reaction-steps/s.

## Split equivariant node update into lean per-channel edge aggregation plus node kernel

New measurement: 3710 reaction-steps/s, median of 6. Within noise of the previous version (+0.4%).

```diff
diff --git a/oareactdiff_amd/_capi.py b/oareactdiff_amd/_capi.py
--- a/oareactdiff_amd/_capi.py
+++ b/oareactdiff_amd/_capi.py
@@ -192,7 +192,7 @@
     L.oard_timing_reset.argtypes = []; L.oard_timing_reset.restype = C.c_int
     L.oard_timing_get.argtypes = [C.c_char_p, C.POINTER(C.c_double), C.POINTER(i64)]; L.oard_timing_get.restype = C.c_int
     for env, opt in (("OARD_GCL_VARIANT", b"gcl_variant"), ("OARD_EQUI_VARIANT", b"equi_variant"),
-                     ("OARD_NODE_VARIANT", b"node_variant"), ("OARD_GCL_SKIP", b"gcl_skip"), ("OARD_EQUI_SKIP", b"equi_skip"), ("OARD_EQUI_L0_SKIP", b"equi_l0_skip"), ("OARD_EQUI_RBF_TABLE", b"equi_rbf_table"),("OARD_GCL_MSUM", b"gcl_msum"), ("OARD_GCL_PERSIST", b"gcl_persist"), ("OARD_GCL_GRID", b"gcl_grid"), ("OARD_PARTS", b"parts"), ("OARD_SEQUENTIAL", b"sequential"), ("OARD_POISON", b"poison"), ("OARD_AUTO_SMALL", b"auto_small"), ("OARD_AUTO_TINY", b"auto_tiny"), ("OARD_NPB", b"npb"),
+                     ("OARD_NODE_VARIANT", b"node_variant"), ("OARD_GCL_SKIP", b"gcl_skip"), ("OARD_EQUI_SKIP", b"equi_skip"), ("OARD_EQUI_L0_SKIP", b"equi_l0_skip"), ("OARD_EQUI_AGG", b"equi_agg"), ("OARD_EQUI_RBF_TABLE", b"equi_rbf_table"),("OARD_GCL_MSUM", b"gcl_msum"), ("OARD_GCL_PERSIST", b"gcl_persist"), ("OARD_GCL_GRID", b"gcl_grid"), ("OARD_PARTS", b"parts"), ("OARD_SEQUENTIAL", b"sequential"), ("OARD_POISON", b"poison"), ("OARD_AUTO_SMALL", b"auto_small"), ("OARD_AUTO_TINY", b"auto_tiny"), ("OARD_NPB", b"npb"),
                      ("OARD_WGRAD_WGS", b"wgrad_wgs"), ("OARD_WGRAD_LDS", b"wgrad_lds"), ("OARD_WGRAD_T16", b"wgrad_t16"), ("OARD_WGRAD_QUEUE", b"wgrad_queue"), ("OARD_GATE_FOLD", b"gate_fold"), ("OARD_WGRAD_SHAPES", b"wgrad_shapes"), ("OARD_TRAIN_DUAL", b"train_dual"), ("OARD_SMALL_SPLIT", b"small_split"),
                      ("OARD_SKIP_FAMILIES", b"skip_families")):
         if os.environ.get(env) not in (None, ""):
diff --git a/oareactdiff_amd/csrc/oard_hip.hip b/oareactdiff_amd/csrc/oard_hip.hip
--- a/oareactdiff_amd/csrc/oard_hip.hip
+++ b/oareactdiff_amd/csrc/oard_hip.hip
@@ -70,6 +70,7 @@
 int g_poison = 0;
 int g_gcl_msum_taken = 0;
 int g_equi_l0_taken = 0;
+int g_equi_agg_taken = 0;
 int g_equi_rbf_taken = 0;
 int g_parts = 0;
 int g_wgrad_shapes = 3;
@@ -341,6 +342,7 @@
     w.d1s = take((size_t)cdiv((long long)td.A, 128) * 8 * d.D1T * 1024);
     w.small_a = E <= (size_t)OARD_SMALL_MAX_EDGES ? take(A * d.D1P * 4) : 0;
     w.rbt = take(A * RBT_ROW * 4);
+    w.eagg = take((N + 1) * 4 * d.HP * 4);
     w.total = cur;
     return w;
 }
@@ -536,6 +538,7 @@
     bool any_rbt = false, all_rbt = c->num_layers > 0;
     for (int l = 0; l < c->num_layers; ++l) { any_rbt = any_rbt || plan.rbf_table[l]; all_rbt = all_rbt && plan.rbf_table[l]; }
     g_equi_rbf_taken = all_rbt;
+    g_equi_agg_taken = plan.equi_agg;
     const bool msum = plan.msum, use_al = plan.use_al, nv1 = plan.node != NODE_V0;
     const int stop_after = train ? 0 : g_stop_after;
     int* al_cnt = (int*)(ws + w.al_cnt);
@@ -616,7 +619,16 @@
 #define EQUI_NODE_V1(D_, ROWS_, XC_) LAUNCH(F_NODE, (k_equi_node_v1<D_, NW, ROWS_, XC_>), gN16, NW * 64, st, tp, wb, lo, (const float*)vmsg, \
                        (const float*)xq, (const float*)geo, (const float*)x1, (const float*)s_mid_at(l), s_at(l + 1), (const float*)vcur, vnext, \
                        train ? (float*)(tape + to.s_a[l]) : nullptr, train ? (float*)(tape + to.vec_a[l]) : nullptr, al)
-            if (nv1 && rows) {
+            if (nv1 && plan.equi_agg && A > 0) {
+                float* eagg = (float*)(ws + w.eagg);
+#define EQUI_AGG_LEAN(D_, XC_) LAUNCH2(F_NODE, (k_equi_agg_lean<D_, XC_>), cdiv(N, 16), D::HT, 64, st, tp, (const float*)vmsg, (const float*)xq, \
+                       (const float*)geo, (const float*)vcur, eagg, al)
+                if (l0_skip) { if (lo.xcross) EQUI_AGG_LEAN(Layer0<D>, true); else EQUI_AGG_LEAN(Layer0<D>, false); }
+                else { if (lo.xcross) EQUI_AGG_LEAN(D, true); else EQUI_AGG_LEAN(D, false); }
+                LAUNCH(F_NODE, (k_equi_node_v1<AggSums<D>, NW, false, false>), gN16, NW * 64, st, tp, wb, lo, (const float*)eagg, (const float*)xq,
+                       (const float*)geo, (const float*)x1, (const float*)s_mid_at(l), s_at(l + 1), (const float*)vcur, vnext, (float*)nullptr,
+                       (float*)nullptr, ActList{nullptr, nullptr, nullptr, nullptr});
+            } else if (nv1 && rows) {
                 if (lo.xcross) EQUI_NODE_V1(D, true, true); else EQUI_NODE_V1(D, true, false);
             } else if (nv1 && l0_skip) {
                 if (lo.xcross) EQUI_NODE_V1(Layer0<D>, false, true); else EQUI_NODE_V1(Layer0<D>, false, false);
@@ -2506,13 +2518,14 @@
         {"gcl_variant", &g_fwd.gcl_variant}, {"equi_variant", &g_fwd.equi_variant}, {"node_variant", &g_fwd.node_variant},
         {"auto_small", &g_fwd.auto_small}, {"auto_tiny", &g_fwd.auto_tiny}, {"small_split", &g_fwd.small_split},
         {"gcl_persist", &g_fwd.gcl_persist}, {"gcl_grid", &g_fwd.gcl_grid}, {"gcl_skip", &g_fwd.gcl_skip}, {"equi_skip", &g_fwd.equi_skip},
-        {"equi_l0_skip", &g_fwd.equi_l0_skip}, {"gcl_msum", &g_fwd.gcl_msum}, {"equi_rbf_table", &g_fwd.equi_rbf_table},
+        {"equi_l0_skip", &g_fwd.equi_l0_skip}, {"gcl_msum", &g_fwd.gcl_msum}, {"equi_rbf_table", &g_fwd.equi_rbf_table}, {"equi_agg", &g_fwd.equi_agg},
         {"skip_families", &g_skip_families}, {"parts", &g_parts}, {"sequential", &g_sequential}, {"poison", &g_poison}, {"npb", &g_npb},
         {"wgrad_wgs", &g_wgrad_wgs}, {"wgrad_t16", &g_wgrad_t16}, {"wgrad_queue", &g_wgrad_queue}, {"gate_fold", &g_gate_fold},
         {"wgrad_lds", &g_wgrad_lds}, {"wgrad_shapes", &g_wgrad_shapes}, {"train_dual", &g_train_dual}};
     if (strcmp(name, "experiments") == 0) return kV0 ? OARD_OK : OARD_EINVAL;
     if (strcmp(name, "gcl_msum_taken") == 0) return g_gcl_msum_taken ? OARD_OK : OARD_EINVAL;
     if (strcmp(name, "equi_rbf_taken") == 0) return g_equi_rbf_taken ? OARD_OK : OARD_EINVAL;
+    if (strcmp(name, "equi_agg_taken") == 0) return g_equi_agg_taken ? OARD_OK : OARD_EINVAL;
     if (strcmp(name, "equi_l0_taken") == 0) return g_equi_l0_taken ? OARD_OK : OARD_EINVAL;
     for (const auto& e : table) {
         if (strcmp(name, e.name) != 0) continue;
diff --git a/oareactdiff_amd/csrc/oard_inst.h b/oareactdiff_amd/csrc/oard_inst.h
--- a/oareactdiff_amd/csrc/oard_inst.h
+++ b/oareactdiff_amd/csrc/oard_inst.h
@@ -62,13 +62,20 @@
 #define OARD_A_GCL_NODE (TopoDev, const float*, LayerOff, const float*, const float*, float*, float*, float*)
 #define OARD_A_OUT (TopoDev, const float*, PackOff, const float*, const float*, float*, float*, int*)
 #define OARD_A_SCAL_BWD (TopoDev, const float*, const float*, int, const float*, const float*, float*, float*)
+#define OARD_A_AGG_LEAN (TopoDev, const float*, const float*, const float*, const float*, float*, ActList)
+#ifndef OARD_A_EQUI_NODE
+#define OARD_A_EQUI_NODE (TopoDev, const float*, LayerOff, const float*, const float*, const float*, const float*, const float*, float*, const float*, float*, float*, float*, ActList)
+#endif
 #define OARD_A_MSG_BWD (TopoDev, const float*, Strided3, Strided3, const float*, Strided3, const float*, int, Strided3, float*, float*, float*, float*, int, int, int)
 #define X(h, r) \
     OARD_INST((k_gcl_node_v1<Dims<h, r>, OARD_NW(h), false>), OARD_A_GCL_NODE) OARD_INST((k_gcl_node_v1<Dims<h, r>, OARD_NW(h), true>), OARD_A_GCL_NODE) \
     OARD_INST((k_gcl_node_v1<Dims<h, r>, OARD_NW(h), false, true>), OARD_A_GCL_NODE) \
     OARD_INST((k_out_v1<Dims<h, r>, OARD_NW(h)>), OARD_A_OUT) \
     OARD_INST((k_scalarize_bwd<Dims<h, r>, 2, false>), OARD_A_SCAL_BWD) OARD_INST((k_scalarize_bwd<Dims<h, r>, 2, true>), OARD_A_SCAL_BWD) \
-    OARD_INST((k_equi_msg_bwd<Dims<h, r> >), OARD_A_MSG_BWD)
+    OARD_INST((k_equi_msg_bwd<Dims<h, r> >), OARD_A_MSG_BWD) \
+    OARD_INST((k_equi_agg_lean<Dims<h, r>, false>), OARD_A_AGG_LEAN) OARD_INST((k_equi_agg_lean<Dims<h, r>, true>), OARD_A_AGG_LEAN) \
+    OARD_INST((k_equi_agg_lean<Layer0<Dims<h, r> >, false>), OARD_A_AGG_LEAN) OARD_INST((k_equi_agg_lean<Layer0<Dims<h, r> >, true>), OARD_A_AGG_LEAN) \
+    OARD_INST((k_equi_node_v1<AggSums<Dims<h, r> >, OARD_NW(h), false, false>), OARD_A_EQUI_NODE)
 OARD_DIMS_LIST
 #undef X
 OARD_INST((k_lin3u_bwd_fused<4>), (const float*, const float*, const float*, long long, float*, float*))
diff --git a/oareactdiff_amd/csrc/oard_layout.h b/oareactdiff_amd/csrc/oard_layout.h
--- a/oareactdiff_amd/csrc/oard_layout.h
+++ b/oareactdiff_amd/csrc/oard_layout.h
@@ -124,4 +124,5 @@
     size_t rbt;
     size_t d1s;
     size_t small_a;
+    size_t eagg;
 };
diff --git a/oareactdiff_amd/csrc/oard_node_v1.h b/oareactdiff_amd/csrc/oard_node_v1.h
--- a/oareactdiff_amd/csrc/oard_node_v1.h
+++ b/oareactdiff_amd/csrc/oard_node_v1.h
@@ -472,6 +472,24 @@
 template <class D> struct Layer0 : D {};
 template <class D> struct is_layer0 { static constexpr bool value = false; };
 template <class D> struct is_layer0<Layer0<D> > { static constexpr bool value = true; };
+template <class D> struct AggSums : D {};
+template <class D> struct is_agg_sums { static constexpr bool value = false; };
+template <class D> struct is_agg_sums<AggSums<D> > { static constexpr bool value = true; };
+
+template <bool XC>
+OARD_DEV void equi_msg_add(f4& dx, f4& v0, f4& v1, f4& v2, f4 xn0, f4 xn1, f4 xn2, f4 y0, f4 y1, f4 y2, f4 q0, f4 q1, f4 q2,
+                           f4 w0, f4 w1, f4 w2, float gx, float gy, float gz, float cx, float cy, float cz,
+                           float inv_sqrt3, float inv_sqrt_h) {
+    const f4 xm = (y0 + xn0) * q0;
+    dx += xm;
+    const f4 a2 = (y1 + xn1) * q1 * inv_sqrt3;
+    const f4 a3 = (y2 + xn2) * q2;
+    const f4 u0 = __builtin_elementwise_fma(w0, a2, a3 * gx), u1 = __builtin_elementwise_fma(w1, a2, a3 * gy),
+             u2 = __builtin_elementwise_fma(w2, a2, a3 * gz);
+    v0 += (XC ? u0 + xm * cx : u0) * inv_sqrt_h;
+    v1 += (XC ? u1 + xm * cy : u1) * inv_sqrt_h;
+    v2 += (XC ? u2 + xm * cz : u2) * inv_sqrt_h;
+}
 template <class D, int WAVES, bool ROWS = false, bool XC = false>
 __global__ __launch_bounds__(WAVES * 64) void k_equi_node_v1(TopoDev tp, const float* __restrict__ wb, LayerOff lo,
                                                              const float* __restrict__ qbuf, const float* __restrict__ xq,
@@ -480,8 +498,9 @@
                                                              float* __restrict__ vec_out,
                                                              float* __restrict__ sa_out, float* __restrict__ va_out ,
                                                              ActList al ) {
-    constexpr bool L0 = is_layer0<D>::value;
+    constexpr bool L0 = is_layer0<D>::value, AGG = is_agg_sums<D>::value;
     static_assert(!(L0 && ROWS), "the layer-0 form exists for the large-batch gather only");
+    static_assert(!(AGG && (ROWS || XC)), "the form that reads the sums has one instantiation: it forms no message");
     constexpr int HT = D::HT;
     constexpr int TPW = (HT + WAVES - 1) / WAVES;
     __shared__ __attribute__((aligned(16))) float sm[6 * HT * 256 + 48 * 12 + L3T_FLOATS];
@@ -517,88 +536,80 @@
 
     for (int t = nb.wave; t < HT; t += WAVES) {
         f4 dx = f4zero(), v0 = f4zero(), v1 = f4zero(), v2 = f4zero();
-        const f4 xn0 = ld_blk(xq, n, 3 * D::HP, t, nb.lane), xn1 = ld_blk(xq, n, 3 * D::HP, HT + t, nb.lane),
-                 xn2 = ld_blk(xq, n, 3 * D::HP, 2 * HT + t, nb.lane);
-        const int a_hi = (int)max(tp.A - 1, 0LL);
-        if (ROWS) {
-            const RowLanes rl = row_lanes(tp.N, tp.npb, nb.lane);
-            const int nn = min(blockIdx.x * tp.npb + rl.node, tp.N - 1);
-            const int b0 = listed ? al.pre[tp.act_ptr[nn]] : tp.act_ptr[nn];
-            const int cnt2 = rl.live ? (listed ? al.pre[tp.act_ptr[nn + 1]] : tp.act_ptr[nn + 1]) - b0 : 0;
-            const int mx2 = wave_max(cnt2);
-            const f4 zn0 = ld_blk(xq, nn, 3 * D::HP, t, nb.lane), zn1 = ld_blk(xq, nn, 3 * D::HP, HT + t, nb.lane),
-                     zn2 = ld_blk(xq, nn, 3 * D::HP, 2 * HT + t, nb.lane);
-            for (int k = 0; k < mx2; k += rl.L) {
-                const int kk = k + rl.slot;
-                const int ke = min(b0 + min(kk, max(cnt2 - 1, 0)), a_hi);
-                const size_t a = cnt2 > 0 ? (size_t)row_of(ke) : 0;
-                const int m = cnt2 > 0 ? src_of(ke) : 0;
-                const float* gp = geo + a * GEO_STRIDE;
-                const float gx = gp[2], gy = gp[3], gz = gp[4];
-                const float cx = XC ? gp[5] : 0.f, cy = XC ? gp[6] : 0.f, cz = XC ? gp[7] : 0.f;
-                const f4 q0 = ld_blk(qbuf, a, 3 * D::HP, t, nb.lane), q1 = ld_blk(qbuf, a, 3 * D::HP, HT + t, nb.lane),
-                         q2 = ld_blk(qbuf, a, 3 * D::HP, 2 * HT + t, nb.lane);
-                const f4 y0 = ld_blk(xq, m, 3 * D::HP, t, nb.lane), y1 = ld_blk(xq, m, 3 * D::HP, HT + t, nb.lane),
-                         y2 = ld_blk(xq, m, 3 * D::HP, 2 * HT + t, nb.lane);
-                const f4 w0 = ld_blk(vec_in, (size_t)m * 3 + 0, D::HP, t, nb.lane), w1 = ld_blk(vec_in, (size_t)m * 3 + 1, D::HP, t, nb.lane),
-                         w2 = ld_blk(vec_in, (size_t)m * 3 + 2, D::HP, t, nb.lane);
-                if (kk < cnt2) {
-                    const f4 xm = (y0 + zn0) * q0;
-                    dx += xm;
-                    const f4 a2 = (y1 + zn1) * q1 * inv_sqrt3;
-                    const f4 a3 = (y2 + zn2) * q2;
-                    v0 += (XC ? w0 * a2 + a3 * gx + xm * cx : w0 * a2 + a3 * gx) * inv_sqrt_h;
-                    v1 += (XC ? w1 * a2 + a3 * gy + xm * cy : w1 * a2 + a3 * gy) * inv_sqrt_h;
-                    v2 += (XC ? w2 * a2 + a3 * gz + xm * cz : w2 * a2 + a3 * gz) * inv_sqrt_h;
+        if constexpr (AGG) {
+            dx = ld_blk(qbuf, (size_t)n * 4 + 0, D::HP, t, nb.lane); v0 = ld_blk(qbuf, (size_t)n * 4 + 1, D::HP, t, nb.lane);
+            v1 = ld_blk(qbuf, (size_t)n * 4 + 2, D::HP, t, nb.lane); v2 = ld_blk(qbuf, (size_t)n * 4 + 3, D::HP, t, nb.lane);
+        } else {
+            const f4 xn0 = ld_blk(xq, n, 3 * D::HP, t, nb.lane), xn1 = ld_blk(xq, n, 3 * D::HP, HT + t, nb.lane),
+                     xn2 = ld_blk(xq, n, 3 * D::HP, 2 * HT + t, nb.lane);
+            const int a_hi = (int)max(tp.A - 1, 0LL);
+            if (ROWS) {
+                const RowLanes rl = row_lanes(tp.N, tp.npb, nb.lane);
+                const int nn = min(blockIdx.x * tp.npb + rl.node, tp.N - 1);
+                const int b0 = listed ? al.pre[tp.act_ptr[nn]] : tp.act_ptr[nn];
+                const int cnt2 = rl.live ? (listed ? al.pre[tp.act_ptr[nn + 1]] : tp.act_ptr[nn + 1]) - b0 : 0;
+                const int mx2 = wave_max(cnt2);
+                const f4 zn0 = ld_blk(xq, nn, 3 * D::HP, t, nb.lane), zn1 = ld_blk(xq, nn, 3 * D::HP, HT + t, nb.lane),
+                         zn2 = ld_blk(xq, nn, 3 * D::HP, 2 * HT + t, nb.lane);
+                for (int k = 0; k < mx2; k += rl.L) {
+                    const int kk = k + rl.slot;
+                    const int ke = min(b0 + min(kk, max(cnt2 - 1, 0)), a_hi);
+                    const size_t a = cnt2 > 0 ? (size_t)row_of(ke) : 0;
+                    const int m = cnt2 > 0 ? src_of(ke) : 0;
+                    const float* gp = geo + a * GEO_STRIDE;
+                    const float gx = gp[2], gy = gp[3], gz = gp[4];
+                    const float cx = XC ? gp[5] : 0.f, cy = XC ? gp[6] : 0.f, cz = XC ? gp[7] : 0.f;
+                    const f4 q0 = ld_blk(qbuf, a, 3 * D::HP, t, nb.lane), q1 = ld_blk(qbuf, a, 3 * D::HP, HT + t, nb.lane),
+                             q2 = ld_blk(qbuf, a, 3 * D::HP, 2 * HT + t, nb.lane);
+                    const f4 y0 = ld_blk(xq, m, 3 * D::HP, t, nb.lane), y1 = ld_blk(xq, m, 3 * D::HP, HT + t, nb.lane),
+                             y2 = ld_blk(xq, m, 3 * D::HP, 2 * HT + t, nb.lane);
+                    const f4 w0 = ld_blk(vec_in, (size_t)m * 3 + 0, D::HP, t, nb.lane), w1 = ld_blk(vec_in, (size_t)m * 3 + 1, D::HP, t, nb.lane),
+                             w2 = ld_blk(vec_in, (size_t)m * 3 + 2, D::HP, t, nb.lane);
+                    if (kk < cnt2)
+                        equi_msg_add<XC>(dx, v0, v1, v2, zn0, zn1, zn2, y0, y1, y2, q0, q1, q2, w0, w1, w2, gx, gy, gz, cx, cy, cz, inv_sqrt3, inv_sqrt_h);
                 }
-            }
-            dx = rows_total4(dx, rl, nb.lane); v0 = rows_total4(v0, rl, nb.lane);
-            v1 = rows_total4(v1, rl, nb.lane); v2 = rows_total4(v2, rl, nb.lane);
-        }
-        int mnext[2], rnext[2];
-        auto entry = [&](int kk, int& m, int& r) {
-            const int ke = min(a0 + min(kk, max(cnt - 1, 0)), a_hi);
-            m = cnt > 0 ? src_of(ke) : 0;
-            r = cnt > 0 ? row_of(ke) : 0;
-        };
-#pragma unroll
-        for (int i = 0; i < 2; ++i) entry(i, mnext[i], rnext[i]);
-        float zero1 = 0.f;
-        if (L0) asm volatile("" : "+v"(zero1));
-        const f4 zero4 = {zero1, zero1, zero1, zero1};
-        for (int k = 0; !ROWS && k < mx; k += 2) {
-            f4 q0[2], q1[2], q2[2], y0[2], y1[2], y2[2], w0[2], w1[2], w2[2];
-            float gx[2], gy[2], gz[2], cx[2], cy[2], cz[2];
-            const int mc[2] = {mnext[0], mnext[1]}, rc[2] = {rnext[0], rnext[1]};
-#pragma unroll
-            for (int i = 0; i < 2; ++i)
-                entry(k + 2 + i, mnext[i], rnext[i]);
-#pragma unroll
-            for (int i = 0; i < 2; ++i) {
-                const size_t a = (size_t)rc[i];
-                const int m = mc[i];
-                const float* g = geo + a * GEO_STRIDE;
-                gx[i] = g[2]; gy[i] = g[3]; gz[i] = g[4];
-                cx[i] = XC ? g[5] : 0.f; cy[i] = XC ? g[6] : 0.f; cz[i] = XC ? g[7] : 0.f;
-                q0[i] = ld_blk(qbuf, a, 3 * D::HP, t, nb.lane); q1[i] = L0 ? zero4 : ld_blk(qbuf, a, 3 * D::HP, HT + t, nb.lane);
-                q2[i] = ld_blk(qbuf, a, 3 * D::HP, 2 * HT + t, nb.lane);
-                y0[i] = ld_blk(xq, m, 3 * D::HP, t, nb.lane); y1[i] = L0 ? zero4 : ld_blk(xq, m, 3 * D::HP, HT + t, nb.lane);
-                y2[i] = ld_blk(xq, m, 3 * D::HP, 2 * HT + t, nb.lane);
-                w0[i] = L0 ? zero4 : ld_blk(vec_in, (size_t)m * 3 + 0, D::HP, t, nb.lane);
-                w1[i] = L0 ? zero4 : ld_blk(vec_in, (size_t)m * 3 + 1, D::HP, t, nb.lane);
-                w2[i] = L0 ? zero4 : ld_blk(vec_in, (size_t)m * 3 + 2, D::HP, t, nb.lane);
-            }
-#pragma unroll
-            for (int i = 0; i < 2; ++i)
-                if (k + i < cnt) {
-                    const f4 xm = (y0[i] + xn0) * q0[i];
-                    dx += xm;
-                    const f4 a2 = (y1[i] + xn1) * q1[i] * inv_sqrt3;
-                    const f4 a3 = (y2[i] + xn2) * q2[i];
-                    v0 += (XC ? w0[i] * a2 + a3 * gx[i] + xm * cx[i] : w0[i] * a2 + a3 * gx[i]) * inv_sqrt_h;
-                    v1 += (XC ? w1[i] * a2 + a3 * gy[i] + xm * cy[i] : w1[i] * a2 + a3 * gy[i]) * inv_sqrt_h;
-                    v2 += (XC ? w2[i] * a2 + a3 * gz[i] + xm * cz[i] : w2[i] * a2 + a3 * gz[i]) * inv_sqrt_h;
+                dx = rows_total4(dx, rl, nb.lane); v0 = rows_total4(v0, rl, nb.lane);
+                v1 = rows_total4(v1, rl, nb.lane); v2 = rows_total4(v2, rl, nb.lane);
+            }
+            int mnext[2], rnext[2];
+            auto entry = [&](int kk, int& m, int& r) {
+                const int ke = min(a0 + min(kk, max(cnt - 1, 0)), a_hi);
+                m = cnt > 0 ? src_of(ke) : 0;
+                r = cnt > 0 ? row_of(ke) : 0;
+            };
+#pragma unroll
+            for (int i = 0; i < 2; ++i) entry(i, mnext[i], rnext[i]);
+            float zero1 = 0.f;
+            if (L0) asm volatile("" : "+v"(zero1));
+            const f4 zero4 = {zero1, zero1, zero1, zero1};
+            for (int k = 0; !ROWS && k < mx; k += 2) {
+                f4 q0[2], q1[2], q2[2], y0[2], y1[2], y2[2], w0[2], w1[2], w2[2];
+                float gx[2], gy[2], gz[2], cx[2], cy[2], cz[2];
+                const int mc[2] = {mnext[0], mnext[1]}, rc[2] = {rnext[0], rnext[1]};
+#pragma unroll
+                for (int i = 0; i < 2; ++i)
+                    entry(k + 2 + i, mnext[i], rnext[i]);
+#pragma unroll
+                for (int i = 0; i < 2; ++i) {
+                    const size_t a = (size_t)rc[i];
+                    const int m = mc[i];
+                    const float* g = geo + a * GEO_STRIDE;
+                    gx[i] = g[2]; gy[i] = g[3]; gz[i] = g[4];
+                    cx[i] = XC ? g[5] : 0.f; cy[i] = XC ? g[6] : 0.f; cz[i] = XC ? g[7] : 0.f;
+                    q0[i] = ld_blk(qbuf, a, 3 * D::HP, t, nb.lane); q1[i] = L0 ? zero4 : ld_blk(qbuf, a, 3 * D::HP, HT + t, nb.lane);
+                    q2[i] = ld_blk(qbuf, a, 3 * D::HP, 2 * HT + t, nb.lane);
+                    y0[i] = ld_blk(xq, m, 3 * D::HP, t, nb.lane); y1[i] = L0 ? zero4 : ld_blk(xq, m, 3 * D::HP, HT + t, nb.lane);
+                    y2[i] = ld_blk(xq, m, 3 * D::HP, 2 * HT + t, nb.lane);
+                    w0[i] = L0 ? zero4 : ld_blk(vec_in, (size_t)m * 3 + 0, D::HP, t, nb.lane);
+                    w1[i] = L0 ? zero4 : ld_blk(vec_in, (size_t)m * 3 + 1, D::HP, t, nb.lane);
+                    w2[i] = L0 ? zero4 : ld_blk(vec_in, (size_t)m * 3 + 2, D::HP, t, nb.lane);
                 }
+#pragma unroll
+                for (int i = 0; i < 2; ++i)
+                    if (k + i < cnt)
+                        equi_msg_add<XC>(dx, v0, v1, v2, xn0, xn1, xn2, y0[i], y1[i], y2[i], q0[i], q1[i], q2[i], w0[i], w1[i], w2[i],
+                                         gx[i], gy[i], gz[i], cx[i], cy[i], cz[i], inv_sqrt3, inv_sqrt_h);
+            }
         }
         const f4 sa = (ld_blk(s, n, D::HP, t, nb.lane) + dx) * inv_sqrt2;
         v0 += ld_blk(vec_in, (size_t)n * 3 + 0, D::HP, t, nb.lane);
@@ -703,6 +714,70 @@
     TL_END();
 }
 
+template <class D, bool XC>
+__global__ __launch_bounds__(64) void k_equi_agg_lean(TopoDev tp, const float* __restrict__ qbuf, const float* __restrict__ xq, const float* __restrict__ geo,
+                     const float* __restrict__ vec_in, float* __restrict__ eagg, ActList al) {
+    constexpr bool L0 = is_layer0<D>::value;
+    constexpr int HT = D::HT, EF = L0 ? 2 : 1;
+    const int lane = threadIdx.x, t = blockIdx.y;
+    const int c = blockIdx.x * 16 + (lane & 15);
+    const bool valid = c < tp.N;
+    const int n = valid ? c : tp.N - 1;
+    const bool listed = al.pre != nullptr && (long long)__builtin_amdgcn_readfirstlane(*al.n) != tp.A;
+    const int a0 = listed ? al.pre[tp.act_ptr[n]] : tp.act_ptr[n];
+    const int cnt = valid ? (listed ? al.pre[tp.act_ptr[n + 1]] : tp.act_ptr[n + 1]) - a0 : 0;
+    const int mx = wave_max(cnt);
+    const int a_hi = (int)max(tp.A - 1, 0LL);
+    const float inv_sqrt3 = 0.57735026918962576f, inv_sqrt_h = 1.0f / sqrtf((float)D::H);
+    auto entry = [&](int kk, int& m, int& r) {
+        const int ke = min(a0 + min(kk, max(cnt - 1, 0)), a_hi);
+        m = cnt > 0 ? (listed ? al.src[ke] : tp.act_src[ke]) : 0;
+        r = cnt > 0 ? (listed ? al.rows[ke] : ke) : 0;
+    };
+    f4 dx = f4zero(), v0 = f4zero(), v1 = f4zero(), v2 = f4zero();
+    float zero1 = 0.f;
+    if (L0) asm volatile("" : "+v"(zero1));
+    const f4 zero4 = {zero1, zero1, zero1, zero1};
+    const f4 xn0 = ld_blk(xq, n, 3 * D::HP, t, lane), xn1 = ld_blk(xq, n, 3 * D::HP, HT + t, lane),
+             xn2 = ld_blk(xq, n, 3 * D::HP, 2 * HT + t, lane);
+    int mnext[EF], rnext[EF];
+#pragma unroll
+    for (int i = 0; i < EF; ++i) entry(i, mnext[i], rnext[i]);
+    for (int k = 0; k < mx; k += EF) {
+        f4 q0[EF], q1[EF], q2[EF], y0[EF], y1[EF], y2[EF], w0[EF], w1[EF], w2[EF];
+        float gx[EF], gy[EF], gz[EF], cx[EF], cy[EF], cz[EF];
+        int mc[EF], rc[EF];
+#pragma unroll
+        for (int i = 0; i < EF; ++i) { mc[i] = mnext[i]; rc[i] = rnext[i]; }
+#pragma unroll
+        for (int i = 0; i < EF; ++i)
+            entry(k + EF + i, mnext[i], rnext[i]);
+#pragma unroll
+        for (int i = 0; i < EF; ++i) {
+            const size_t a = (size_t)rc[i];
+            const int m = mc[i];
+            const float* g = geo + a * GEO_STRIDE;
+            gx[i] = g[2]; gy[i] = g[3]; gz[i] = g[4];
+            cx[i] = XC ? g[5] : 0.f; cy[i] = XC ? g[6] : 0.f; cz[i] = XC ? g[7] : 0.f;
+            q0[i] = ld_blk(qbuf, a, 3 * D::HP, t, lane); q1[i] = L0 ? zero4 : ld_blk(qbuf, a, 3 * D::HP, HT + t, lane);
+            q2[i] = ld_blk(qbuf, a, 3 * D::HP, 2 * HT + t, lane);
+            y0[i] = ld_blk(xq, m, 3 * D::HP, t, lane); y1[i] = L0 ? zero4 : ld_blk(xq, m, 3 * D::HP, HT + t, lane);
+            y2[i] = ld_blk(xq, m, 3 * D::HP, 2 * HT + t, lane);
+            w0[i] = L0 ? zero4 : ld_blk(vec_in, (size_t)m * 3 + 0, D::HP, t, lane);
+            w1[i] = L0 ? zero4 : ld_blk(vec_in, (size_t)m * 3 + 1, D::HP, t, lane);
+            w2[i] = L0 ? zero4 : ld_blk(vec_in, (size_t)m * 3 + 2, D::HP, t, lane);
+        }
+#pragma unroll
+        for (int i = 0; i < EF; ++i)
+            if (k + i < cnt)
+                equi_msg_add<XC>(dx, v0, v1, v2, xn0, xn1, xn2, y0[i], y1[i], y2[i], q0[i], q1[i], q2[i], w0[i], w1[i], w2[i],
+                                 gx[i], gy[i], gz[i], cx[i], cy[i], cz[i], inv_sqrt3, inv_sqrt_h);
+    }
+    const size_t row = (size_t)(valid ? c : tp.N) * 4;
+    st_blk(eagg, row + 0, D::HP, t, lane, dx); st_blk(eagg, row + 1, D::HP, t, lane, v0);
+    st_blk(eagg, row + 2, D::HP, t, lane, v1); st_blk(eagg, row + 3, D::HP, t, lane, v2);
+}
+
 template <class D, int WAVES>
 __global__ __launch_bounds__(WAVES * 64) void k_neighbor_v1(TopoDev tp, const float* __restrict__ wb, PackOff po,
                                                             const float* __restrict__ zemb, const float* __restrict__ nbe,
diff --git a/oareactdiff_amd/csrc/oard_plan.h b/oareactdiff_amd/csrc/oard_plan.h
--- a/oareactdiff_amd/csrc/oard_plan.h
+++ b/oareactdiff_amd/csrc/oard_plan.h
@@ -16,6 +16,7 @@
     int equi_l0_skip = 1;
     int gcl_msum = 1;
     int equi_rbf_table = 1;
+    int equi_agg = 1;
 };
 
 enum GclShape {
@@ -53,6 +54,7 @@
     NodeForm node;
     bool l0_skip;
     bool rbf_table[16];
+    bool equi_agg = false;
     const GclLayer& gcl_at(int l) const { return gcl[(l == 0 ? 1 : 0) | (l == num_layers - 1 ? 2 : 0)]; }
 };
 
@@ -111,6 +113,7 @@
     p.equi = plan_equi_shape(in);
     p.use_al = !in.train && o.equi_skip && in.A > 0 && nv1;
     p.l0_skip = !in.train && o.equi_l0_skip && in.A > 0 && p.node == NODE_LARGE && p.equi == EQ_W8;
+    p.equi_agg = !in.train && o.equi_agg && in.A > 0 && p.node == NODE_LARGE && p.equi == EQ_W8;
     for (int l = 0; l < 16; ++l)
         p.rbf_table[l] = !in.train && o.equi_rbf_table && in.A > 0 && p.equi == EQ_W8 && l < in.num_layers && ((in.rbf_good >> l) & 1u);
     auto throughput = [&](long long n) { const GclShape s = plan_gcl_shape(in, n); return n == 0 || s == GCL_PERSIST || s == GCL_RING3; };
```
